# FabricioArendTorres/FlowConductor

Measured on AMD Instinct MI355X. Metric: log_prob samples/sec, 32xRQ-NSF coupling D=64 K=8, higher is better.
Workload: dtype f32

## Files before the change

flowconductor_amd/_hip.py:

```python
import ctypes
import os

import torch

_HERE = os.path.dirname(os.path.abspath(__file__))
LIB_PATH = os.path.join(_HERE, "csrc", "libflowcon_hip.so")

ABI_VERSION = 3

ERR_OUTSIDE_DOMAIN = 1
ERR_DISCRIMINANT = 2
ERR_NONFINITE = 4
ERR_NOT_LOWER_TRIANGULAR = 8
ERR_DIAGONAL_NONPOSITIVE = 16
ERR_NOT_SYMMETRIC = 32
ERR_NOT_POSITIVE_DEFINITE = 64
ERR_CHOLESKY_FAILED = 128


class HipLibraryMissing(RuntimeError):
    pass


class RQConfig(ctypes.Structure):

    _fields_ = [
        ("num_bins", ctypes.c_int32),
        ("tails", ctypes.c_int32),
        ("inverse", ctypes.c_int32),
        ("flags", ctypes.c_int32),
        ("left", ctypes.c_float),
        ("right", ctypes.c_float),
        ("bottom", ctypes.c_float),
        ("top", ctypes.c_float),
        ("min_bin_width", ctypes.c_double),
        ("min_bin_height", ctypes.c_double),
        ("min_derivative", ctypes.c_double),
        ("wh_divisor", ctypes.c_float),
        ("softplus_beta", ctypes.c_float),
        ("tail_constant", ctypes.c_float),
        ("reserved2", ctypes.c_float),
    ]


class SplineConfig(ctypes.Structure):

    _fields_ = [
        ("kind", ctypes.c_int32),
        ("num_bins", ctypes.c_int32),
        ("tails", ctypes.c_int32),
        ("inverse", ctypes.c_int32),
        ("left", ctypes.c_float),
        ("right", ctypes.c_float),
        ("bottom", ctypes.c_float),
        ("top", ctypes.c_float),
        ("min_bin_width", ctypes.c_double),
        ("min_bin_height", ctypes.c_double),
        ("width_divisor", ctypes.c_float),
        ("height_divisor", ctypes.c_float),
        ("cubic_eps", ctypes.c_float),
        ("cubic_quadratic_threshold", ctypes.c_float),
    ]


class PackJob(ctypes.Structure):

    _fields_ = [("w", ctypes.c_void_p), ("b", ctypes.c_void_p), ("frag", ctypes.c_void_p), ("unscale", ctypes.c_void_p),
                ("bias_out", ctypes.c_void_p), ("rows", ctypes.c_int32), ("cols", ctypes.c_int32),
                ("mode", ctypes.c_int32), ("p", ctypes.c_int32), ("pp", ctypes.c_int32), ("nks", ctypes.c_int32),
                ("nt", ctypes.c_int32), ("group", ctypes.c_int32)]


_P = ctypes.c_void_p
_I32 = ctypes.c_int32
_I64 = ctypes.c_int64
_F = ctypes.c_float

SIGNATURES = {
    "fc_abi_version": [],
    "fc_rq_spline": [_P, _P, _P, _P, _P, _P, _I64, _I32, _I32, _I32, _I32,
                     ctypes.POINTER(RQConfig), _P],
    "fc_rq_spline_backward": [_P, _P, _P, _P, _P, _P, _P, _I64, _I32, _I32, ctypes.POINTER(RQConfig), _P],
    "fc_standard_normal_log_prob": [_P, _P, _P, _I64, _I32, _F, _P],
    "fc_permute": [_P, _P, _P, _I64, _I32, _I64, _P],
    "fc_pointwise_affine": [_P, _P, _P, _P, _P, _P, _I64, _I64, _I32, _I32, _I32, _P],
    "fc_householder": [_P, _P, _P, _I64, _I32, _I32, _I32, _I32, _P],
    "fc_planar": [_P, _P, _P, _P, _P, _P, _I64, _I32, _I32, _P],
    "fc_linear_per_sample": [_P, _P, _P, _P, _I64, _I32, _I32, _F, _F, _P],
    "fc_linear": [_P, _P, _P, _P, _P, _I64, _I32, _I32, _P],
    "fc_sylvester": [_P, _P, _P, _P, _P, _P, _P, _P, _I64, _I32, _I32, _I32, _P],
    "fc_sum_of_sigmoids": [_P, _P, _P, _P, _P, _P, _I64, _I32, _I32, _I32, _I32, _I32, _F, _F, _F,
                           _I32, _I32, _P],
    "fc_sum_of_sigmoids_backward": [_P, _P, _P, _P, _P, _P, _I64, _I32, _I32, _F, _P],
    "fc_deep_sigmoid": [_P, _P, _P, _P, _P, _P, _I64, _I32, _I32, _I32, _I32, _I32, _F, _F, _F, _F, _I32, _I32, _P],
    "fc_deep_sigmoid_backward": [_P, _P, _P, _P, _P, _P, _I64, _I32, _I32, _F, _F, _F, _I32, _P],
    "fc_deep_sigmoid_backward_rows": [_I64, _I32, _I32],
    "fc_planar_backward": [_P, _P, _P, _P, _P, _P, _P, _P, _P, _P, _I64, _I32, _P],
    "fc_sylvester_mid_backward": [_P, _P, _P, _P, _P, _P, _I64, _I32, _P],
    "fc_householder_backward": [_P, _P, _P, _P, _P, _I64, _I32, _I32, _I32, _P],
    "fc_hdh_linear": [_P] * 7 + [_I64, _I32, _I32, _I32, _I32, _I32, _P],
    "fc_hdh_linear_backward": [_P] * 12 + [_I64, _I32, _I32, _I32, _I32, _I32, _P],
    "fc_elementwise": [_P, _P, _P, _P, _P, _P, _I64, _I64, _I32, _I32, _F, _F, _F, _F, _P],
    "fc_piecewise_spline_backward": [_P, _P, _P, _P, _P, _P, _P, _I64, _I32, _I32, ctypes.POINTER(SplineConfig), _P],
    "fc_piecewise_spline": [_P, _P, _P, _P, _P, _P, _I64, _I32, _I32, _I32, _I32,
                            ctypes.POINTER(SplineConfig), _P],
    "fc_rq_spline_fused_linear": [_P, _P, _P, _P, _P, _P, _P, _P, _I64, _I32, _I32, _I32,
                                  ctypes.POINTER(RQConfig), _P],
    "fc_rq_spline_fused_general": [_P, _P, _P, _P, _P, _P, _P, _P, _P, _I64, _I32, _I32, _I32,
                                   ctypes.POINTER(RQConfig), _P],
    "fc_rq_fused_linear_backward": [_I32, _P, _P, _P, _P, _P, _P, _P, _P, _P, _P, _P, _P, _P, _I64, _I32, _I32,
                                    ctypes.POINTER(RQConfig), _P],
    "fc_resnet_hidden": [_P, _P, _P, _P, _P, _P, _P, _I64, _I32, _I32, _I32, _I32, _I32, ctypes.c_float, _P],
    "fc_affine_coupling_resnet": [_P, _P, _P, _P, _P, _P, _P, _P, _I64, _I32, _I32, _I32, _I32, _I32, _I32, _I32, _I32, _P],
    "fc_made_inverse": [_P, _P, _P, _P, _P, _P, _P, _P, _P, _P, _P, _I64, _I32, _I32, _I32, _I32, ctypes.POINTER(RQConfig), _P],
    "fc_made_inverse_context": [_P] * 15 + [_I64, _I32, _I32, _I32, _I32, _I32, ctypes.POINTER(RQConfig), _P],
    "fc_mog_log_prob": [_P, _P, _P, _I64, _I32, _I32, _F, _I32, _P],
    "fc_mog_log_prob_backward": [_P, _P, _P, _P, _P, _I64, _I32, _I32, _F, _P],
    "fc_made_mog_sample": [_P] * 11 + [_I64, _I32, _I32, _I32, _F, _P],
    "fc_made_mog_sample_context": [_P] * 15 + [_I64, _I32, _I32, _I32, _I32, _F, _P],
    "fc_resnet_hidden_packed": [_P, _P, _P, _P, _P, _P, _I64, _I32, _I32, _I32, _I32, _I32, ctypes.c_float, _P],
    "fc_resnet_hidden_backward": [_P, _P, _P, _P, _P, _P, _P, _P, _P, _P, _P, _I64, _I32, _I32, _I32, _I32, _I32, _P],
    "fc_resnet_hidden_backward_accum": [_P, _P, _P, _P, _P, _P, _P, _P, _P, _P, _P, _I64, _I32, _I32, _I32, _I32, _I32, _P],
    "fc_resnet_hidden_wide": [_P, _P, _P, _P, _P, _P, _I64, _I32, _I32, _I32, _I32, _I32, ctypes.c_float, _P],
    "fc_resnet_hidden_context": [_P, _P, _P, _P, _P, _P, _P, _P, _P, _P, _I64, _I32, _I32, _I32, _I32, _I32, _I32,
                                 _I32, ctypes.c_float, _P],
    "fc_affine": [_P, _P, _P, _P, _P, _I64, _I32, _I32, _I32, _I32, _I32, _I32, _P],
    "fc_dense_mm": [_P, _P, _P, _P, _I64, _I32, _P],
    "fc_dense_mm_shifted": [_P, _P, _P, _P, _P, _I64, _I32, _P],
    "fc_sylvester_mm": [_P, _P, _P, _P, _P, _P, _P, _I64, _I32, _P],
    "fc_affine_backward": [_P, _P, _P, _P, _P, _P, _P, _I64, _I32, _I32, _I32, _P],
    "fc_pack_fragments": [_P, _I32, _P],
    "fc_pack_job_bytes": [],
    "fc_comm_unique_id": [_P],
    "fc_comm_init_rank": [ctypes.POINTER(ctypes.c_void_p), _I32, _P, _I32],
    "fc_comm_init_rank_on_device": [ctypes.POINTER(ctypes.c_void_p), _I32, _P, _I32, _I32],
    "fc_comm_destroy": [_P],
    "fc_comm_abort": [_P],
    "fc_allreduce_loglik": [_P, _P, _P],
    "fc_tril_pack": [_P, _P, _I64, _I32, _I32, _P],
    "fc_matrix_diag": [_P, _P, _P, _I64, _I32, _I32, _P],
    "fc_cholesky_outer": [_P, _P, _P, _P, _I64, _I32, _I32, _P],
    "fc_cholesky_outer_backward": [_P, _P, _P, _P, _I64, _I32, _P],
    "fc_cholesky": [_P, _P, _P, _P, _I64, _I32, _F, _I32, _P],
    "fc_squeeze": [_P, _P, _I64, _I32, _I32, _I32, _I32, _P],
    "fc_conv1x1": [_P, _P, _P, _P, _P, _I64, _I32, _I64, _P],
    "fc_iresnet_forward": [_P, _P, _P, _P, _P, _P, _I64, _I32, _I32, _I32, _I32, _I32, _I32, _P],
    "fc_iresnet_inverse": [_P, _P, _P, _P, _P, _P, _I64, _I32, _I32, _I32, _I32, _I32, _I32, _I32, _F, _F, _P],
    "fc_umnn": [_P] * 7 + [_I64, _I32, _I32, _I32, _I32, _I32, _I32, _P],
    "fc_radial": [_P] * 6 + [_I64, _I32, _I32, _P],
    "fc_radial_backward": [_P] * 10 + [_I64, _I32, _P],
    "fc_unit_vector": [_P] * 4 + [_I64, _I32, _I32, _P],
    "fc_unit_vector_backward": [_P] * 4 + [_I64, _I32, _I32, _P],
}

_lib = None


def use_library(path):
    global LIB_PATH
    if _lib is not None:
        raise RuntimeError("flowconductor_amd: %s is already loaded" % LIB_PATH)
    LIB_PATH = os.path.abspath(path)


def library_info():
    import hashlib

    with open(LIB_PATH, "rb") as f:
        blob = f.read()
    return {"path": os.path.relpath(LIB_PATH, os.path.dirname(_HERE)), "sha256": hashlib.sha256(blob).hexdigest(),
            "bytes": len(blob)}


def load():
    global _lib
    if _lib is not None:
        return _lib
    if not os.path.exists(LIB_PATH):
        raise HipLibraryMissing(
            "flowconductor_amd: %s not found. Build it with `python -c 'import __graft_entry__ as g; "
            "g.build()'` or `make -C flowconductor_amd/csrc`. There is no CPU fallback." % LIB_PATH
        )
    lib = ctypes.CDLL(LIB_PATH)
    for name, argtypes in SIGNATURES.items():
        fn = getattr(lib, name)
        fn.argtypes = argtypes
        fn.restype = ctypes.c_int
    got = lib.fc_abi_version()
    if got != ABI_VERSION:
        raise HipLibraryMissing("libflowcon_hip.so ABI %d != expected %d: rebuild" % (got, ABI_VERSION))
    _lib = lib
    return lib


def is_built():
    return os.path.exists(LIB_PATH)


def check(code, what):
    if code != 0:
        raise RuntimeError("flowconductor_amd: %s failed with hipError %d" % (what, code))


_raw_stream = getattr(torch._C, "_cuda_getCurrentRawStream", None)


def stream_ptr(device):
    if _raw_stream is not None:
        index = device.index
        return ctypes.c_void_p(_raw_stream(torch.cuda.current_device() if index is None else index))
    return ctypes.c_void_p(torch.cuda.current_stream(device).cuda_stream)


def dev_f32(t, name):
    if not isinstance(t, torch.Tensor):
        raise TypeError("%s must be a tensor" % name)
    if not t.is_cuda:
        raise RuntimeError(
            "flowconductor_amd: %s lives on %s; the bijector kernels run on a HIP device only "
            "(no CPU fallback)" % (name, t.device)
        )
    if t.dtype != torch.float32:
        raise TypeError("flowconductor_amd: %s must be float32, got %s" % (name, t.dtype))
    return t if t.is_contiguous() else t.contiguous()


def ptr(t):
    return ctypes.c_void_p(t.data_ptr()) if t is not None else None


def require_no_grad(*tensors):
    if torch.is_grad_enabled() and any(t is not None and t.requires_grad for t in tensors):
        raise RuntimeError(
            "flowconductor_amd: the HIP bijector kernels implement forward/inverse/logabsdet only; "
            "autograd through them is not available yet. Wrap the call in torch.no_grad()."
        )
```

flowconductor_amd/csrc/fc_resnet_hidden.hip:

```cpp
#include <hip/hip_runtime.h>
#include <stdint.h>
#include "fc_split.h"
#include "fc_lane.h"
#include "fc_math.h"
#include "fc_device.h"
#include "../../include/flowcon_hip.h"

#ifndef FC_HIDDEN_PREFETCH_X
#define FC_HIDDEN_PREFETCH_X 1
#endif

namespace fc {

constexpr int kHid = 64;
constexpr int kHidThreads = 512;

struct HiddenArgs {
  const float* x;
  float* h;
  const int32_t* id_cols;
  const float* w0;
  const float* b0;
  const float* wb;
  const float* bb;
  int64_t blocks16;
  int D;
  int k0;
  const float* ctx;
  const float* wc;
  const float* bc;
  int C;
  int act;
  float act_param;
  const f16x8* image;
  const float* image_un;
  const float* image_bias;
  float* y;
  const int32_t* tr_cols;
  float* lad;
  int d_t, affine_act, inverse, accumulate;
};

__host__ __device__ constexpr int hid_feat(int t, int g, int r) { return 32 * (t >> 1) + 8 * g + 4 * (t & 1) + r; }

template <int NB, int K0S, int kCtx, int kTail = 0>
struct HiddenLds {
  static constexpr int kMain = 1 + 2 * NB + kTail;
  static constexpr int kCtxLayers = kCtx == 1 ? NB : kCtx == 2 ? NB + 1 : 0;
  static constexpr int kLayers = kMain + kCtxLayers;
  static constexpr int kFrag0 = K0S * 4 * 2;
  static constexpr int kFragL = 2 * 4 * 2;
  static constexpr int kFragG = 1 * 4 * 2;
  static constexpr int kFragsMain = kFrag0 + (2 * NB + kTail) * kFragL;
  static constexpr int kFrags = kFragsMain + kCtxLayers * kFragG;
  static constexpr size_t kBytes = (size_t)kFrags * 64 * 16 + kLayers * 64 * 4 + 16 * 4 + 32 * K0S * 4 + 16 * 8 * 4;
  static_assert(kLayers <= 16, "wun holds 16 entries");
  static_assert(kBytes <= 160 * 1024, "weight fragments exceed the CU's LDS");
};

template <int NB, int K0S, int kCtx, int kAct, int BPW, int kTail = 0, int XVT = 8>
__global__ __launch_bounds__(512, (kCtx || BPW > 1 || kTail) ? 2 : 4) void resnet_hidden_kernel(HiddenArgs a) {
  static_assert(!kTail || kCtx == 0, "the coupling tail: no context");
  using L = HiddenLds<NB, K0S, kCtx, kTail>;
  constexpr bool kPrefetchX = FC_HIDDEN_PREFETCH_X && (K0S == 1 || kCtx != 0 || BPW > 1);
  extern __shared__ __attribute__((aligned(16))) unsigned char hsmem[];
  f16x8* wfrag = reinterpret_cast<f16x8*>(hsmem);
  float* bias = reinterpret_cast<float*>(hsmem + (size_t)L::kFrags * 64 * 16);
  float* wun = bias + L::kLayers * 64;
  int* ids = reinterpret_cast<int*>(wun + 16);
  float* red = reinterpret_cast<float*>(ids + 32 * K0S);

  const int tid = threadIdx.x, lane = tid & 63, wave = tid >> 6;
  const int s16 = lane & 15, g = lane >> 4;
  const int k0 = a.k0, D = a.D, C = kCtx ? a.C : 0;
#ifdef FC_HID_STAMP
  const uint64_t stamp_entry = __builtin_amdgcn_s_memtime();
#endif

  const int C0 = kCtx == 1 ? C : 0;
  for (int i = tid; i < 32 * K0S; i += kHidThreads) ids[i] = i < k0 ? a.id_cols[i] : (i < k0 + C0 ? -2 - (i - k0) : -1);
  if (kCtx == 0 && a.image) {
    for (int f = wave; f < L::kFrags; f += kHidThreads / 64)
      __builtin_amdgcn_global_load_lds((const __attribute__((address_space(1))) void*)(a.image + (size_t)f * 64 + lane),
                                       (__attribute__((address_space(3))) void*)(wfrag + f * 64), 16, 0, 0);
    for (int i = tid; i < L::kLayers * 64; i += kHidThreads) bias[i] = a.image_bias[i];
    if (tid < L::kLayers) wun[tid] = a.image_un[tid];
    asm volatile("s_waitcnt vmcnt(0)" ::: "memory");
    __syncthreads();
  } else if constexpr (!kTail) {
  auto layer_src = [&](int l, const float*& w, const float*& b, int& kin, int& nks, int& base) {
    const bool gate = l >= L::kMain;
    w = l == 0 ? a.w0 : gate ? a.wc + (size_t)(l - L::kMain) * kHid * C : a.wb + (size_t)(l - 1) * kHid * kHid;
    b = l == 0 ? a.b0 : gate ? a.bc + (size_t)(l - L::kMain) * kHid : a.bb + (size_t)(l - 1) * kHid;
    kin = l == 0 ? k0 + C0 : gate ? C : kHid;
    nks = l == 0 ? K0S : gate ? 1 : 2;
    base = l == 0 ? 0 : gate ? L::kFragsMain + (l - L::kMain) * L::kFragG : L::kFrag0 + (l - 1) * L::kFragL;
  };
  float wmax[L::kLayers];
#pragma unroll
  for (int l = 0; l < L::kLayers; ++l) {
    const float *w, *b;
    int kin, nks, base;
    layer_src(l, w, b, kin, nks, base);
    float m = 0.f;
    if (kin == kHid) {
      const float4* w4 = reinterpret_cast<const float4*>(w) + 2 * tid;
      const float4 p = w4[0], q = w4[1];
      m = fmaxf(fmaxf(fmaxf(fabsf(p.x), fabsf(p.y)), fmaxf(fabsf(p.z), fabsf(p.w))),
                fmaxf(fmaxf(fabsf(q.x), fabsf(q.y)), fmaxf(fabsf(q.z), fabsf(q.w))));
    } else {
      const int total = kHid * kin;
      for (int i = tid; i < total; i += 4 * kHidThreads) {
        const float v0 = w[i];
        const float v1 = i + kHidThreads < total ? w[i + kHidThreads] : 0.f;
        const float v2 = i + 2 * kHidThreads < total ? w[i + 2 * kHidThreads] : 0.f;
        const float v3 = i + 3 * kHidThreads < total ? w[i + 3 * kHidThreads] : 0.f;
        m = fmaxf(fmaxf(m, fmaxf(fabsf(v0), fabsf(v1))), fmaxf(fabsf(v2), fabsf(v3)));
      }
    }
    wmax[l] = m;
  }
#pragma unroll
  for (int l = 0; l < L::kLayers; ++l) {
    float m = wmax[l];
#pragma unroll
    for (int o = 32; o > 0; o >>= 1) m = fmaxf(m, __shfl_xor(m, o));
    if (lane == 0) red[l * (kHidThreads / 64) + wave] = m;
  }
  __syncthreads();
#pragma unroll
  for (int l = 0; l < L::kLayers; ++l) {
    const float *w, *b;
    int kin, nks, base;
    layer_src(l, w, b, kin, nks, base);
    float m = red[l * (kHidThreads / 64)];
#pragma unroll
    for (int i = 1; i < kHidThreads / 64; ++i) m = fmaxf(m, red[l * (kHidThreads / 64) + i]);
    float sc, un;
    pow2_scale(m, sc, un);
    if (tid == 0) wun[l] = un;
    for (int e = tid; e < nks * 4 * 64; e += kHidThreads) {
      const int ln = e & 63, t = (e >> 6) & 3, ks = e >> 8;
      const int rho = ln & 15, f = hid_feat(t, rho >> 2, rho & 3);
      f16x8 hi, lo;
      float v[8];
      if (kin == kHid) {
        const float4* w4 = reinterpret_cast<const float4*>(w + (size_t)f * kHid + 32 * ks + 8 * (ln >> 4));
        const float4 p = w4[0], q = w4[1];
        v[0] = p.x, v[1] = p.y, v[2] = p.z, v[3] = p.w, v[4] = q.x, v[5] = q.y, v[6] = q.z, v[7] = q.w;
      } else {
#pragma unroll
        for (int j = 0; j < 8; ++j) {
          const int k = 32 * ks + 8 * (ln >> 4) + j;
          v[j] = k < kin ? w[(size_t)f * kin + k] : 0.f;
        }
      }
#pragma unroll
      for (int j = 0; j < 8; ++j) {
        _Float16 ph, pl;
        split2(v[j] * sc, ph, pl);
        hi[j] = ph;
        lo[j] = pl;
      }
      wfrag[(base + (ks * 4 + t) * 2 + 0) * 64 + ln] = hi;
      wfrag[(base + (ks * 4 + t) * 2 + 1) * 64 + ln] = lo;
    }
    for (int i = tid; i < 64; i += kHidThreads) {
      const int gg = i >> 4, t = (i >> 2) & 3, r = i & 3;
      bias[l * 64 + i] = b[hid_feat(t, gg, r)];
    }
  }
  __syncthreads();
  }

  auto activate16 = [&](const f32x4 (&in)[4], f32x4 (&out)[4]) {
#define FC_ACT_LOOP(expr)                                            \
  _Pragma("unroll") for (int t = 0; t < 4; ++t)                      \
  _Pragma("unroll") for (int r = 0; r < 4; ++r) {                    \
    const float v = in[t][r];                                        \
    out[t][r] = (expr);                                              \
  }
    if constexpr (kAct == 0) {
      FC_ACT_LOOP(fmaxf(v, 0.f))
    } else {
      switch (a.act) {
        case FC_ACT_TANH: FC_ACT_LOOP(tanhf(v)) break;
        case FC_ACT_SILU: FC_ACT_LOOP(div_lean(v, 1.f + exp_lean(fminf(-v, 87.f)))) break;
        case FC_ACT_ELU: FC_ACT_LOOP(v > 0.f ? v : a.act_param * (exp_lean(v) - 1.f)) break;
        case FC_ACT_LEAKY_RELU: FC_ACT_LOOP(v > 0.f ? v : v * a.act_param) break;
        case FC_ACT_SIGMOID: FC_ACT_LOOP(div_lean(1.f, 1.f + exp_lean(fminf(-v, 87.f)))) break;
        default: FC_ACT_LOOP(fmaxf(v, 0.f)) break;
      }
    }
#undef FC_ACT_LOOP
  };
  auto make_operand = [&](const f32x4 (&v)[4], f16x8 (&bh)[2], f16x8 (&bl)[2]) {
    float m = 0.f;
#pragma unroll
    for (int t = 0; t < 4; ++t)
#pragma unroll
      for (int r = 0; r < 4; ++r) m = fmaxf(m, fabsf(v[t][r]));
    m = rows4_allmax(m, lane);
    float sc, un;
    pow2_scale(m, sc, un);
    u32x4 hh[2], ll[2];
#pragma unroll
    for (int t = 0; t < 4; ++t)
#pragma unroll
      for (int p = 0; p < 2; ++p) {
        uint32_t ph, pl;
        split2_pair(v[t][2 * p], v[t][2 * p + 1], sc, ph, pl);
        hh[t >> 1][2 * (t & 1) + p] = ph;
        ll[t >> 1][2 * (t & 1) + p] = pl;
      }
#pragma unroll
    for (int ks = 0; ks < 2; ++ks) {
      bh[ks] = __builtin_bit_cast(f16x8, hh[ks]);
      bl[ks] = __builtin_bit_cast(f16x8, ll[ks]);
    }
    return un;
  };
  auto layer = [&](int base, int nks, const f16x8 (&bh)[BPW][2], const f16x8 (&bl)[BPW][2], f32x4 (&acc)[BPW][4]) {
#pragma unroll
    for (int b = 0; b < BPW; ++b)
#pragma unroll
      for (int t = 0; t < 4; ++t) acc[b][t] = f32x4{0.f, 0.f, 0.f, 0.f};
    const f16x8* wf = wfrag + base * 64 + lane;
#pragma unroll
    for (int ks = 0; ks < 2; ++ks)
      if (ks < nks) {
        f16x8 wl[4];
#pragma unroll
        for (int t = 0; t < 4; ++t) wl[t] = wf[((ks * 4 + t) * 2 + 1) * 64];
#pragma unroll
        for (int t = 0; t < 4; ++t)
#pragma unroll
          for (int b = 0; b < BPW; ++b) acc[b][t] = __builtin_amdgcn_mfma_f32_16x16x32_f16(wl[t], bh[b][ks], acc[b][t], 0, 0, 0);
      }
#pragma unroll
    for (int ks = 0; ks < 2; ++ks)
      if (ks < nks) {
        f16x8 wh[4];
#pragma unroll
        for (int t = 0; t < 4; ++t) wh[t] = wf[((ks * 4 + t) * 2 + 0) * 64];
#pragma unroll
        for (int t = 0; t < 4; ++t)
#pragma unroll
          for (int b = 0; b < BPW; ++b) acc[b][t] = __builtin_amdgcn_mfma_f32_16x16x32_f16(wh[t], bl[b][ks], acc[b][t], 0, 0, 0);
#pragma unroll
        for (int t = 0; t < 4; ++t)
#pragma unroll
          for (int b = 0; b < BPW; ++b) acc[b][t] = __builtin_amdgcn_mfma_f32_16x16x32_f16(wh[t], bh[b][ks], acc[b][t], 0, 0, 0);
      }
  };
  auto finish = [&](int l, float un_act, const f32x4 (&acc)[4], f32x4 (&out)[4]) {
    const float c = un_act * wun[l];
    const f32x4* bsrc = reinterpret_cast<const f32x4*>(bias + l * 64 + g * 16);
#pragma unroll
    for (int t = 0; t < 4; ++t) {
      const f32x4 b = bsrc[t];
#pragma unroll
      for (int r = 0; r < 4; ++r) out[t][r] = __builtin_fmaf(acc[t][r], c, b[r]);
    }
  };

  int mycol[K0S][8];
#pragma unroll
  for (int ks = 0; ks < K0S; ++ks)
#pragma unroll
    for (int j = 0; j < 8; ++j) mycol[ks][j] = ids[32 * ks + 8 * g + j];

  const int64_t nwaves = (int64_t)gridDim.x * (kHidThreads / 64);
  int alt = -1;
  if (kCtx == 0 && D == 2 * k0 && k0 == 32 * K0S && ((uintptr_t)a.x & 15u) == 0 && (ids[0] == 0 || ids[0] == 1)) {
    alt = ids[0];
    for (int i = 1; i < k0; ++i)
      if (ids[i] != 2 * i + ids[0]) alt = -1;
  }
  auto gather = [&](int64_t blk, f32x4 (&xv)[4]) {
    const float* xrow = a.x + (blk * 16 + s16) * D;
    const float* crow_ = kCtx ? a.ctx + (blk * 16 + s16) * C : nullptr;
    if (alt >= 0) {
#pragma unroll
      for (int ks = 0; ks < 2; ++ks) {
        if (ks < K0S) {
          const float4* q = reinterpret_cast<const float4*>(xrow + 64 * ks + 16 * g);
          const float4 q0 = q[0], q1 = q[1], q2 = q[2], q3 = q[3];
          xv[2 * ks] = alt ? f32x4{q0.y, q0.w, q1.y, q1.w} : f32x4{q0.x, q0.z, q1.x, q1.z};
          xv[2 * ks + 1] = alt ? f32x4{q2.y, q2.w, q3.y, q3.w} : f32x4{q2.x, q2.z, q3.x, q3.z};
        } else {
          xv[2 * ks] = xv[2 * ks + 1] = f32x4{0.f, 0.f, 0.f, 0.f};
        }
      }
      return;
    }
#pragma unroll
    for (int t = 0; t < 4; ++t)
#pragma unroll
      for (int r = 0; r < 4; ++r) {
        const int ks = t >> 1, j = 4 * (t & 1) + r;
        float v = 0.f;
        if (ks < K0S) {
          const int c = mycol[ks < K0S ? ks : 0][j];
          if constexpr (kCtx == 1)
            v = c >= 0 ? xrow[c] : (c <= -2 ? crow_[-2 - c] : 0.f);
          else
            v = c >= 0 ? xrow[c] : 0.f;
        }
        xv[t][r] = v;
      }
  };
  if constexpr (kTail) {
    const int TS = D | 1, wrap = TS - D;
    float* tile = reinterpret_cast<float*>(hsmem + ((L::kBytes + 15) & ~size_t(15))) + (size_t)wave * BPW * 16 * TS;
    const int chunk4 = 4 * D;
    constexpr int XV = XVT;
    int toff[XV], tcol[XV];
#pragma unroll
    for (int k = 0; k < XV; ++k) {
      const int e = 4 * (lane + 64 * k), r = e / D;
      tcol[k] = e - r * D;
      toff[k] = r * TS + tcol[k];
    }
    auto fetch_rows = [&](int64_t blk, float4 (&raw)[XV]) __attribute__((always_inline)) {
      const float4* src = reinterpret_cast<const float4*>(a.x + blk * 16 * D);
#pragma unroll
      for (int k = 0; k < XV; ++k)
        if (lane + 64 * k < chunk4) raw[k] = src[lane + 64 * k];
    };
    const int64_t groups = (a.blocks16 + BPW - 1) / BPW;
    const int64_t nw = (int64_t)gridDim.x * (kHidThreads / 64);
    const int64_t first = (int64_t)blockIdx.x * (kHidThreads / 64) + wave;
    auto blk_of = [&](int64_t grp, int b) {
      const int64_t blk = grp * BPW + b;
      return blk < a.blocks16 ? blk : a.blocks16 - 1;
    };
    float4 raw[BPW][XV];
    if (first < groups) {
#pragma unroll
      for (int b = 0; b < BPW; ++b) fetch_rows(blk_of(first, b), raw[b]);
    }
    int tc[8];
#pragma unroll
    for (int e = 0; e < 8; ++e) {
      const int dim = 8 * g + e;
      tc[e] = a.tr_cols[dim < a.d_t ? dim : 0];
    }
    for (int64_t grp = first; grp < groups; grp += nw) {
      asm volatile("" ::: "memory");
#pragma unroll
      for (int b = 0; b < BPW; ++b)
#pragma unroll
        for (int k = 0; k < XV; ++k)
          if (lane + 64 * k < chunk4) {
            const float v[4] = {raw[b][k].x, raw[b][k].y, raw[b][k].z, raw[b][k].w};
#pragma unroll
            for (int j = 0; j < 4; ++j) tile[b * 16 * TS + toff[k] + j + (tcol[k] + j >= D ? wrap : 0)] = v[j];
          }
      __builtin_amdgcn_wave_barrier();
      if (grp + nw < groups) {
#pragma unroll
        for (int b = 0; b < BPW; ++b) fetch_rows(blk_of(grp + nw, b), raw[b]);
      }
      f32x4 xin[BPW][4];
      float xt[BPW][8];
#pragma unroll
      for (int b = 0; b < BPW; ++b) {
        const float* trow = tile + (b * 16 + s16) * TS;
#pragma unroll
        for (int t = 0; t < 4; ++t)
#pragma unroll
          for (int r = 0; r < 4; ++r) {
            const int ks = t >> 1, j = 4 * (t & 1) + r;
            float v = 0.f;
            if (ks < K0S) {
              const int c = mycol[ks < K0S ? ks : 0][j];
              v = c >= 0 ? trow[c] : 0.f;
            }
            xin[b][t][r] = v;
          }
#pragma unroll
        for (int e = 0; e < 8; ++e) xt[b][e] = trow[tc[e]];
      }
      f16x8 bh[BPW][2], bl[BPW][2];
      f32x4 acc[BPW][4], h[BPW][4], tmid[BPW][4];
      float un[BPW];
#pragma unroll
      for (int b = 0; b < BPW; ++b) un[b] = make_operand(xin[b], bh[b], bl[b]);
      layer(0, K0S, bh, bl, acc);
#pragma unroll
      for (int b = 0; b < BPW; ++b) finish(0, un[b], acc[b], h[b]);
#pragma unroll
      for (int nb = 0; nb < NB; ++nb) {
#pragma unroll
        for (int b = 0; b < BPW; ++b) {
          f32x4 act[4];
          activate16(h[b], act);
          un[b] = make_operand(act, bh[b], bl[b]);
        }
        layer(L::kFrag0 + (2 * nb) * L::kFragL, 2, bh, bl, acc);
#pragma unroll
        for (int b = 0; b < BPW; ++b) {
          finish(1 + 2 * nb, un[b], acc[b], tmid[b]);
          f32x4 act[4];
          activate16(tmid[b], act);
          un[b] = make_operand(act, bh[b], bl[b]);
        }
        layer(L::kFrag0 + (2 * nb + 1) * L::kFragL, 2, bh, bl, acc);
#pragma unroll
        for (int b = 0; b < BPW; ++b) {
          finish(2 + 2 * nb, un[b], acc[b], tmid[b]);
#pragma unroll
          for (int t = 0; t < 4; ++t)
#pragma unroll
            for (int r = 0; r < 4; ++r) h[b][t][r] += tmid[b][t][r];
        }
      }
#pragma unroll
      for (int b = 0; b < BPW; ++b) un[b] = make_operand(h[b], bh[b], bl[b]);
      layer(L::kFrag0 + 2 * NB * L::kFragL, 2, bh, bl, acc);
#pragma unroll
      for (int b = 0; b < BPW; ++b) {
        f32x4 prm[4];
        finish(1 + 2 * NB, un[b], acc[b], prm);
        float ladsum = 0.f;
        float* wrow = tile + (b * 16 + s16) * TS;
#pragma unroll
        for (int t = 0; t < 2; ++t)
#pragma unroll
          for (int r = 0; r < 4; ++r) {
            const int e = 4 * t + r;
            if (8 * g + e < a.d_t) {
              const float xv = xt[b][e], shift = prm[t][r], u = prm[2 + t][r];
              float sc = 1.f, ls = 0.f;
              if (a.affine_act == FC_AFFINE_SIGMOID_PLUS2) {
                const float v = u + 2.f;
                const float ex = exp_lean(-fabsf(v));
                const float rcp = div_lean(1.f, 1.f + ex);
                sc = (v >= 0.f ? rcp : ex * rcp) + 1e-3f;
                ls = log_lean(sc);
              } else if (a.affine_act == FC_AFFINE_SOFTPLUS_CLAMP3) {
                const float v = softplus_lean(u, 1.f) + 1e-3f;
                sc = v < 0.f ? 0.f : (v > 3.f ? 3.f : v);
                ls = log_lean(sc);
              } else if (a.affine_act == FC_AFFINE_MAF_SOFTPLUS) {
                sc = softplus_lean(u, 1.f) + 1e-3f;
                ls = log_lean(sc);
              }
              wrow[tc[e]] = a.inverse ? div_lean(xv - shift, sc) : xv * sc + shift;
              ladsum += a.inverse ? -ls : ls;
            }
          }
        const float l = rows4_allsum(ladsum, lane);
        const bool real = grp * BPW + b < a.blocks16;
        const int64_t row = blk_of(grp, b) * 16 + s16;
        if (g == 0 && real) a.lad[row] = a.accumulate ? a.lad[row] + l : l;
      }
      __builtin_amdgcn_wave_barrier();
#pragma unroll
      for (int b = 0; b < BPW; ++b) {
        if (grp * BPW + b >= a.blocks16) continue;
        float4* dst = reinterpret_cast<float4*>(a.y + blk_of(grp, b) * 16 * D);
#pragma unroll
        for (int k = 0; k < XV; ++k)
          if (lane + 64 * k < chunk4) {
            float v[4];
#pragma unroll
            for (int j = 0; j < 4; ++j) v[j] = tile[b * 16 * TS + toff[k] + j + (tcol[k] + j >= D ? wrap : 0)];
            dst[lane + 64 * k] = float4{v[0], v[1], v[2], v[3]};
          }
      }
      __builtin_amdgcn_wave_barrier();
    }
    return;
  }

  const int64_t groups = (a.blocks16 + BPW - 1) / BPW;
  const int64_t grp0 = (int64_t)blockIdx.x * (kHidThreads / 64) + wave;
  auto block_of = [&](int64_t grp, int b) {
    const int64_t blk = grp * BPW + b;
    return blk < a.blocks16 ? blk : a.blocks16 - 1;
  };
  f32x4 xpre[kPrefetchX ? BPW : 1][kPrefetchX ? 4 : 1];
  if constexpr (kPrefetchX) {
    if (grp0 < groups) {
#pragma unroll
      for (int b = 0; b < BPW; ++b) gather(block_of(grp0, b), xpre[b]);
    }
  }
#define FC_EACH_BLOCK _Pragma("unroll") for (int b = 0; b < BPW; ++b)
#ifdef FC_HID_STAMP
  const uint64_t stamp0 = __builtin_amdgcn_s_memtime(), stamp_r0 = __builtin_amdgcn_s_memrealtime();
#endif
  for (int64_t grp = grp0; grp < groups; grp += nwaves) {
    asm volatile("" ::: "memory");
    f32x4 xin[BPW][4];
    FC_EACH_BLOCK {
      if constexpr (kPrefetchX) {
#pragma unroll
        for (int t = 0; t < 4; ++t) xin[b][t] = xpre[b][t];
      } else {
        gather(block_of(grp, b), xin[b]);
      }
    }
    f16x8 bh[BPW][2], bl[BPW][2];
    f32x4 acc[BPW][4], h[BPW][4], tmid[BPW][4];
    float un[BPW];
    f16x8 ch[BPW][2] = {}, cl[BPW][2] = {};
    float unc[BPW];
    FC_EACH_BLOCK unc[b] = 1.f;
    if constexpr (kCtx) {
      FC_EACH_BLOCK {
        const float* crow = a.ctx + (block_of(grp, b) * 16 + s16) * C;
        float cv[8], m = 0.f;
#pragma unroll
        for (int j = 0; j < 8; ++j) {
          const int k = 8 * g + j;
          cv[j] = crow[k < C ? k : 0];
          cv[j] = k < C ? cv[j] : 0.f;
          m = fmaxf(m, fabsf(cv[j]));
        }
        m = rows4_allmax(m, lane);
        float sc;
        pow2_scale(m, sc, unc[b]);
#pragma unroll
        for (int j = 0; j < 8; ++j) {
          _Float16 ph, pl;
          split2(cv[j] * sc, ph, pl);
          ch[b][0][j] = ph;
          cl[b][0][j] = pl;
        }
      }
    }
    FC_EACH_BLOCK un[b] = make_operand(xin[b], bh[b], bl[b]);
    if constexpr (kPrefetchX) {
      const int64_t nxt = grp + nwaves < groups ? grp + nwaves : grp;
      FC_EACH_BLOCK gather(block_of(nxt, b), xpre[b]);
    }
    layer(0, K0S, bh, bl, acc);
    FC_EACH_BLOCK finish(0, un[b], acc[b], h[b]);
    if constexpr (kCtx == 2) {
      layer(L::kFragsMain, 1, ch, cl, acc);
      FC_EACH_BLOCK {
        f32x4 cpre[4], cact[4];
        finish(L::kMain, unc[b], acc[b], cpre);
        activate16(cpre, cact);
#pragma unroll
        for (int t = 0; t < 4; ++t)
#pragma unroll
          for (int r = 0; r < 4; ++r) h[b][t][r] += cact[t][r];
      }
    }
#pragma unroll
    for (int nb = 0; nb < NB; ++nb) {
      FC_EACH_BLOCK {
        f32x4 act[4];
        activate16(h[b], act);
        un[b] = make_operand(act, bh[b], bl[b]);
      }
      layer(L::kFrag0 + (2 * nb) * L::kFragL, 2, bh, bl, acc);
      FC_EACH_BLOCK finish(1 + 2 * nb, un[b], acc[b], tmid[b]);
      if constexpr (kCtx == 2) {
        layer(L::kFragsMain + (1 + nb) * L::kFragG, 1, ch, cl, acc);
        FC_EACH_BLOCK {
          f32x4 cpre[4];
          finish(L::kMain + 1 + nb, unc[b], acc[b], cpre);
#pragma unroll
          for (int t = 0; t < 4; ++t)
#pragma unroll
            for (int r = 0; r < 4; ++r) tmid[b][t][r] += cpre[t][r];
        }
      }
      FC_EACH_BLOCK {
        f32x4 act[4];
        activate16(tmid[b], act);
        un[b] = make_operand(act, bh[b], bl[b]);
      }
      layer(L::kFrag0 + (2 * nb + 1) * L::kFragL, 2, bh, bl, acc);
      FC_EACH_BLOCK finish(2 + 2 * nb, un[b], acc[b], tmid[b]);
      if constexpr (kCtx == 1) {
        layer(L::kFragsMain + nb * L::kFragG, 1, ch, cl, acc);
        FC_EACH_BLOCK {
          f32x4 gpre[4];
          finish(L::kMain + nb, unc[b], acc[b], gpre);
#pragma unroll
          for (int t = 0; t < 4; ++t)
#pragma unroll
            for (int r = 0; r < 4; ++r)
              tmid[b][t][r] *= __builtin_amdgcn_rcpf(1.f + exp_lean(fminf(-gpre[t][r], 87.f)));
        }
      }
      FC_EACH_BLOCK {
#pragma unroll
        for (int t = 0; t < 4; ++t)
#pragma unroll
          for (int r = 0; r < 4; ++r) h[b][t][r] += tmid[b][t][r];
      }
    }
    FC_EACH_BLOCK {
      const int64_t blk = grp * BPW + b;
      if (blk < a.blocks16) {
        float4* hrow = reinterpret_cast<float4*>(a.h + (blk * 16 + s16) * kHid);
        hrow[2 * g] = float4{h[b][0][0], h[b][0][1], h[b][0][2], h[b][0][3]};
        hrow[2 * g + 1] = float4{h[b][1][0], h[b][1][1], h[b][1][2], h[b][1][3]};
        hrow[8 + 2 * g] = float4{h[b][2][0], h[b][2][1], h[b][2][2], h[b][2][3]};
        hrow[8 + 2 * g + 1] = float4{h[b][3][0], h[b][3][1], h[b][3][2], h[b][3][3]};
      }
    }
  }
#ifdef FC_HID_STAMP
  if (lane == 0 && grp0 < groups) {
    float* dst = a.h + (grp0 * BPW * 16) * kHid;
    dst[0] = (float)(__builtin_amdgcn_s_memtime() - stamp0);
    dst[1] = (float)((groups - grp0 + nwaves - 1) / nwaves * BPW);
    dst[2] = (float)(stamp0 - stamp_entry);
    dst[3] = (float)(__builtin_amdgcn_s_memrealtime() - stamp_r0);
  }
#endif
#undef FC_EACH_BLOCK
}

template <int NB, int K0S, int kCtx, int kAct, int BPW, int kTail = 0, int XVT = 8>
hipError_t launch_hidden(const HiddenArgs& a, int64_t grid, hipStream_t s) {
  using L = HiddenLds<NB, K0S, kCtx, kTail>;
  static PerDeviceOnce attr;
  const hipError_t ea = ensure_max_dynamic_lds(
      attr, reinterpret_cast<const void*>(&resnet_hidden_kernel<NB, K0S, kCtx, kAct, BPW, kTail, XVT>), 160 * 1024);
  if (ea != hipSuccess) return ea;
  if (kTail && a.D > 16 * XVT) return hipErrorInvalidValue;
  const size_t lds = kTail ? ((L::kBytes + 15) & ~size_t(15)) + (size_t)(kHidThreads / 64) * BPW * 16 * (a.D | 1) * 4 : L::kBytes;
  if (lds > 160 * 1024) return hipErrorInvalidConfiguration;
  hipLaunchKernelGGL((resnet_hidden_kernel<NB, K0S, kCtx, kAct, BPW, kTail, XVT>), dim3((unsigned)grid), dim3(kHidThreads), lds,
                     s, a);
  return hipGetLastError();
}

template <int NB, int K0S>
inline hipError_t launch_coupling_tail(const HiddenArgs& a, hipStream_t s) {
  using L = HiddenLds<NB, K0S, 0, 1>;
  const int64_t cus = device_cu_count();
  const size_t lds2 = ((L::kBytes + 15) & ~size_t(15)) + (size_t)(kHidThreads / 64) * 2 * 16 * (a.D | 1) * 4;
  const bool pairs = a.blocks16 >= 2 * cus * 8 && lds2 <= 160 * 1024 && a.D <= 64;
  const int64_t units = pairs ? (a.blocks16 + 1) / 2 : a.blocks16;
  int64_t grid = cus;
  const int64_t need = (units + 7) / 8;
  if (grid > need) grid = need;
  if (!pairs) return launch_hidden<NB, K0S, 0, 0, 1, 1>(a, grid, s);
  if (a.D <= 32) return launch_hidden<NB, K0S, 0, 0, 2, 1, 2>(a, grid, s);
  return launch_hidden<NB, K0S, 0, 0, 2, 1, 4>(a, grid, s);
}

inline hipError_t dispatch_coupling_tail(const HiddenArgs& a, int num_blocks, hipStream_t s) {
  const bool wide = a.k0 > 32;
  switch (num_blocks * 2 + (wide ? 1 : 0)) {
    case 0: return launch_coupling_tail<0, 1>(a, s);
    case 1: return launch_coupling_tail<0, 2>(a, s);
    case 2: return launch_coupling_tail<1, 1>(a, s);
    case 3: return launch_coupling_tail<1, 2>(a, s);
    case 4: return launch_coupling_tail<2, 1>(a, s);
    case 5: return launch_coupling_tail<2, 2>(a, s);
    case 6: return launch_coupling_tail<3, 1>(a, s);
    case 7: return launch_coupling_tail<3, 2>(a, s);
    default: return hipErrorInvalidValue;
  }
}

template <int kCtx, int kAct>
hipError_t dispatch_hidden(const HiddenArgs& a, int num_blocks, hipStream_t s) {
  const int cus = device_cu_count();
  const bool wide = a.k0 + (kCtx == 1 ? a.C : 0) > 32;
#ifdef FC_HID_FORCE_BPW
  constexpr bool kPairs = kCtx == 0 && kAct == 0;
  const bool pairs = kPairs && FC_HID_FORCE_BPW == 2;
#else
  const bool pairs = false;
#endif
  const size_t frags = (size_t)(wide ? 16 : 8) + (size_t)num_blocks * (2 * 16 + (kCtx ? 8 : 0));
  int64_t grid = (int64_t)cus * (!pairs && !kCtx && frags * 1024 + 2048 <= 80 * 1024 ? 2 : 1);
  const int64_t need = ((pairs ? (a.blocks16 + 1) / 2 : a.blocks16) + 7) / 8;
  if (grid > need) grid = need;
#ifdef FC_HID_FORCE_BPW
#define FC_HIDDEN_CASE(NB_, K0S_)                                                            \
  do {                                                                                       \
    if constexpr (kPairs) {                                                                  \
      if (pairs) return launch_hidden<NB_, K0S_, kCtx, kAct, 2>(a, grid, s);                 \
    }                                                                                        \
    return launch_hidden<NB_, K0S_, kCtx, kAct, 1>(a, grid, s);                              \
  } while (0)
#else
#define FC_HIDDEN_CASE(NB_, K0S_) return launch_hidden<NB_, K0S_, kCtx, kAct, 1>(a, grid, s)
#endif
  switch (num_blocks * 2 + (wide ? 1 : 0)) {
    case 0: FC_HIDDEN_CASE(0, 1);
    case 1: FC_HIDDEN_CASE(0, 2);
    case 2: FC_HIDDEN_CASE(1, 1);
    case 3: FC_HIDDEN_CASE(1, 2);
    case 4: FC_HIDDEN_CASE(2, 1);
    case 5: FC_HIDDEN_CASE(2, 2);
    case 6: FC_HIDDEN_CASE(3, 1);
    case 7: FC_HIDDEN_CASE(3, 2);
    default: break;
  }
  if constexpr (!kCtx) {
    if (wide) FC_HIDDEN_CASE(4, 2);
    FC_HIDDEN_CASE(4, 1);
  }
#undef FC_HIDDEN_CASE
  return hipErrorInvalidValue;
}

}

extern "C" int fc_resnet_hidden(const float* x, float* h, const int32_t* id_cols, const float* w0,
                                const float* b0, const float* wb, const float* bb, int64_t n, int32_t d,
                                int32_t in_features, int32_t hidden, int32_t num_blocks, int32_t activation,
                                float activation_param, void* stream) {
  if (n < 0 || d <= 0 || hidden != fc::kHid || num_blocks < 0 || num_blocks > 4) return hipErrorInvalidValue;
  if (activation < FC_ACT_RELU || activation > FC_ACT_SIGMOID) return hipErrorInvalidValue;
  if (in_features <= 0 || in_features > 64 || in_features > d) return hipErrorInvalidValue;
  if (n % 16 != 0) return hipErrorInvalidValue;
  if (n == 0) return hipSuccess;
  if (!x || !h || !id_cols || !w0 || !b0 || (num_blocks > 0 && (!wb || !bb))) return hipErrorInvalidValue;
  if (((uintptr_t)h & 15u) != 0 || ((uintptr_t)wb & 15u) != 0) return hipErrorInvalidValue;
  fc::HiddenArgs a{x, h, id_cols, w0, b0, wb, bb, n / 16, d, in_features, nullptr, nullptr, nullptr, 0,
                   activation, activation_param, nullptr, nullptr, nullptr, nullptr, nullptr, nullptr, 0, 0, 0, 0};
  if (activation == FC_ACT_RELU) return fc::dispatch_hidden<0, 0>(a, num_blocks, static_cast<hipStream_t>(stream));
  return fc::dispatch_hidden<0, 1>(a, num_blocks, static_cast<hipStream_t>(stream));
}

extern "C" int fc_resnet_hidden_packed(const float* x, float* h, const int32_t* id_cols, const void* w_frag,
                                       const float* w_unscale, const float* bias_acc, int64_t n, int32_t d,
                                       int32_t in_features, int32_t hidden, int32_t num_blocks, int32_t activation,
                                       float activation_param, void* stream) {
  if (n < 0 || d <= 0 || hidden != fc::kHid || num_blocks < 0 || num_blocks > 4) return hipErrorInvalidValue;
  if (activation < FC_ACT_RELU || activation > FC_ACT_SIGMOID) return hipErrorInvalidValue;
  if (in_features <= 0 || in_features > 64 || in_features > d) return hipErrorInvalidValue;
  if (n % 16 != 0) return hipErrorInvalidValue;
  if (n == 0) return hipSuccess;
  if (!x || !h || !id_cols || !w_frag || !w_unscale || !bias_acc) return hipErrorInvalidValue;
  if (((uintptr_t)h & 15u) != 0 || ((uintptr_t)w_frag & 15u) != 0) return hipErrorInvalidValue;
  fc::HiddenArgs a{x, h, id_cols, nullptr, nullptr, nullptr, nullptr, n / 16, d, in_features, nullptr, nullptr, nullptr, 0,
                   activation, activation_param, static_cast<const fc::f16x8*>(w_frag), w_unscale, bias_acc,
                   nullptr, nullptr, nullptr, 0, 0, 0, 0};
  if (activation == FC_ACT_RELU) return fc::dispatch_hidden<0, 0>(a, num_blocks, static_cast<hipStream_t>(stream));
  return fc::dispatch_hidden<0, 1>(a, num_blocks, static_cast<hipStream_t>(stream));
}

extern "C" int fc_affine_coupling_resnet(const float* x, float* y, const int32_t* id_cols, const int32_t* tr_cols,
                                         const void* w_frag, const float* w_unscale, const float* bias_acc,
                                         float* logabsdet, int64_t n, int32_t d, int32_t in_features, int32_t d_t,
                                         int32_t hidden, int32_t num_blocks, int32_t scale_activation, int32_t inverse,
                                         int32_t accumulate, void* stream) {
  if (n < 0 || d <= 0 || hidden != fc::kHid || num_blocks < 0 || num_blocks > 3) return hipErrorInvalidValue;
  if (in_features <= 0 || in_features > 64 || d_t <= 0 || d_t > 32 || in_features > d || d_t > d || d > 128) return hipErrorInvalidValue;
  if (scale_activation != FC_AFFINE_SIGMOID_PLUS2 && scale_activation != FC_AFFINE_SOFTPLUS_CLAMP3 &&
      scale_activation != FC_AFFINE_ADDITIVE && scale_activation != FC_AFFINE_MAF_SOFTPLUS)
    return hipErrorInvalidValue;
  if (n % 16 != 0) return hipErrorInvalidValue;
  if (n == 0) return hipSuccess;
  if (!x || !y || x == y || !id_cols || !tr_cols || !w_frag || !w_unscale || !bias_acc || !logabsdet) return hipErrorInvalidValue;
  if (((uintptr_t)w_frag & 15u) != 0) return hipErrorInvalidValue;
  fc::HiddenArgs a{x, nullptr, id_cols, nullptr, nullptr, nullptr, nullptr, n / 16, d, in_features, nullptr, nullptr, nullptr, 0,
                   FC_ACT_RELU, 0.f, static_cast<const fc::f16x8*>(w_frag), w_unscale, bias_acc,
                   y, tr_cols, logabsdet, d_t, scale_activation, inverse ? 1 : 0, accumulate ? 1 : 0};
  return fc::dispatch_coupling_tail(a, num_blocks, static_cast<hipStream_t>(stream));
}

extern "C" int fc_resnet_hidden_context(const float* x, const float* context, float* h, const int32_t* id_cols,
                                        const float* w0, const float* b0, const float* wb, const float* bb,
                                        const float* wc, const float* bc, int64_t n, int32_t d,
                                        int32_t in_features, int32_t context_features, int32_t hidden,
                                        int32_t num_blocks, int32_t context_mode, int32_t activation,
                                        float activation_param, void* stream) {
  if (activation < FC_ACT_RELU || activation > FC_ACT_SIGMOID) return hipErrorInvalidValue;
  if (context_mode != FC_CONTEXT_GLU && context_mode != FC_CONTEXT_ADDITIVE) return hipErrorInvalidValue;
  if (n < 0 || d <= 0 || hidden != fc::kHid || num_blocks < 0 || num_blocks > 3) return hipErrorInvalidValue;
  if (in_features <= 0 || in_features > d || context_features <= 0 || context_features > 32 ||
      in_features + (context_mode == FC_CONTEXT_GLU ? context_features : 0) > 64)
    return hipErrorInvalidValue;
  if (n % 16 != 0) return hipErrorInvalidValue;
  if (n == 0) return hipSuccess;
  if (!x || !context || !h || !id_cols || !w0 || !b0 || (num_blocks > 0 && (!wb || !bb || !wc || !bc)))
    return hipErrorInvalidValue;
  if (context_mode == FC_CONTEXT_ADDITIVE && (!wc || !bc)) return hipErrorInvalidValue;
  if (((uintptr_t)h & 15u) != 0 || ((uintptr_t)wb & 15u) != 0) return hipErrorInvalidValue;
  fc::HiddenArgs a{x, h, id_cols, w0, b0, wb, bb, n / 16, d, in_features, context, wc, bc, context_features,
                   activation, activation_param, nullptr, nullptr, nullptr, nullptr, nullptr, nullptr, 0, 0, 0, 0};
  hipStream_t s = static_cast<hipStream_t>(stream);
  if (context_mode == FC_CONTEXT_GLU)
    return activation == FC_ACT_RELU ? fc::dispatch_hidden<1, 0>(a, num_blocks, s) : fc::dispatch_hidden<1, 1>(a, num_blocks, s);
  return activation == FC_ACT_RELU ? fc::dispatch_hidden<2, 0>(a, num_blocks, s) : fc::dispatch_hidden<2, 1>(a, num_blocks, s);
}
```

flowconductor_amd/csrc/fc_rq_fused.h:

```cpp
#pragma once
#include <hip/hip_runtime.h>
#include <stdint.h>
#include "fc_rq_op.h"

namespace fc {

constexpr int kRowsMin = 32;
constexpr int kH = 64;
constexpr int kDt = 32;
constexpr int kK = 8;
constexpr int kPP = 24;

struct FusedArgs {
  const float* x;
  float* y;
  const float* h;
  const float* wpad;
  const float* bias;
  const int32_t* cols;
  float* logabsdet;
  uint32_t* err;
  int64_t tiles;
  int D;
  int accumulate;
  int dt;
  int wrows;
};

size_t fused3_lds_bytes(int d, int rows);
hipError_t launch_fused3(const RQOp<kK>& op, const FusedArgs& a, int rows, unsigned grid, hipStream_t stream);

}
```

flowconductor_amd/csrc/fc_rq_fused.hip:

```cpp
#include <hip/hip_runtime.h>
#include <stdint.h>
#include "fc_tile.h"
#include "fc_rq_op.h"
#include "fc_rq_fused.h"
#include "../../include/flowcon_hip.h"

extern "C" int fc_rq_spline_fused_linear(const float* x, float* y, const float* h, const float* w_pad,
                                         const float* bias_pad, const int32_t* cols, float* logabsdet,
                                         uint32_t* err_flag, int64_t n, int32_t d, int32_t d_t, int32_t hidden,
                                         const fc_rq_config* cfg, void* stream) {
  if (!cfg || n < 0 || d < d_t) return hipErrorInvalidValue;
  if (hidden != fc::kH || d_t < 1 || d_t > fc::kDt || cfg->num_bins != fc::kK || cfg->tails != 1 ||
      d > 128)
    return hipErrorInvalidValue;
  if (n % fc::kRowsMin != 0) return hipErrorInvalidValue;
  if (n == 0) return hipSuccess;
  if (!x || !y || !h || !w_pad || !bias_pad || !cols || !logabsdet) return hipErrorInvalidValue;
  if ((((uintptr_t)h | (uintptr_t)x | (uintptr_t)y) & 15u) != 0) return hipErrorInvalidValue;

  fc::RQOp<fc::kK> op;
  fc::RQParams& q = op.q;
  q.K = cfg->num_bins; q.tails = 1; q.inverse = cfg->inverse;
  q.left = cfg->left; q.right = cfg->right; q.bottom = cfg->bottom; q.top = cfg->top;
  q.min_w = (float)cfg->min_bin_width; q.min_h = (float)cfg->min_bin_height; q.min_d = (float)cfg->min_derivative;
  q.cw = (float)(1.0 - cfg->min_bin_width * q.K);
  q.ch = (float)(1.0 - cfg->min_bin_height * q.K);
  fc::rq_finish_params(q);
  q.wh_div = cfg->wh_divisor > 0.f ? cfg->wh_divisor : 1.f;
  q.beta = cfg->softplus_beta;
  q.tail_const = cfg->tail_constant;
  op.inv_div = 1.f / q.wh_div;
  op.inv_beta = 1.f / q.beta;

  const int acc = (cfg->flags & FC_RQ_ACCUMULATE_LOGABSDET) ? 1 : 0;
  const int wrows = (cfg->flags & FC_RQ_RAW_WEIGHTS) ? fc::kPP - 1 : fc::kPP;
  hipStream_t s = static_cast<hipStream_t>(stream);
  const int64_t cus = fc::device_cu_count();
  const bool wide_ok = fc::fused3_lds_bytes(d, 64) <= 160 * 1024;
  const int64_t n64 = wide_ok ? n - n % 64 : 0;
  if (n64 > 0) {
    fc::FusedArgs a{x, y, h, w_pad, bias_pad, cols, logabsdet, err_flag, n64 / 64, d, acc, d_t, wrows};
    const hipError_t e = fc::launch_fused3(op, a, 64, (unsigned)(cus < a.tiles ? cus : a.tiles), s);
    if (e != hipSuccess) return e;
  }
  if (n64 < n) {
    fc::FusedArgs a{x + n64 * d, y + n64 * d, h + n64 * fc::kH, w_pad, bias_pad, cols, logabsdet + n64, err_flag,
                    (n - n64) / 32, d, acc, d_t, wrows};
    return fc::launch_fused3(op, a, 32, (unsigned)(cus < a.tiles ? cus : a.tiles), s);
  }
  return hipSuccess;
}
```

flowconductor_amd/csrc/fc_rq_fused3.hip:

```cpp
#include <hip/hip_runtime.h>
#include <stdint.h>
#include <type_traits>
#include "fc_tile.h"
#include "fc_math.h"
#include "fc_rq_op.h"
#include "fc_rq_fused.h"
#include "fc_split.h"
#include "fc_lane.h"
#include "../../include/flowcon_hip.h"

#ifndef FC_ABL
#define FC_ABL 0
#endif

namespace fc {

#ifndef FC_HOOK_MASK
#define FC_HOOK_MASK 0
#endif
#define FC_F2 f2
#ifndef FC_PRIO_PERIOD
#define FC_PRIO_PERIOD 36
#endif

constexpr int kCt3 = 6;
constexpr int kHB = kH + 16;
constexpr int kKnotFloats = (kK + 1) * 64 * 2;
constexpr int kDerFloats = (kK + 1) * 64;
constexpr int kTabBytes = 8 * (kKnotFloats + kDerFloats) * 4;

template <int R>
struct Fused3Lds {
  static constexpr int kHPiece = R * kHB;
  static constexpr int kHbufBytes = 2 * 2 * kHPiece * 2;
  static constexpr int kLpartBytes = 3 * 8 * R * 4;
  static constexpr int kHscaleBytes = 3 * R * 4;
  static constexpr size_t bytes(int d) {
    return (size_t)kHbufBytes + kLpartBytes + kHscaleBytes + kTabBytes + 3 * R * (d + 4) * 4 + kDt * 4;
  }
};

size_t fused3_lds_bytes(int d, int rows) { return rows == 64 ? Fused3Lds<64>::bytes(d) : Fused3Lds<32>::bytes(d); }

template <bool kInv, int R, int XV, bool kFull, bool kPadX>
__global__ __launch_bounds__(512) void rq_fused_linear_kernel3(RQOp<kK> op, FusedArgs a) {
  using L = Fused3Lds<R>;
  constexpr int kHPiece = L::kHPiece;
  constexpr int NB = R / 16;
  constexpr int HV = R / 32;
  extern __shared__ __attribute__((aligned(16))) unsigned char smem3[];
  _Float16* hbuf = reinterpret_cast<_Float16*>(smem3);
  float* lpart = reinterpret_cast<float*>(smem3 + L::kHbufBytes);
  float* hscale = lpart + 3 * 8 * R;
  float* tabs = hscale + 3 * R;
  float* xbuf = tabs + kTabBytes / 4;
  const int D = a.D, XS = kPadX ? D + 4 : D;
  int* cs = reinterpret_cast<int*>(xbuf + 3 * R * (D + 4));

  const int tid = threadIdx.x, wave = tid >> 6, lane = tid & 63;
  const int s16 = lane & 15, g = lane >> 4;
  const int64_t stride = gridDim.x;
  const int64_t tile0 = blockIdx.x;
  if (tile0 >= a.tiles) return;
  if (tid < kDt) cs[tid] = tid < a.dt ? a.cols[tid] : 0;
  const int WD = kFull ? 8 : (a.dt + 3) >> 2;
  const bool dim_ok = kFull || 4 * wave + g < a.dt;
  const bool active = kFull || wave < WD;
  const float inv_div = op.inv_div;
#if FC_ABL & 16
  const uint64_t stamp_r_entry = __builtin_amdgcn_s_memrealtime();
#endif

  constexpr auto slot_param = [](int s) { return s < 16 ? ((s & 1) ? 8 + (s >> 1) : (s >> 1)) : s; };
  f16x8 wh[kCt3][2], wl[kCt3][2];
  float w_unscale;
  {
    float wv[kCt3][2][8];
    float wmax = 0.f;
#pragma unroll
    for (int t = 0; t < kCt3; ++t) {
      const int wdim = 4 * (active ? wave : 0) + (s16 >> 2), wprm = slot_param(4 * t + (s16 & 3));
      const bool wreal = wprm < kPP - 1 && wdim < a.dt;
      const int row = wreal ? wdim * a.wrows + wprm : 0;
      const float wmask = wreal ? 1.f : 0.f;
#pragma unroll
      for (int ks = 0; ks < 2; ++ks) {
        const float4* src = reinterpret_cast<const float4*>(a.wpad + (int64_t)row * kH + 32 * ks + 8 * g);
        const float4 v0 = src[0], v1 = src[1];
        const float v[8] = {v0.x * wmask, v0.y * wmask, v0.z * wmask, v0.w * wmask,
                            v1.x * wmask, v1.y * wmask, v1.z * wmask, v1.w * wmask};
#pragma unroll
        for (int j = 0; j < 8; ++j) {
          wv[t][ks][j] = v[j];
          wmax = fmaxf(wmax, fabsf(v[j]));
        }
      }
    }
#pragma unroll
    for (int o = 32; o > 0; o >>= 1) wmax = fmaxf(wmax, __shfl_xor(wmax, o));
    float w_scale;
    pow2_scale(wmax, w_scale, w_unscale);
#pragma unroll
    for (int t = 0; t < kCt3; ++t)
#pragma unroll
      for (int ks = 0; ks < 2; ++ks)
#pragma unroll
        for (int j = 0; j < 8; ++j) {
          _Float16 ph, pl;
          split2(wv[t][ks][j] * w_scale, ph, pl);
          wh[t][ks][j] = ph;
          wl[t][ks][j] = pl;
        }
  }
  const float wh_mul = (float)((double)inv_div * 1.4426950408889634);
  f32x4 bw[kCt3];
#pragma unroll
  for (int t = 0; t < kCt3; ++t) {
    const int bdim = 4 * (active ? wave : 0) + g;
    const float* bsrc = a.bias + bdim * a.wrows;
    const float m = t < 4 ? wh_mul : op.q.beta;
    const bool bdim_ok = bdim < a.dt;
    auto bias_of = [&](int slot) {
      const int prm = slot_param(slot);
      const bool real = prm < kPP - 1 && bdim_ok;
      return (real ? bsrc[prm] : a.bias[0]) * (real ? m : 0.f);
    };
    bw[t] = f32x4{bias_of(4 * t), bias_of(4 * t + 1), bias_of(4 * t + 2), bias_of(4 * t + 3)};
  }
  const double span_x = (double)op.q.right - (double)op.q.left, span_y = (double)op.q.top - (double)op.q.bottom;
  const f2 sc1 = {(float)(span_x * (double)op.q.cw), (float)(span_y * (double)op.q.ch)};
  auto knot_const = [&](int i) {
    if (i < kK / 2)
      return f2{(float)((double)op.q.left + span_x * (double)op.q.min_w * (double)(i + 1)),
                (float)((double)op.q.bottom + span_y * (double)op.q.min_h * (double)(i + 1))};
    return f2{(float)((double)op.q.right - span_x * (double)op.q.min_w * (double)(kK - 1 - i)),
              (float)((double)op.q.top - span_y * (double)op.q.min_h * (double)(kK - 1 - i))};
  };
  const f2 kc0 = knot_const(0), kc1 = knot_const(1), kc2 = knot_const(2), kc3 = knot_const(3), kc4 = knot_const(4),
           kc5 = knot_const(5), kc6 = knot_const(6);
  static_assert(kK == 8, "kc0 .. kc6: the generated evaluation is for 8 bins");

  float* ktab = tabs + wave * (kKnotFloats + kDerFloats) + lane * 2;
  float* dtab = tabs + wave * (kKnotFloats + kDerFloats) + kKnotFloats + lane;
  *reinterpret_cast<f2*>(ktab) = f2{op.q.left, op.q.bottom};
  *reinterpret_cast<f2*>(ktab + kK * 128) = f2{op.q.right, op.q.top};
  dtab[0] = op.q.tail_const * op.q.beta;
  dtab[kK * 64] = op.q.tail_const * op.q.beta;

  uint32_t err = 0;
  int mycol = 0;
  const int xvec = R * D / 4;
  constexpr bool kCarry = kFull && XV <= 2;
  float4 hv0, hv1, xv0, xv1, xv2, xv3;
  hv0 = hv1 = xv0 = xv1 = xv2 = xv3 = float4{0.f, 0.f, 0.f, 0.f};
  int64_t fetched = tile0;
  auto fetch = [&](int64_t t) __attribute__((always_inline)) {
    fetched = t;
    if (FC_ABL & 8) t = tile0;
    const float4* hg = reinterpret_cast<const float4*>(a.h + t * R * kH);
    hv0 = hg[tid];
    if constexpr (HV > 1 && kFull) hv1 = hg[tid + 512];
    const float4* xg = reinterpret_cast<const float4*>(a.x + t * R * D);
    xv0 = xg[tid < xvec ? tid : 0];
    if constexpr (kCarry) {
      if constexpr (XV > 1) xv1 = xg[tid + 512 < xvec ? tid + 512 : 0];
      if constexpr (XV > 2) xv2 = xg[tid + 1024 < xvec ? tid + 1024 : 0];
      if constexpr (XV > 3) xv3 = xg[tid + 1536 < xvec ? tid + 1536 : 0];
    }
  };
  auto xslot = [&](int buf, int i) __attribute__((always_inline)) {
    if constexpr (!kPadX) return reinterpret_cast<float4*>(xbuf + buf * R * XS + 4 * i);
    const int e = i * 4, r = e / D, c = e - r * D;
    return reinterpret_cast<float4*>(xbuf + (buf * R + r) * XS + c);
  };
  auto park_h = [&](int buf, int xbuf3, int k, const float4& hvk) __attribute__((always_inline)) {
    const int c = (tid & 15) * 4, r = (tid >> 4) + 32 * k;
#if FC_ABL & 32
    {
      _Float16* dst = hbuf + (buf * 2 * R + r) * kHB + c;
      *reinterpret_cast<u32x2*>(dst) = u32x2{__float_as_uint(hvk.x) & 0x3bff3bffu, __float_as_uint(hvk.y) & 0x3bff3bffu};
      *reinterpret_cast<u32x2*>(dst + kHPiece) = u32x2{__float_as_uint(hvk.z) & 0x3bff3bffu, __float_as_uint(hvk.w) & 0x3bff3bffu};
      if ((tid & 15) == 0) hscale[xbuf3 * R + r] = 1.f;
      return;
    }
#endif
    const float v[4] = {hvk.x, hvk.y, hvk.z, hvk.w};
    const float m = row16_allmax(fmaxf(fmaxf(fabsf(v[0]), fabsf(v[1])), fmaxf(fabsf(v[2]), fabsf(v[3]))));
    float sc, un;
    pow2_scale(m, sc, un);
    u32x2 p0, p1;
#pragma unroll
    for (int j = 0; j < 2; ++j) {
      uint32_t ph, pl;
      split2_pair(v[2 * j], v[2 * j + 1], sc, ph, pl);
      p0[j] = ph; p1[j] = pl;
    }
    _Float16* dst = hbuf + (buf * 2 * R + r) * kHB + c;
    *reinterpret_cast<u32x2*>(dst) = p0;
    *reinterpret_cast<u32x2*>(dst + kHPiece) = p1;
    if ((tid & 15) == 0) hscale[xbuf3 * R + r] = un;
  };
  auto park = [&](int hb2, int x3) __attribute__((always_inline)) {
    park_h(hb2, x3, 0, hv0);
    if constexpr (HV > 1 && !kFull)
      hv1 = reinterpret_cast<const float4*>(a.h + ((FC_ABL & 8) ? tile0 : fetched) * R * kH)[tid + 512];
    if constexpr (HV > 1) park_h(hb2, x3, 1, hv1);
    if (tid < xvec) *xslot(x3, tid) = xv0;
    if constexpr (!kCarry && XV > 1) {
      const float4* xg = reinterpret_cast<const float4*>(a.x + ((FC_ABL & 8) ? tile0 : fetched) * R * D);
      xv1 = xg[tid + 512 < xvec ? tid + 512 : 0];
      if constexpr (XV > 2) xv2 = xg[tid + 1024 < xvec ? tid + 1024 : 0];
      if constexpr (XV > 3) xv3 = xg[tid + 1536 < xvec ? tid + 1536 : 0];
    }
    if constexpr (XV > 1) if (tid + 512 < xvec) *xslot(x3, tid + 512) = xv1;
    if constexpr (XV > 2) if (tid + 1024 < xvec) *xslot(x3, tid + 1024) = xv2;
    if constexpr (XV > 3) if (tid + 1536 < xvec) *xslot(x3, tid + 1536) = xv3;
  };
  auto hfrag = [&](int hb, int blk, int hp, int ks) {
    return *reinterpret_cast<const f16x8*>(hbuf + ((hb * 2 + hp) * R + 16 * blk + s16) * kHB + 32 * ks + 8 * g);
  };

  auto mfma_n = [&](auto N, f32x4 (&acc)[kCt3], const f16x8& bcur) {
    constexpr int n = decltype(N)::value, term = n / 12, ks = (n / 6) % 2, t = n % 6;
    const f16x8& aop = term == 0 ? wl[t][ks] : wh[t][ks];
    acc[t] = __builtin_amdgcn_mfma_f32_16x16x32_f16(aop, bcur, n < kCt3 ? f32x4{0.f, 0.f, 0.f, 0.f} : acc[t], 0, 0, 0);
  };
  constexpr auto term_h = [](int term) { return term == 1 ? 1 : 0; };

#define FC_ALL36(M)                                                                                          \
  M(0) M(1) M(2) M(3) M(4) M(5) M(6) M(7) M(8) M(9) M(10) M(11) M(12) M(13) M(14) M(15) M(16) M(17) M(18)     \
  M(19) M(20) M(21) M(22) M(23) M(24) M(25) M(26) M(27) M(28) M(29) M(30) M(31) M(32) M(33) M(34) M(35)

  auto produce_only = [&](f32x4 (&acc)[kCt3], int hb, int blk) {
    f16x8 bcur = hfrag(hb, blk, term_h(0), 0);
    auto one = [&](auto N) {
      constexpr int n = decltype(N)::value;
      if constexpr (n % 6 == 0 && n > 0) bcur = hfrag(hb, blk, term_h(n / 12), (n / 6) % 2);
      mfma_n(N, acc, bcur);
    };
#define FC_S(n) one(std::integral_constant<int, n>{});
    FC_ALL36(FC_S)
#undef FC_S
  };

  auto step = [&](const f32x4 (&pa)[kCt3], int xb, int cblk, f32x4 (&acc)[kCt3], int hb, int pblk, float& lad_out) {
    float* xr = xbuf + (xb * R + 16 * cblk + s16) * XS + mycol;
    const float x = *xr;
    const float c_d = hscale[xb * R + 16 * cblk + s16] * w_unscale;
    const float c_wh = c_d * wh_mul;
    const float c_ud = c_d * op.q.beta;
    f16x8 bcur, bnext = hfrag(hb, pblk, term_h(0), 0);
    auto hook = [&](auto N) {
      constexpr int n = decltype(N)::value;
      if constexpr (n % 6 == 0) {
        bcur = bnext;
        if constexpr (n + 6 < 36) bnext = hfrag(hb, pblk, term_h((n + 6) / 12), ((n + 6) / 6) % 2);
      }
      if constexpr (!(FC_ABL & 4)) mfma_n(N, acc, bcur);
      if constexpr (n % (FC_PRIO_PERIOD / 4) == FC_PRIO_PERIOD / 4 - 1)
        __builtin_amdgcn_s_setprio(3 - ((n + 1) % FC_PRIO_PERIOD) / (FC_PRIO_PERIOD / 4));
      __builtin_amdgcn_sched_barrier(FC_HOOK_MASK);
    };
    const RQParams& q = op.q;
    const float inv_beta = op.inv_beta;
    float y, lad;
    __builtin_amdgcn_s_setprio(3);
    __builtin_amdgcn_sched_barrier(0);
#define FC_HOOK(n) hook(std::integral_constant<int, n>{});
#define FC_WH_SLOT(i) ((i) < 8 ? 2 * (i) : 2 * ((i) - 8) + 1)
#define FC_WH(i) __builtin_fmaf(pa[FC_WH_SLOT(i) >> 2][FC_WH_SLOT(i) & 3], c_wh, bw[FC_WH_SLOT(i) >> 2][FC_WH_SLOT(i) & 3])
#define FC_UD(j) __builtin_fmaf(pa[((j) + 16) >> 2][((j) + 16) & 3], c_ud, bw[((j) + 16) >> 2][((j) + 16) & 3])
#define FC_KNOT_ST(slot, v) *reinterpret_cast<f2*>(ktab + (slot) * 128) = (v)
#define FC_KNOT_LD(i, off) *reinterpret_cast<const f2*>(ktab + ((i) + (off)) * 128)
#define FC_DER_ST(slot, v) dtab[(slot) * 64] = (v)
#define FC_DER_LD(i, off) dtab[((i) + (off)) * 64]
#define FC_COUNT_GE(count, a, b)                                                              \
  do {                                                                                        \
    const float fc_b_ = (b);                                                                  \
    asm("v_cmp_ge_f32 vcc, %1, %2\n\tv_addc_co_u32 %0, vcc, 0, %0, vcc" : "+v"(count) : "v"(a), "v"(fc_b_) : "vcc"); \
  } while (0)
#if FC_ABL & 1
    FC_ALL36(FC_HOOK)
    y = x + (FC_WH(0) + FC_WH(5) + FC_WH(10) + FC_WH(15) + FC_UD(0) + FC_UD(5)) * 0.f + q.left * 0.f;
    lad = 0.f;
#else
#include "fc_rq_fused3_eval.inc"
#endif
#undef FC_COUNT_GE
#undef FC_DER_LD
#undef FC_DER_ST
#undef FC_KNOT_LD
#undef FC_KNOT_ST
#undef FC_UD
#undef FC_WH
#undef FC_WH_SLOT
#undef FC_HOOK
    if (dim_ok) *xr = y;
    lad_out = dim_ok ? lad : 0.f;
  };
  auto after_steps = [&](int xb, const float (&lb)[NB]) __attribute__((always_inline)) {
    if constexpr (NB == 4) {
      const float l = lane_merge16(lb[0], lane_merge32(lb[2], lb[3]));
      lpart[(xb * 8 + wave) * R + 16 * rows4_sum4_index(g) + s16] = l;
    } else {
      const float m = lane_merge32(lb[0], lb[1]);
      const float l = m + lane_xor16(m, lane);
      if ((g & 1) == 0) lpart[(xb * 8 + wave) * R + 16 * (g >> 1) + s16] = l;
    }
  };

#if FC_ABL & 16
  const uint64_t stamp_c0 = __builtin_amdgcn_s_memtime(), stamp_r0 = __builtin_amdgcn_s_memrealtime();
#endif
#if FC_ABL & 16
  uint64_t barrier_wait = 0, phase_cyc[6] = {0, 0, 0, 0, 0, 0}, phase_t = __builtin_amdgcn_s_memtime();
#define FC_PHASE(k)                                              \
  do {                                                           \
    const uint64_t now = __builtin_amdgcn_s_memtime();           \
    phase_cyc[k] += now - phase_t;                               \
    phase_t = now;                                               \
  } while (0)
#define FC_TIMED_BARRIER()                                        \
  do {                                                            \
    const uint64_t b0 = __builtin_amdgcn_s_memtime();             \
    __syncthreads();                                              \
    barrier_wait += __builtin_amdgcn_s_memtime() - b0;            \
  } while (0)
#else
#define FC_TIMED_BARRIER() __syncthreads()
#define FC_PHASE(k)
#endif
  f32x4 acc0[kCt3], acc1[kCt3];
#pragma unroll
  for (int t = 0; t < kCt3; ++t) acc0[t] = acc1[t] = f32x4{0.f, 0.f, 0.f, 0.f};
  auto write_out = [&](int64_t t, int x3) __attribute__((always_inline)) {
    float4* yg = reinterpret_cast<float4*>(a.y + t * R * D);
#pragma unroll
    for (int k = 0; k < XV; ++k)
      if (tid + 512 * k < xvec) yg[tid + 512 * k] = *xslot(x3, tid + 512 * k);
    if (tid < R) {
      const float* lp = lpart + x3 * 8 * R + tid;
      float l = lp[0];
#pragma unroll
      for (int w = 1; w < 8; ++w)
        if (w < WD) l += lp[w * R];
      a.logabsdet[t * R + tid] = a.accumulate ? a.logabsdet[t * R + tid] + l : l;
    }
  };
  fetch(tile0);
  park(0, 0);
  __syncthreads();
  mycol = cs[(4 * wave + g) & (kDt - 1)];
  if (active) produce_only(acc0, 0, 0);
  int hb = 0, x3 = 0;
  int64_t prev_tile = -1;
  for (int64_t tile = tile0; tile < a.tiles; tile += stride) {
    const bool has_next = tile + stride < a.tiles;
    const int x3n = x3 == 2 ? 0 : x3 + 1, x3p = x3 == 0 ? 2 : x3 - 1;
    FC_PHASE(0);
    if (has_next) fetch(tile + stride);
    float lb[NB];
#pragma unroll
    for (int b = 0; b < NB; ++b) lb[b] = 0.f;
    if (active) {
      step(acc0, x3, 0, acc1, hb, 1, lb[0]);
      if constexpr (NB == 4) {
        step(acc1, x3, 1, acc0, hb, 2, lb[1]);
        lb[0] = lane_merge32(lb[0], lb[1]);
        step(acc0, x3, 2, acc1, hb, 3, lb[2]);
      }
    }
    FC_PHASE(1);
    if (has_next) park(hb ^ 1, x3n);
    FC_PHASE(2);
    FC_TIMED_BARRIER();
    FC_PHASE(3);
    if (prev_tile >= 0) write_out(prev_tile, x3p);
    FC_PHASE(5);
    if (active) {
      step(acc1, x3, NB - 1, acc0, hb ^ 1, 0, lb[NB - 1]);
      after_steps(x3, lb);
    }
    FC_PHASE(4);
    prev_tile = tile;
    hb ^= 1;
    x3 = x3n;
  }
  __syncthreads();
  if (prev_tile >= 0) write_out(prev_tile, x3 == 0 ? 2 : x3 - 1);
#if FC_ABL & 16
  if (tid == 0) {
    a.y[tile0 * R * D] = (float)(__builtin_amdgcn_s_memtime() - stamp_c0);
    a.y[tile0 * R * D + 1] = (float)(__builtin_amdgcn_s_memrealtime() - stamp_r0);
    a.y[tile0 * R * D + 2] = (float)(stamp_r0 - stamp_r_entry);
    a.y[tile0 * R * D + 3] = (float)(stamp_r_entry & 0xffffff);
  }
  if (lane == 0) {
    a.y[tile0 * R * D + 4 + wave] = (float)barrier_wait;
#pragma unroll
    for (int k = 0; k < 6; ++k) a.y[tile0 * R * D + 12 + wave * 6 + k] = (float)phase_cyc[k];
  }
#endif
  if (err && a.err) atomicOr(a.err, err);
}
#undef FC_ALL36
#undef FC_TIMED_BARRIER
#undef FC_PHASE

template <bool kInv, int R, int XV, bool kFull, bool kPadX>
static hipError_t launch_cfg(const RQOp<kK>& op, const FusedArgs& a, unsigned grid, hipStream_t stream) {
  const size_t lds = Fused3Lds<R>::bytes(a.D);
  if (lds > 160 * 1024) return hipErrorInvalidConfiguration;
  static PerDeviceOnce attr;
  const hipError_t ea = ensure_max_dynamic_lds(
      attr, reinterpret_cast<const void*>(&rq_fused_linear_kernel3<kInv, R, XV, kFull, kPadX>), 160 * 1024);
  if (ea != hipSuccess) return ea;
  hipLaunchKernelGGL((rq_fused_linear_kernel3<kInv, R, XV, kFull, kPadX>), dim3(grid), dim3(512), lds, stream, op, a);
  return hipGetLastError();
}

template <bool kInv, int R, int XV>
static hipError_t launch_one(const RQOp<kK>& op, const FusedArgs& a, unsigned grid, hipStream_t stream) {
  if (a.D & 3) return launch_cfg<kInv, R, XV, false, false>(op, a, grid, stream);
  return a.dt == kDt ? launch_cfg<kInv, R, XV, true, true>(op, a, grid, stream)
                     : launch_cfg<kInv, R, XV, false, true>(op, a, grid, stream);
}

hipError_t launch_fused3(const RQOp<kK>& op, const FusedArgs& a, int rows, unsigned grid, hipStream_t stream) {
  const bool inv = op.q.inverse != 0;
  if (rows == 64) {
    if (a.D <= 32) return inv ? launch_one<true, 64, 1>(op, a, grid, stream) : launch_one<false, 64, 1>(op, a, grid, stream);
    if (a.D <= 64) return inv ? launch_one<true, 64, 2>(op, a, grid, stream) : launch_one<false, 64, 2>(op, a, grid, stream);
    return inv ? launch_one<true, 64, 4>(op, a, grid, stream) : launch_one<false, 64, 4>(op, a, grid, stream);
  }
  if (a.D <= 64) return inv ? launch_one<true, 32, 1>(op, a, grid, stream) : launch_one<false, 32, 1>(op, a, grid, stream);
  return inv ? launch_one<true, 32, 2>(op, a, grid, stream) : launch_one<false, 32, 2>(op, a, grid, stream);
}

}
```

flowconductor_amd/nn/nets/resnet.py:

```python
import torch
from torch import nn
from torch.nn import functional as F

from flowconductor_amd import ops


class ResidualBlock(nn.Module):

    def __init__(self, features, context_features, activation=torch.nn.ReLU(),
                 dropout_probability=0.0, use_batch_norm=False, zero_initialization=True):
        super().__init__()
        self.activation = activation
        self.use_batch_norm = use_batch_norm
        if use_batch_norm:
            self.batch_norm_layers = nn.ModuleList(nn.BatchNorm1d(features, eps=1e-3) for _ in range(2))
        if context_features is not None:
            self.context_layer = nn.Linear(context_features, features)
        self.linear_layers = nn.ModuleList(nn.Linear(features, features) for _ in range(2))
        self.dropout = nn.Dropout(p=dropout_probability)
        if zero_initialization:
            last = self.linear_layers[-1]
            nn.init.uniform_(last.weight, -1e-3, 1e-3)
            nn.init.uniform_(last.bias, -1e-3, 1e-3)

    def forward(self, inputs, context=None):
        h = inputs
        for i in range(2):
            if self.use_batch_norm:
                h = self.batch_norm_layers[i](h)
            h = self.activation(h)
            if i == 1:
                h = self.dropout(h)
            h = self.linear_layers[i](h)
        if context is not None:
            h = F.glu(torch.cat((h, self.context_layer(context)), dim=1), dim=1)
        return inputs + h


class ResidualNet(nn.Module):

    def __init__(self, in_features, out_features, hidden_features, context_features=None,
                 num_blocks=2, activation=torch.nn.ReLU(), dropout_probability=0.0,
                 use_batch_norm=False):
        super().__init__()
        self.hidden_features = hidden_features
        self.context_features = context_features
        first_in = in_features if context_features is None else in_features + context_features
        self.initial_layer = nn.Linear(first_in, hidden_features)
        self.blocks = nn.ModuleList(
            ResidualBlock(features=hidden_features, context_features=context_features,
                          activation=activation, dropout_probability=dropout_probability,
                          use_batch_norm=use_batch_norm)
            for _ in range(num_blocks)
        )
        self.final_layer = nn.Linear(hidden_features, out_features)

    def hidden(self, inputs, context=None):
        if context is not None:
            inputs = torch.cat((inputs, context), dim=1)
        h = self.initial_layer(inputs)
        for block in self.blocks:
            h = block(h, context=context)
        return h

    def forward(self, inputs, context=None):
        if self._hip_forward_ok(inputs, context):
            n = inputs.shape[0]
            body = n - n % 16
            ids = ops.memo(self, "all_cols", (inputs.shape[1], inputs.device),
                           lambda: torch.arange(inputs.shape[1], dtype=torch.int32, device=inputs.device))
            hidden = self.hidden_hip(inputs[:body], ids, None if context is None else context[:body])
            if body < n:
                hidden = torch.cat((hidden, self.hidden_padded(inputs[body:],
                                                               None if context is None else context[body:])))
            return self.final_from_padded(hidden)
        return self.final_layer(self.hidden(inputs, context))

    def _hip_forward_ok(self, inputs, context):
        from flowconductor_amd import options

        from flowconductor_amd import ops

        if not (inputs.dim() == 2 and inputs.is_cuda and inputs.dtype == torch.float32 and inputs.shape[0] >= 16
                and options.get("fused_hidden") and not ops.has_hooks(self)):
            return False
        if torch.is_grad_enabled() and (inputs.requires_grad or any(p.requires_grad for p in self.parameters())):
            return False
        return inputs.shape[1] + (0 if context is None else self.context_features or 0) == self.initial_layer.in_features \
            and self.hip_hidden_supported(inputs.shape[1], context)

    def train(self, mode=True):
        from flowconductor_amd import ops

        ops.invalidate_hip_caches()
        return super().train(mode)

    def hip_hidden_supported(self, features_total, context=None):
        from flowconductor_amd import ops

        def known(f):
            return ops.activation_code(f) is not None

        if self.hidden_features > 64 or len(self.blocks) > 4:
            return False
        in_f = self.initial_layer.in_features
        if (self.context_features is None) != (context is None):
            return False
        if context is not None:
            c = self.context_features
            if len(self.blocks) > 3:
                return False
            if (context.dim() != 2 or context.shape[1] != c or c > 32 or context.dtype != torch.float32
                    or not context.is_cuda or context.requires_grad and torch.is_grad_enabled()):
                return False
            if in_f - c <= 0 or in_f - c > features_total:
                return False
        if in_f > 64 or (context is None and in_f > features_total):
            return False
        for block in self.blocks:
            if block.use_batch_norm or not known(block.activation):
                return False
            if ops.activation_code(block.activation) != ops.activation_code(self.blocks[0].activation):
                return False
            if block.dropout.p > 0 and self.training:
                return False
        return True

    def hip_hidden_wide_supported(self, features_total, context=None):
        from flowconductor_amd import ops

        if not 64 < self.hidden_features <= 256 or context is not None or self.context_features is not None:
            return False
        in_f = self.initial_layer.in_features
        if in_f > 64 or in_f > features_total or len(self.blocks) > 16:
            return False
        for block in self.blocks:
            code = ops.activation_code(block.activation)
            if block.use_batch_norm or code is None or code != ops.activation_code(self.blocks[0].activation):
                return False
            if block.dropout.p > 0 and self.training:
                return False
        return True

    def hidden_hip_wide(self, rows, id_cols):
        from flowconductor_amd import ops

        width = ops.general_hidden_width(self.hidden_features)
        packed = ops.memo(self, "hip_packed_wide", ops.cache_key(*self._param_list(), extra=("wide", width)),
                          lambda: ops.pack_resnet_hidden_wide(self, width))
        act = ops.activation_code(self.blocks[0].activation) if len(self.blocks) else (ops.ACT_RELU, 0.0)
        return ops.resnet_hidden_wide(rows, id_cols, packed, self.initial_layer.in_features, len(self.blocks), width, act)

    def hip_hidden_backward_supported(self):
        from flowconductor_amd import ops

        if self.hidden_features > 64 or len(self.blocks) > 2 or self.context_features is not None:
            return False
        if self.initial_layer.in_features > 64:
            return False
        for block in self.blocks:
            code = ops.activation_code(block.activation)
            if block.use_batch_norm or code is None or code[0] != ops.ACT_RELU or (block.dropout.p > 0 and self.training):
                return False
        return True

    def _storage_key(self):
        return tuple(p.data_ptr() for p in self._param_list())

    def _param_list(self):
        return ops.param_list(self)

    def _apply(self, fn, *args, **kwargs):
        out = super()._apply(fn, *args, **kwargs)
        ops.drop_param_list(self)
        return out

    def hidden_backward_packed(self):
        from flowconductor_amd import ops

        pack, packed = self.hidden_backward_plan()
        pack.refresh()
        return packed

    def hidden_backward_plan(self):
        from flowconductor_amd import ops

        return ops.device_plan(self, "hip_packed_bwd", self._storage_key(),
                               lambda: ops.device_pack_resnet_hidden_backward(self))

    def hidden_padded(self, inputs, context=None):
        h = self.hidden(inputs, context)
        return h if h.shape[1] == 64 else F.pad(h, (0, 64 - h.shape[1]))

    def final_from_padded(self, hidden64):
        from flowconductor_amd import ops

        lin = self.final_layer
        if lin.in_features == 64:
            return lin(hidden64)
        weight = ops.memo(self, "final_padded", ops.cache_key(lin.weight),
                          lambda: F.pad(lin.weight.detach(), (0, 64 - lin.in_features)))
        return F.linear(hidden64, weight, lin.bias)

    def hidden_hip(self, rows, id_cols, context=None):
        from flowconductor_amd import ops

        in_features = self.initial_layer.in_features - (self.context_features or 0)
        act = ops.activation_code(self.blocks[0].activation) if len(self.blocks) else (ops.ACT_RELU, 0.0)
        if context is None:
            if self.training and self.hip_hidden_backward_supported():
                w_frag, _, w_un, bias_acc, _ = self.hidden_backward_packed()
                return ops.resnet_hidden_packed(rows, id_cols, (w_frag, w_un, bias_acc), in_features, len(self.blocks), act)
            pack, image = ops.device_plan(self, "hip_image", self._storage_key(),
                                          lambda: ops.device_pack_resnet_hidden_forward(self))
            pack.refresh()
            return ops.resnet_hidden_packed(rows, id_cols, image, in_features, len(self.blocks), act)
        packed = ops.memo(self, "hip_packed", ops.cache_key(*self._param_list()), lambda: ops.pack_resnet_hidden(self))
        return ops.resnet_hidden(rows, id_cols, packed, in_features, len(self.blocks), context, act)


class ConvResidualBlock(nn.Module):

    def __init__(self, channels, context_channels=None, activation=F.relu, dropout_probability=0.0,
                 use_batch_norm=False, zero_initialization=True):
        super().__init__()
        self.activation = activation
        if context_channels is not None:
            self.context_layer = nn.Conv2d(in_channels=context_channels, out_channels=channels, kernel_size=1,
                                           padding=0)
        self.use_batch_norm = use_batch_norm
        if use_batch_norm:
            self.batch_norm_layers = nn.ModuleList(nn.BatchNorm2d(channels, eps=1e-3) for _ in range(2))
        self.conv_layers = nn.ModuleList(nn.Conv2d(channels, channels, kernel_size=3, padding=1) for _ in range(2))
        self.dropout = nn.Dropout(p=dropout_probability)
        if zero_initialization:
            nn.init.uniform_(self.conv_layers[-1].weight, -1e-3, 1e-3)
            nn.init.uniform_(self.conv_layers[-1].bias, -1e-3, 1e-3)

    def forward(self, inputs, context=None):
        h = inputs
        for i in range(2):
            if self.use_batch_norm:
                h = self.batch_norm_layers[i](h)
            h = self.activation(h)
            if i == 1:
                h = self.dropout(h)
            h = self.conv_layers[i](h)
        if context is not None:
            h = F.glu(torch.cat((h, self.context_layer(context)), dim=1), dim=1)
        return inputs + h


class ConvResidualNet(nn.Module):

    def __init__(self, in_channels, out_channels, hidden_channels, context_channels=None, num_blocks=2,
                 activation=F.relu, dropout_probability=0.0, use_batch_norm=False):
        super().__init__()
        self.context_channels = context_channels
        self.hidden_channels = hidden_channels
        first_in = in_channels if context_channels is None else in_channels + context_channels
        self.initial_layer = nn.Conv2d(in_channels=first_in, out_channels=hidden_channels, kernel_size=1, padding=0)
        self.blocks = nn.ModuleList(
            ConvResidualBlock(channels=hidden_channels, context_channels=context_channels, activation=activation,
                              dropout_probability=dropout_probability, use_batch_norm=use_batch_norm)
            for _ in range(num_blocks))
        self.final_layer = nn.Conv2d(hidden_channels, out_channels, kernel_size=1, padding=0)

    def forward(self, inputs, context=None):
        if context is None:
            temps = self.initial_layer(inputs)
        else:
            temps = self.initial_layer(torch.cat((inputs, context), dim=1))
        for block in self.blocks:
            temps = block(temps, context)
        return self.final_layer(temps)
```

flowconductor_amd/ops/__init__.py:

```python
from ._core import (
    InputOutsideDomain, InverseNotAvailable, KernelTimer, LAD_ACCUMULATE, LAD_ACCUMULATE_NEG, LAD_STORE, LAD_STORE_NEG,
    MSG_CHOLESKY_FAILED, MSG_DIAGONAL_NONPOSITIVE, MSG_NOT_LOWER_TRIANGULAR, MSG_NOT_POSITIVE_DEFINITE, MSG_NOT_SQUARE,
    MSG_NOT_SYMMETRIC, _aligned16, _as_cols, _call, _check_now, _err_word, _finish, _flag_for, _flags,
    _logabsdet_target, _pad_to, _prep_2d, _raise_for, _state, buffer_list, cache_key, cached, capture_mode,
    check_errors, deferred_errors, device_plan, drop_param_list, has_hooks, invalidate_hip_caches, memo, module_list,
    param_list, rq_param_count, static_memo, structure_key)
from .rq import (
    DEFAULT_MIN_BIN_HEIGHT, DEFAULT_MIN_BIN_WIDTH, DEFAULT_MIN_DERIVATIVE, _RQSplineFunction, _inverse_through_forward,
    _rq_config, rq_spline, rq_spline_autograd, rq_spline_backward)
from .packing import (
    DevicePack, FRAG_ELEMS, FRAG_KSTEP, FUSED_BINS, FUSED_DT, FUSED_HIDDEN, FUSED_ROWS, PACK_FINAL, PACK_FINAL_T,
    PACK_HIDDEN, PACK_HIDDEN_T, PACK_HIDDEN_T0, _a_fragments, _add_hidden_jobs, _bias_accumulator_order, _exact_pow2,
    _hb_perm, _hidden_image, _hidden_image_fragments, _hidden_layer_fragments, _hidden_linears, _made_pass_prefix,
    _pow2_scale, device_pack_affine_coupling, device_pack_final_layer, device_pack_made_affine,
    device_pack_resnet_hidden_backward, device_pack_resnet_hidden_forward, householder_matrix, pack_final_layer,
    pack_final_layer_general, pack_final_layer_transposed, pack_made_inverse, pack_made_inverse_context,
    pack_resnet_hidden, pack_resnet_hidden_backward, pack_resnet_hidden_wide, pack_sylvester)
from .fused_rq import (
    GENERAL_BINS, GENERAL_HIDDEN, fused_backward_supported, fused_general_supported, fused_linear_supported,
    general_hidden_width, rq_fused_linear_backward, rq_spline_fused_general, rq_spline_fused_linear)
from .affine import (
    AFFINE_ADDITIVE, AFFINE_MAF_SOFTPLUS, AFFINE_SCALE_GIVEN, AFFINE_SCALE_SOFTPLUS, AFFINE_SHIFT_TANH2,
    AFFINE_SIGMOID_PLUS2, AFFINE_SOFTPLUS_CLAMP3, _AffineFunction, _StdNormalLogProbFunction, _affine_coupling_nograd,
    _standard_normal_log_prob_nograd, affine_coupling, standard_normal_log_prob)
from .conditioner import (
    ACT_ELU, ACT_LEAKY_RELU, ACT_RELU, ACT_SIGMOID, ACT_SILU, ACT_TANH, CONTEXT_ADDITIVE, CONTEXT_GLU, HIDDEN_BWD_ROWS,
    HIDDEN_ROWS, MADE_AFFINE, MADE_RQ, WIDE_ROWS, activation_code, affine_coupling_resnet, affine_tail_activation,
    affine_tail_fits, made_inverse, made_inverse_context_fits, resnet_hidden, resnet_hidden_backward,
    resnet_hidden_packed, resnet_hidden_wide)
from .mog import (
    MOG_MAX_COMPONENTS, _MoGLogProbFunction, _mog_log_prob_nograd, _mog_operands, made_mog_sample, mog_log_prob,
    mog_log_prob_backward)
from .pointwise import (
    EW_CAUCHY_CDF, EW_EXP, EW_EXTENDED_SOFTPLUS, EW_GLU, EW_LEAKY_RELU, EW_LOGTANH, EW_SIGMOID, EW_SOFTPLUS, EW_TANH,
    _PermuteFunction, _PointwiseAffineFunction, _item_vector, _permute_nograd, batchnorm_eval, elementwise, permute,
    pointwise_affine, pointwise_affine_autograd)
from .rowwave import (
    HDH_MAX_REFLECTIONS, LINEAR_DENSE, LINEAR_DENSE_SHIFTED, LINEAR_LU_FORWARD, LINEAR_LU_INVERSE, MAX_ROW_FEATURES,
    PER_SAMPLE_DENSE, PER_SAMPLE_DENSE_T, PER_SAMPLE_LU_FORWARD, PER_SAMPLE_LU_INVERSE, SYLVESTER_MM_ROWS,
    _DenseLinearFunction, _HDHLinearFunction, _HouseholderFunction, _LULinearFunction, _PlanarFunction, _SylvesterFunction,
    _UpperLinearFunction, _hdh_operands, _householder_backward, _param, _rows, dense_linear_autograd, dense_mm, hdh_linear,
    hdh_linear_autograd, householder, householder_autograd, linear, linear_per_sample, lu_linear_autograd, planar,
    planar_autograd, sylvester, sylvester_autograd, sylvester_mm, sylvester_mm_supported, upper_linear,
    upper_linear_autograd)
from .rownorm import (
    _RadialFunction, _UnitVectorFunction, _radial_inverse_through_forward, radial, radial_autograd, unit_vector,
    unit_vector_autograd)
from .sigmoids import (
    _DeepSigmoidFunction, _SoSFunction, deep_sigmoid, deep_sigmoid_autograd, deep_sigmoid_bound, deep_sigmoid_fits,
    sum_of_sigmoids, sum_of_sigmoids_autograd)
from .splines import (
    SPLINE_CUBIC, SPLINE_LINEAR, SPLINE_QUADRATIC, _PiecewiseSplineFunction, _spline_config, piecewise_spline,
    piecewise_spline_autograd, piecewise_spline_backward_supported, spline_multiplier)
from .spd import (
    SPD_MAX_DIM, _CholeskyOuterFunction, _DiagExtractFunction, _DiagReplaceFunction, _TrilPackFunction,
    _cholesky_outer_nograd, _diag_extract_nograd, _diag_replace_nograd, _matrices, _tril_pack_nograd, cholesky,
    cholesky_outer, fill_triangular, matrix_diagonal, matrix_replace_diagonal, tril_gather)
from .image import (
    CONV1X1_MAX_CHANNELS, _Conv1x1Function, _SqueezeFunction, _conv1x1_nograd, _conv1x1_operand, _squeeze_nograd,
    conv1x1, squeeze)
from .iresnet import (
    IRES_ACT_CLIPSWISH, IRES_ACT_CSIN, IRES_ACT_ELU, IRES_ACT_LEAKY_LSWISH, IRES_ACT_LIPSWISH, IRES_ACT_RELU,
    IRES_ACT_SIN, IRES_ACT_SWISH, IRES_ACT_TANH, IRES_CONCAT_ACTS, IRES_MAX_DEPTH, IRES_MAX_DIM, IRES_MAX_WIDTH,
    _ires_operands, _pad4, iresnet_forward, iresnet_image_floats, iresnet_inverse, iresnet_supported)
from .umnn import (
    UMNN_MAX_COND, UMNN_MAX_HIDDEN_LAYERS, UMNN_MAX_STEPS, UMNN_MAX_WIDTH, UMNN_POINTS, pack_umnn, umnn, umnn_fits,
    umnn_image, umnn_image_floats)
```

flowconductor_amd/ops/conditioner.py:

```python
import torch

from flowconductor_amd import _hip
from ._core import _aligned16, _as_cols, _call, _err_word, _finish, _logabsdet_target, _prep_2d
from .rq import DEFAULT_MIN_BIN_HEIGHT, DEFAULT_MIN_BIN_WIDTH, DEFAULT_MIN_DERIVATIVE, _rq_config
from .affine import AFFINE_ADDITIVE, AFFINE_MAF_SOFTPLUS, AFFINE_SIGMOID_PLUS2, AFFINE_SOFTPLUS_CLAMP3


HIDDEN_ROWS = 16

ACT_RELU, ACT_TANH, ACT_SILU, ACT_ELU, ACT_LEAKY_RELU, ACT_SIGMOID = range(6)


def activation_code(fn):
    import torch.nn as nn
    from torch.nn import functional as F

    if isinstance(fn, nn.ReLU) or fn in (F.relu, torch.relu):
        return ACT_RELU, 0.0
    if isinstance(fn, nn.Tanh) or fn in (torch.tanh, F.tanh):
        return ACT_TANH, 0.0
    if isinstance(fn, nn.SiLU) or fn is F.silu:
        return ACT_SILU, 0.0
    if isinstance(fn, nn.ELU):
        return ACT_ELU, float(fn.alpha)
    if fn is F.elu:
        return ACT_ELU, 1.0
    if isinstance(fn, nn.LeakyReLU):
        return ACT_LEAKY_RELU, float(fn.negative_slope)
    if fn is F.leaky_relu:
        return ACT_LEAKY_RELU, 0.01
    if isinstance(fn, nn.Sigmoid) or fn in (torch.sigmoid, F.sigmoid):
        return ACT_SIGMOID, 0.0
    return None


CONTEXT_GLU, CONTEXT_ADDITIVE = 1, 2

WIDE_ROWS = 64

HIDDEN_BWD_ROWS = 128

MADE_AFFINE, MADE_RQ = 0, 1


def made_inverse_context_fits(features, num_blocks, per_dim):
    k0s = 1 if features <= 32 else 2
    pt = -(-per_dim // 16)
    image = (k0s * 8 + 2 * num_blocks * 16) * 1024 + (1 + 2 * num_blocks) * 256 + 64 + 8 * 16 * (16 * pt + 4) * 4
    context = (1 + num_blocks) * (8 * 1024 + 256) + 64
    return num_blocks <= 3 and features <= 64 and per_dim <= 48 and image + context <= 160 * 1024


def made_inverse(inputs, packed, num_blocks, per_dim, kind, rq=None, logabsdet_accum=None, context=None,
                 context_pack=None):
    lib = _hip.load()
    z = _prep_2d(inputs)
    _hip.require_no_grad(inputs)
    n, d = z.shape
    if n % HIDDEN_ROWS != 0 or d > 64:
        raise ValueError("fc_made_inverse: rows must be a multiple of %d, D <= 64" % HIDDEN_ROWS)
    if (context is None) != (context_pack is None):
        raise ValueError("made_inverse: context and context_pack go together")
    if context is not None:
        _hip.require_no_grad(context)
        if (not torch.is_tensor(context) or context.dtype != torch.float32 or context.dim() != 2 or context.shape[0] != n
                or not 1 <= context.shape[1] <= 32 or not context.is_contiguous() or context.device != z.device):
            raise ValueError("made_inverse: context must be a contiguous float32 [N, C <= 32] tensor on the inputs' device")
        if not made_inverse_context_fits(d, num_blocks, per_dim):
            raise ValueError("fc_made_inverse_context has no instantiation for D = %d, %d blocks, %d parameters per dim"
                             % (d, num_blocks, per_dim))
        cf, cu, cb = context_pack
        if cf.numel() != (1 + num_blocks) * 4096 or cu.numel() != 1 + num_blocks or cb.numel() != (1 + num_blocks) * 64:
            raise ValueError("made_inverse: context_pack does not match num_blocks = %d" % num_blocks)
    cfg = None
    if kind == MADE_RQ:
        rq = dict(rq)
        cfg = _rq_config(rq.pop("num_bins"), rq.pop("tails"), rq.pop("tail_bound", 1.0),
                         (rq.pop("left", 0.0), rq.pop("right", 1.0), rq.pop("bottom", 0.0), rq.pop("top", 1.0)),
                         rq.pop("min_bin_width", DEFAULT_MIN_BIN_WIDTH), rq.pop("min_bin_height", DEFAULT_MIN_BIN_HEIGHT),
                         rq.pop("min_derivative", DEFAULT_MIN_DERIVATIVE), rq.pop("enable_identity_init", False),
                         rq.pop("wh_divisor", 1.0), True)
        if rq:
            raise TypeError("made_inverse: unknown spline arguments %s" % sorted(rq))
    y = torch.empty_like(z)
    lad, flags = _logabsdet_target(logabsdet_accum, n, z.device)
    if flags:
        if cfg is None:
            cfg = _hip.RQConfig()
        cfg.flags = flags
    err = _err_word(z.device, True)
    hf, hu, hb, ff, fu, fb, need = packed
    if need.dtype != torch.int32 or need.numel() != d:
        raise ValueError("made_inverse: units_needed must hold one int32 per dim")
    if context is not None:
        _call("fc_made_inverse_context", lib.fc_made_inverse_context, z.device, _hip.ptr(z), _hip.ptr(context), _hip.ptr(y),
              _hip.ptr(lad), _hip.ptr(hf), _hip.ptr(hu), _hip.ptr(hb), _hip.ptr(cf), _hip.ptr(cu), _hip.ptr(cb), _hip.ptr(ff),
              _hip.ptr(fu), _hip.ptr(fb), _hip.ptr(need), _hip.ptr(err), n, d, context.shape[1], num_blocks, per_dim, kind, cfg,
              _hip.stream_ptr(z.device))
        _finish(True)
        return y, lad
    _call("fc_made_inverse", lib.fc_made_inverse, z.device, _hip.ptr(z), _hip.ptr(y), _hip.ptr(lad), _hip.ptr(hf),
          _hip.ptr(hu), _hip.ptr(hb), _hip.ptr(ff), _hip.ptr(fu), _hip.ptr(fb), _hip.ptr(need), _hip.ptr(err), n, d, num_blocks, per_dim,
          kind, cfg, _hip.stream_ptr(z.device))
    _finish(True)
    return y, lad


def affine_tail_fits(in_features, num_blocks, d):
    k0s = 1 if in_features <= 32 else 2
    layers = 2 + 2 * num_blocks
    image = (k0s * 8 + (2 * num_blocks + 1) * 16) * 1024 + layers * 64 * 4 + 64 + 32 * k0s * 4 + 512
    return d <= 128 and num_blocks <= 3 and image + 16 + 8 * 16 * (d | 1) * 4 <= 160 * 1024


def affine_tail_activation(code):
    return code in (AFFINE_SIGMOID_PLUS2, AFFINE_SOFTPLUS_CLAMP3, AFFINE_ADDITIVE, AFFINE_MAF_SOFTPLUS)


def affine_coupling_resnet(inputs, id_cols, tr_cols, packed, in_features, num_blocks, activation, inverse=False,
                           logabsdet_accum=None):
    lib = _hip.load()
    x = _prep_2d(inputs, align16=True)
    _hip.require_no_grad(inputs)
    n, d = x.shape
    if n % HIDDEN_ROWS != 0 or not affine_tail_activation(activation):
        raise ValueError("fc_affine_coupling_resnet: unsupported rows / activation")
    w_frag, w_un, bias_acc = packed
    ids, cols = _as_cols(id_cols, x.device), _as_cols(tr_cols, x.device)
    y = torch.empty_like(x)
    lad, accumulate = _logabsdet_target(logabsdet_accum, n, x.device)
    _call("fc_affine_coupling_resnet", lib.fc_affine_coupling_resnet, x.device, _hip.ptr(x), _hip.ptr(y), _hip.ptr(ids),
          _hip.ptr(cols), _hip.ptr(w_frag), _hip.ptr(w_un), _hip.ptr(bias_acc), _hip.ptr(lad), n, d, in_features,
          cols.numel(), 64, num_blocks, int(activation), 1 if inverse else 0, accumulate, _hip.stream_ptr(x.device))
    return y, lad


def resnet_hidden_packed(inputs, id_cols, packed, in_features, num_blocks, activation=(ACT_RELU, 0.0)):
    lib = _hip.load()
    x = _prep_2d(inputs)
    _hip.require_no_grad(inputs)
    n, d = x.shape
    if n % HIDDEN_ROWS != 0:
        raise ValueError("fc_resnet_hidden needs a multiple of %d rows" % HIDDEN_ROWS)
    w_frag, w_un, bias_acc = packed
    k0s = 1 if in_features <= 32 else 2
    if w_frag.numel() != (k0s + 4 * num_blocks) * 4096 or w_un.numel() != 1 + 2 * num_blocks:
        raise ValueError("weight image does not match in_features = %d, num_blocks = %d" % (in_features, num_blocks))
    ids = _as_cols(id_cols, x.device)
    h = torch.empty(n, 64, dtype=torch.float32, device=x.device)
    _call("fc_resnet_hidden", lib.fc_resnet_hidden_packed, x.device, _hip.ptr(x), _hip.ptr(h), _hip.ptr(ids),
          _hip.ptr(w_frag), _hip.ptr(w_un), _hip.ptr(bias_acc), n, d, in_features, 64, num_blocks, int(activation[0]),
          float(activation[1]), _hip.stream_ptr(x.device))
    return h


def resnet_hidden_backward(inputs, grad_hidden, id_cols, packed, in_features, num_blocks, grad_inputs_accum=None):
    lib = _hip.load()
    x = _prep_2d(inputs.detach())
    gh = _aligned16(_hip.dev_f32(grad_hidden, "grad_hidden"))
    n, d = x.shape
    if n % HIDDEN_BWD_ROWS != 0 or gh.shape != (n, 64) or not 0 <= num_blocks <= 2:
        raise ValueError("fc_resnet_hidden_backward: unsupported shapes")
    w_frag, wt_frag, w_un, bias_acc, k0s = packed
    ids = _as_cols(id_cols, x.device)
    layers = 1 + 2 * num_blocks
    if grad_inputs_accum is not None and (grad_inputs_accum.shape != x.shape or not grad_inputs_accum.is_contiguous()
                                          or grad_inputs_accum.dtype != torch.float32):
        raise ValueError("grad_inputs_accum must be a contiguous float32 [N, D] tensor")
    gxid = None if grad_inputs_accum is not None else torch.empty(n, 32 * k0s, dtype=torch.float32, device=x.device)
    nb2 = max(1, 2 * num_blocks)
    acc = torch.zeros(64 * 32 * k0s + nb2 * 4096 + layers * 64, dtype=torch.float32, device=x.device)
    gw0 = acc[:64 * 32 * k0s].view(64, 32 * k0s)
    gwb = acc[64 * 32 * k0s:64 * 32 * k0s + nb2 * 4096].view(nb2, 64, 64)
    gb = acc[64 * 32 * k0s + nb2 * 4096:].view(layers, 64)
    fn = lib.fc_resnet_hidden_backward if gxid is not None else lib.fc_resnet_hidden_backward_accum
    _call("fc_resnet_hidden_backward", fn, x.device, _hip.ptr(x), _hip.ptr(gh), _hip.ptr(ids),
          _hip.ptr(w_frag), _hip.ptr(wt_frag), _hip.ptr(w_un), _hip.ptr(bias_acc),
          _hip.ptr(gxid if gxid is not None else grad_inputs_accum), _hip.ptr(gw0),
          _hip.ptr(gwb), _hip.ptr(gb), n, d, in_features, 64, num_blocks, ACT_RELU, _hip.stream_ptr(x.device))
    return (None if gxid is None else gxid[:, :in_features]), gw0[:, :in_features], gwb, gb


def resnet_hidden_wide(inputs, id_cols, packed, in_features, num_blocks, width, activation=(ACT_RELU, 0.0)):
    lib = _hip.load()
    x = _prep_2d(inputs)
    _hip.require_no_grad(inputs)
    n, d = x.shape
    if n % WIDE_ROWS != 0 or width not in (128, 256):
        raise ValueError("fc_resnet_hidden_wide needs a multiple of %d rows and a width of 128 or 256" % WIDE_ROWS)
    w_frag, w_un, bias = packed
    ids = _as_cols(id_cols, x.device)
    h = torch.empty(n, width, dtype=torch.float32, device=x.device)
    _call("fc_resnet_hidden_wide", lib.fc_resnet_hidden_wide, x.device, _hip.ptr(x), _hip.ptr(h), _hip.ptr(ids),
          _hip.ptr(w_frag), _hip.ptr(w_un), _hip.ptr(bias), n, d, in_features, width, num_blocks, int(activation[0]),
          float(activation[1]), _hip.stream_ptr(x.device))
    return h


def resnet_hidden(inputs, id_cols, packed, in_features, num_blocks, context=None, activation=(ACT_RELU, 0.0),
                  context_mode=CONTEXT_GLU):
    lib = _hip.load()
    x = _prep_2d(inputs)
    _hip.require_no_grad(inputs)
    n, d = x.shape
    if n % HIDDEN_ROWS != 0:
        raise ValueError("fc_resnet_hidden needs a multiple of %d rows" % HIDDEN_ROWS)
    w0, b0, wb, bb = packed[:4]
    ids = _as_cols(id_cols, x.device)
    h = torch.empty(n, 64, dtype=torch.float32, device=x.device)
    if context is None:
        _call("fc_resnet_hidden", lib.fc_resnet_hidden, x.device, _hip.ptr(x), _hip.ptr(h), _hip.ptr(ids),
              _hip.ptr(w0), _hip.ptr(b0), _hip.ptr(wb), _hip.ptr(bb), n, d, in_features, 64, num_blocks,
              int(activation[0]), float(activation[1]), _hip.stream_ptr(x.device))
        return h
    wc, bc = packed[4:6]
    c = _prep_2d(context)
    _hip.require_no_grad(context)
    if c.shape[0] != n or w0.shape[1] != in_features + (c.shape[1] if context_mode == CONTEXT_GLU else 0):
        raise ValueError("context rows / width do not match the inputs / the initial layer")
    _call("fc_resnet_hidden_context", lib.fc_resnet_hidden_context, x.device, _hip.ptr(x), _hip.ptr(c), _hip.ptr(h),
          _hip.ptr(ids), _hip.ptr(w0), _hip.ptr(b0), _hip.ptr(wb), _hip.ptr(bb), _hip.ptr(wc), _hip.ptr(bc), n, d,
          in_features, c.shape[1], 64, num_blocks, int(context_mode), int(activation[0]), float(activation[1]),
          _hip.stream_ptr(x.device))
    return h
```

flowconductor_amd/ops/fused_rq.py:

```python
import torch

from flowconductor_amd import _hip
from ._core import _aligned16, _as_cols, _call, _err_word, _finish, _logabsdet_target, _prep_2d, rq_param_count
from .rq import DEFAULT_MIN_BIN_HEIGHT, DEFAULT_MIN_BIN_WIDTH, DEFAULT_MIN_DERIVATIVE, _rq_config
from .packing import FUSED_BINS, FUSED_DT, FUSED_HIDDEN, FUSED_ROWS


def fused_linear_supported(n, d, d_t, hidden, num_bins, tails):
    return (1 <= hidden <= FUSED_HIDDEN and 1 <= d_t <= FUSED_DT and num_bins == FUSED_BINS and tails == "linear"
            and d <= 128 and n >= FUSED_ROWS)


def rq_spline_fused_linear(inputs, hidden, w_pad, bias_pad, cols, *, num_bins, tail_bound,
                           min_bin_width=DEFAULT_MIN_BIN_WIDTH, min_bin_height=DEFAULT_MIN_BIN_HEIGHT,
                           min_derivative=DEFAULT_MIN_DERIVATIVE, wh_divisor=1.0, inverse=False,
                           logabsdet_accum=None, enable_identity_init=False):
    lib = _hip.load()
    x = _prep_2d(inputs, align16=True)
    h = _aligned16(_hip.dev_f32(hidden, "hidden"))
    _hip.require_no_grad(inputs, hidden)
    n, d = x.shape
    cols = _as_cols(cols, x.device)
    d_t = cols.numel()
    raw = w_pad.shape[0] == d_t * 23
    if (n % FUSED_ROWS != 0 or h.shape != (n, FUSED_HIDDEN) or not 1 <= d_t <= FUSED_DT
            or (not raw and w_pad.shape[0] != -(-d_t // 4) * 4 * 24) or w_pad.shape[1] != FUSED_HIDDEN
            or bias_pad.numel() != w_pad.shape[0]):
        raise ValueError("fused RQ layer: unsupported shapes %s / %s" % (tuple(x.shape), tuple(h.shape)))
    w_pad = _aligned16(_hip.dev_f32(w_pad.detach(), "weight"))
    bias_pad = _hip.dev_f32(bias_pad.detach(), "bias")
    cfg = _rq_config(num_bins, "linear", tail_bound, None, min_bin_width, min_bin_height, min_derivative,
                     enable_identity_init, wh_divisor, inverse)
    y = torch.empty_like(x)
    lad, cfg.flags = _logabsdet_target(logabsdet_accum, n, x.device)
    if raw:
        cfg.flags |= 4
    err = _err_word(x.device, True)
    _call("fc_rq_spline_fused_linear", lib.fc_rq_spline_fused_linear, x.device, _hip.ptr(x), _hip.ptr(y),
          _hip.ptr(h), _hip.ptr(w_pad), _hip.ptr(bias_pad), _hip.ptr(cols), _hip.ptr(lad), _hip.ptr(err), n, d,
          d_t, FUSED_HIDDEN, cfg, _hip.stream_ptr(x.device))
    _finish(True)
    return y, lad


GENERAL_BINS = range(4, 17)
GENERAL_HIDDEN = (64, 128, 256)


def general_hidden_width(hidden):
    for w in GENERAL_HIDDEN:
        if hidden <= w:
            return w
    return None


def fused_general_supported(n, d, d_t, hidden, num_bins, tails):
    return (general_hidden_width(hidden) is not None and 1 <= d_t <= FUSED_DT and num_bins in GENERAL_BINS
            and tails in (None, "linear") and d <= 128 and n >= FUSED_ROWS)


def rq_fused_linear_backward(inputs, hidden, grad_outputs, grad_logabsdet, packed, packed_t, cols, *, num_bins, tails,
                             tail_bound=1.0, left=0.0, right=1.0, bottom=0.0, top=1.0,
                             min_bin_width=DEFAULT_MIN_BIN_WIDTH, min_bin_height=DEFAULT_MIN_BIN_HEIGHT,
                             min_derivative=DEFAULT_MIN_DERIVATIVE, wh_divisor=1.0, enable_identity_init=False):
    lib = _hip.load()
    x = _prep_2d(inputs.detach(), align16=True)
    h = _aligned16(_hip.dev_f32(hidden.detach(), "hidden"))
    gy = _aligned16(_hip.dev_f32(grad_outputs, "grad_outputs"))
    gl = None if grad_logabsdet is None else _hip.dev_f32(grad_logabsdet, "grad_logabsdet")
    n, d = x.shape
    cols = _as_cols(cols, x.device)
    d_t = cols.numel()
    w_frag, w_un, bias_pad = packed
    if n % FUSED_ROWS != 0 or h.shape != (n, 64) or not 1 <= d_t <= FUSED_DT:
        raise ValueError("fused RQ layer backward: unsupported shapes %s / %s" % (tuple(x.shape), tuple(h.shape)))
    cfg = _rq_config(num_bins, tails, tail_bound, (left, right, bottom, top), min_bin_width, min_bin_height,
                     min_derivative, enable_identity_init, wh_divisor, False)
    p = rq_param_count(num_bins, tails)
    pp = bias_pad.shape[-1]
    groups = bias_pad.shape[0]
    gx = torch.empty_like(x)
    gh = torch.empty(n, 64, dtype=torch.float32, device=x.device)
    acc = torch.zeros(groups * 4 * pp * 65, dtype=torch.float32, device=x.device)
    gb = acc[:groups * 4 * pp].view(groups, 4, pp)
    gw = acc[groups * 4 * pp:].view(groups, 4, pp, 64)
    args = (_hip.ptr(x), _hip.ptr(h), _hip.ptr(gy), _hip.ptr(gl), _hip.ptr(w_frag), _hip.ptr(w_un),
            _hip.ptr(bias_pad), _hip.ptr(packed_t), _hip.ptr(cols), _hip.ptr(gx), _hip.ptr(gh), _hip.ptr(gb),
            _hip.ptr(gw), n, d, d_t, cfg, _hip.stream_ptr(x.device))
    _call("fc_rq_fused_linear_backward", lib.fc_rq_fused_linear_backward, x.device, 3, *args)
    grad_w = gw.reshape(groups * 4, pp, 64)[:d_t, :p].reshape(d_t * p, 64)
    grad_b = gb.reshape(groups * 4, pp)[:d_t, :p].reshape(d_t * p)
    return gx, gh, grad_w, grad_b


def fused_backward_supported(n, d, d_t, hidden, num_bins, tails):
    if tails not in (None, "linear") or num_bins not in GENERAL_BINS or hidden > 64:
        return False
    p = rq_param_count(num_bins, tails)
    return p <= 32 and 1 <= d_t <= FUSED_DT and d <= 128 and n >= FUSED_ROWS


def rq_spline_fused_general(inputs, hidden, w_frag, w_unscale, bias_pad, cols, *, num_bins, tails, tail_bound=1.0,
                            left=0.0, right=1.0, bottom=0.0, top=1.0, min_bin_width=DEFAULT_MIN_BIN_WIDTH,
                            min_bin_height=DEFAULT_MIN_BIN_HEIGHT, min_derivative=DEFAULT_MIN_DERIVATIVE,
                            wh_divisor=1.0, inverse=False, logabsdet_accum=None, enable_identity_init=False,
                            streamed_weights=False):
    lib = _hip.load()
    x = _prep_2d(inputs, align16=True)
    h = _aligned16(_hip.dev_f32(hidden, "hidden"))
    _hip.require_no_grad(inputs, hidden)
    n, d = x.shape
    cols = _as_cols(cols, x.device)
    d_t = cols.numel()
    hw = h.shape[1]
    if (n % FUSED_ROWS != 0 or h.shape[0] != n or hw not in GENERAL_HIDDEN or not 1 <= d_t <= FUSED_DT
            or w_frag.shape[0] != -(-d_t // 4) or w_frag.shape[1] != hw // 32):
        raise ValueError("general fused RQ layer: unsupported shapes %s / %s" % (tuple(x.shape), tuple(h.shape)))
    cfg = _rq_config(num_bins, tails, tail_bound, (left, right, bottom, top), min_bin_width, min_bin_height,
                     min_derivative, enable_identity_init, wh_divisor, inverse)
    y = torch.empty_like(x)
    lad, cfg.flags = _logabsdet_target(logabsdet_accum, n, x.device)
    if streamed_weights:
        cfg.flags |= 8
    err = _err_word(x.device, True)
    _call("fc_rq_spline_fused_general", lib.fc_rq_spline_fused_general, x.device, _hip.ptr(x), _hip.ptr(y),
          _hip.ptr(h), _hip.ptr(w_frag), _hip.ptr(w_unscale), _hip.ptr(bias_pad), _hip.ptr(cols), _hip.ptr(lad),
          _hip.ptr(err), n, d, d_t, hw, cfg, _hip.stream_ptr(x.device))
    _finish(True)
    return y, lad
```

flowconductor_amd/options.py:

```python
import contextlib

__all__ = ["get", "override", "snapshot"]

_DEFAULTS = {
    "fused_final_layer": True,
    "fused_hidden": True,
    "sylvester_mm": True,
    "ar_incremental": "auto",
    "ar_device_loop": True,
    "rq_force_tile": False,
    "fused_training": True,
    "paranoid_caches": False,
}

_values = dict(_DEFAULTS)


def get(name):
    return _values[name]


def snapshot():
    return dict(_values)


@contextlib.contextmanager
def override(**kw):
    unknown = set(kw) - set(_DEFAULTS)
    if unknown:
        raise KeyError("unknown option(s): %s" % ", ".join(sorted(unknown)))
    saved = {k: _values[k] for k in kw}
    _values.update(kw)
    try:
        yield
    finally:
        _values.update(saved)
```

flowconductor_amd/transforms/coupling.py:

```python
import warnings

import numpy as np
import torch

from flowconductor_amd import ops, options
from flowconductor_amd.transforms import fused_rq
from flowconductor_amd.transforms.base import Transform
from flowconductor_amd.transforms.UMNN import MonotonicNormalizer


def _is_plain_resnet(net):
    from flowconductor_amd.nn.nets.resnet import ResidualNet

    return (isinstance(net, ResidualNet) and type(net).forward is ResidualNet.forward
            and type(net).hidden is ResidualNet.hidden)


def _rows_from_nchw(t):
    b, c, h, w = t.shape
    return t.permute(0, 2, 3, 1).reshape(b * h * w, c), (b, c, h, w)


def _nchw_from_rows(rows, shape):
    b, c, h, w = shape
    return rows.reshape(b, h, w, c).permute(0, 3, 1, 2).contiguous()


class CouplingTransform(Transform):

    def __init__(self, mask, transform_net_create_fn, unconditional_transform=None):
        mask = torch.as_tensor(mask)
        if mask.dim() != 1:
            raise ValueError("Mask must be a 1-dim tensor.")
        if mask.numel() <= 0:
            raise ValueError("Mask can't be empty.")

        super().__init__()
        self.features = len(mask)
        features_vector = torch.arange(self.features)
        self.register_buffer("identity_features", features_vector.masked_select(mask <= 0))
        self.register_buffer("transform_features", features_vector.masked_select(mask > 0))
        assert self.num_identity_features + self.num_transform_features == self.features

        self.transform_net = transform_net_create_fn(
            self.num_identity_features,
            self.num_transform_features * self._transform_dim_multiplier(),
        )
        if unconditional_transform is None:
            self.unconditional_transform = None
        else:
            self.unconditional_transform = unconditional_transform(features=self.num_identity_features)

    @property
    def num_identity_features(self):
        return len(self.identity_features)

    @property
    def num_transform_features(self):
        return len(self.transform_features)

    def _cols(self, device):
        return ops.memo(self, "cols", (self.num_transform_features, device),
                        lambda: self.transform_features.to(device=device, dtype=torch.int32).contiguous())

    def _id_cols(self, device):
        return ops.memo(self, "id_cols", (self.num_identity_features, device),
                        lambda: self.identity_features.to(device=device, dtype=torch.int32).contiguous())

    def _check(self, inputs):
        if inputs.dim() not in [2, 4]:
            raise ValueError("Inputs must be a 2D or a 4D tensor.")
        if inputs.shape[1] != self.features:
            raise ValueError("Expected features = {}, got {}.".format(self.features, inputs.shape[1]))

    def _run(self, inputs, context, inverse):
        self._check(inputs)
        identity_split = logabsdet_identity = None
        if self.unconditional_transform is not None:
            identity_split = inputs[:, self.identity_features, ...]
            if inverse:
                identity_split, logabsdet_identity = self.unconditional_transform.inverse(identity_split, context)

        transform_params = self._conditioner(inputs, identity_split, context)

        if inputs.dim() == 4:
            rows, shape = _rows_from_nchw(inputs)
            prows = self._param_rows_nchw(transform_params, shape)
            out_rows, lad_rows = self._coupling_kernel(rows, prows, inverse)
            outputs = _nchw_from_rows(out_rows, shape)
            logabsdet = lad_rows.reshape(shape[0], -1).sum(dim=1)
        else:
            outputs, logabsdet = self._coupling_kernel(inputs, transform_params, inverse)

        if self.unconditional_transform is not None:
            if not inverse:
                identity_split, logabsdet_identity = self.unconditional_transform(identity_split, context)
            outputs[:, self.identity_features, ...] = identity_split
            logabsdet = logabsdet + logabsdet_identity
        return outputs, logabsdet

    def _conditioner(self, inputs, identity_split, context):
        net = self.transform_net
        n = inputs.shape[0]
        if (_is_plain_resnet(net) and not ops.has_hooks(net) and self.unconditional_transform is None
                and inputs.dim() == 2 and inputs.is_cuda and inputs.dtype == torch.float32 and n >= ops.HIDDEN_ROWS
                and options.get("fused_hidden")
                and net.hip_hidden_supported(inputs.shape[1], context)
                and not (torch.is_grad_enabled()
                         and (inputs.requires_grad or any(p.requires_grad for p in net.parameters())))):
            body = n - n % ops.HIDDEN_ROWS
            hidden = net.hidden_hip(inputs[:body], self._id_cols(inputs.device),
                                    None if context is None else context[:body])
            if body < n:
                hidden = torch.cat((hidden, net.hidden_padded(inputs[body:, self.identity_features],
                                                              None if context is None else context[body:])))
            return net.final_from_padded(hidden)
        if identity_split is None:
            identity_split = inputs[:, self.identity_features, ...]
        return net(identity_split, context)

    def forward(self, inputs, context=None):
        return self._run(inputs, context, inverse=False)

    def inverse(self, inputs, context=None):
        return self._run(inputs, context, inverse=True)

    def _transform_dim_multiplier(self):
        raise NotImplementedError()

    def _coupling_kernel(self, inputs, transform_params, inverse):
        raise NotImplementedError()

    def _param_rows_nchw(self, transform_params, shape):
        raise NotImplementedError()


class UMNNCouplingTransform(CouplingTransform):

    def __init__(self, mask, transform_net_create_fn, integrand_net_layers=[50, 50, 50], cond_size=20, nb_steps=20,
                 solver="CCParallel", apply_unconditional_transform=False):
        if apply_unconditional_transform:
            def unconditional_transform(features):
                return MonotonicNormalizer(integrand_net_layers, 0, nb_steps, solver)
        else:
            unconditional_transform = None
        self.cond_size = cond_size
        super().__init__(mask, transform_net_create_fn, unconditional_transform=unconditional_transform)
        self.transformer = MonotonicNormalizer(integrand_net_layers, cond_size, nb_steps, solver)

    def _transform_dim_multiplier(self):
        return self.cond_size

    def _coupling_kernel(self, inputs, transform_params, inverse):
        split = inputs[:, self.transform_features]
        out, logabsdet = self.transformer.apply_with_logabsdet(
            split, transform_params.reshape(split.shape[0], split.shape[1], -1), inverse=inverse)
        outputs = inputs.clone()
        outputs[:, self.transform_features] = out
        return outputs, logabsdet

    def _run(self, inputs, context, inverse):
        if inputs.dim() != 4 or self.unconditional_transform is not None:
            return super()._run(inputs, context, inverse)
        self._check(inputs)
        transform_params = self._conditioner(inputs, None, context)
        rows, shape = _rows_from_nchw(inputs[:, self.transform_features])
        h = transform_params.permute(0, 2, 3, 1).reshape(rows.shape[0], 1, transform_params.shape[1])
        out_rows, lad_rows = self.transformer.apply_with_logabsdet(rows, h, inverse=inverse)
        outputs = inputs.clone()
        outputs[:, self.transform_features] = _nchw_from_rows(out_rows, shape)
        return outputs, lad_rows.reshape(shape[0], -1).sum(dim=1)


class AffineCouplingTransform(CouplingTransform):

    DEFAULT_SCALE_ACTIVATION = lambda x: torch.sigmoid(x + 2) + 1e-3
    GENERAL_SCALE_ACTIVATION = lambda x: (torch.nn.functional.softplus(x) + 1e-3).clamp(0, 3)

    def __init__(self, mask, transform_net_create_fn, unconditional_transform=None,
                 scale_activation=DEFAULT_SCALE_ACTIVATION):
        self.scale_activation = scale_activation
        super().__init__(mask, transform_net_create_fn, unconditional_transform)

    def _transform_dim_multiplier(self):
        return 2

    def _activation_code(self):
        if self.scale_activation is AffineCouplingTransform.DEFAULT_SCALE_ACTIVATION:
            return ops.AFFINE_SIGMOID_PLUS2
        if self.scale_activation is AffineCouplingTransform.GENERAL_SCALE_ACTIVATION:
            return ops.AFFINE_SOFTPLUS_CLAMP3
        return ops.AFFINE_SCALE_GIVEN

    def _coupling_kernel(self, inputs, transform_params, inverse, total=None):
        code = self._activation_code()
        if code == ops.AFFINE_SCALE_GIVEN:
            d_t = self.num_transform_features
            scale = self.scale_activation(transform_params[:, d_t:])
            transform_params = torch.cat((transform_params[:, :d_t], scale), dim=1)
        return ops.affine_coupling(inputs, transform_params, self._cols(inputs.device),
                                   activation=code, inverse=inverse, logabsdet_accum=total)

    def _one_kernel_ok(self, inputs, context):
        net = self.transform_net
        if not (context is None and inputs.dim() == 2 and inputs.is_cuda and inputs.dtype == torch.float32
                and inputs.shape[0] >= ops.HIDDEN_ROWS and options.get("fused_hidden") and options.get("fused_final_layer")):
            return False

        def structure_ok():
            return (self.unconditional_transform is None and self.num_transform_features <= 32
                    and ops.affine_tail_activation(self._activation_code()) and _is_plain_resnet(net)
                    and ops.affine_tail_fits(net.initial_layer.in_features, len(net.blocks), inputs.shape[1])
                    and net.hip_hidden_supported(inputs.shape[1], None)
                    and all(ops.activation_code(b.activation)[0] == ops.ACT_RELU for b in net.blocks))

        return (ops.static_memo(self, "static_ok", (inputs.shape[1], id(self.unconditional_transform)) + ops.structure_key(net),
                                structure_ok)
                and not ops.has_hooks(net)
                and not (torch.is_grad_enabled()
                         and (inputs.requires_grad or any(p.requires_grad for p in net.parameters()))))

    def _one_kernel(self, inputs, inverse, total):
        net = self.transform_net
        pack, image = ops.device_plan(self, "tail_image", net._storage_key(), lambda: ops.device_pack_affine_coupling(
            net, self.num_transform_features, self._activation_code() == ops.AFFINE_ADDITIVE))
        pack.refresh()
        n = inputs.shape[0]
        body = n - n % ops.HIDDEN_ROWS
        dev = inputs.device
        args = (self._id_cols(dev), self._cols(dev), image, net.initial_layer.in_features, len(net.blocks),
                self._activation_code())
        if body == n:
            return ops.affine_coupling_resnet(inputs, *args, inverse=inverse, logabsdet_accum=total)
        out_a, lad_a = ops.affine_coupling_resnet(inputs[:body], *args, inverse=inverse,
                                                  logabsdet_accum=None if total is None else total[:body])
        rest = inputs[body:].contiguous()
        params = net(rest[:, self.identity_features], None)
        out_b, lad_b = self._coupling_kernel(rest, params, inverse)
        outputs = torch.cat((out_a, out_b))
        if total is None:
            return outputs, torch.cat((lad_a, lad_b))
        total[body:] += lad_b
        return outputs, total

    def _run(self, inputs, context, inverse):
        if self._one_kernel_ok(inputs, context):
            self._check(inputs)
            return self._one_kernel(inputs, inverse, None)
        return super()._run(inputs, context, inverse)

    def _apply_accumulate(self, inputs, context, inverse, total):
        if inputs.dim() != 2 or self.unconditional_transform is not None or not inputs.is_cuda:
            outputs, logabsdet = self._run(inputs, context, inverse)
            total += logabsdet
            return outputs
        self._check(inputs)
        if self._one_kernel_ok(inputs, context):
            outputs, _ = self._one_kernel(inputs, inverse, total)
            return outputs
        transform_params = self._conditioner(inputs, None, context)
        outputs, _ = self._coupling_kernel(inputs, transform_params, inverse, total=total)
        return outputs

    def _param_rows_nchw(self, transform_params, shape):
        return _rows_from_nchw(transform_params)[0]


class AdditiveCouplingTransform(AffineCouplingTransform):

    def _transform_dim_multiplier(self):
        return 1

    def _activation_code(self):
        return ops.AFFINE_ADDITIVE

    def _coupling_kernel(self, inputs, transform_params, inverse, total=None):
        return ops.affine_coupling(inputs, transform_params, self._cols(inputs.device),
                                   activation=ops.AFFINE_ADDITIVE, inverse=inverse)


class PiecewiseCouplingTransform(CouplingTransform):

    def _param_rows_nchw(self, transform_params, shape):
        b, _, h, w = shape
        c = self.num_transform_features
        p = transform_params.reshape(b, c, -1, h, w).permute(0, 3, 4, 1, 2)
        return p.reshape(b * h * w, -1)

    def _wh_divisor(self):
        raise NotImplementedError()


def _softmax_divisor(net, warn):
    if hasattr(net, "hidden_features"):
        return float(np.sqrt(net.hidden_features))
    if hasattr(net, "hidden_channels"):
        return float(np.sqrt(net.hidden_channels))
    if warn:
        warnings.warn("Inputs to the softmax are not scaled down: initialization might be bad.")
    return 1.0


class PiecewiseRationalQuadraticCouplingTransform(PiecewiseCouplingTransform):

    def __init__(self, mask, transform_net_create_fn, num_bins=10, tails=None, tail_bound=1.0,
                 apply_unconditional_transform=False, img_shape=None,
                 min_bin_width=ops.DEFAULT_MIN_BIN_WIDTH, min_bin_height=ops.DEFAULT_MIN_BIN_HEIGHT,
                 min_derivative=ops.DEFAULT_MIN_DERIVATIVE):
        self.num_bins = num_bins
        self.min_bin_width = min_bin_width
        self.min_bin_height = min_bin_height
        self.min_derivative = min_derivative
        self.tails = tails
        self.tail_bound = tail_bound

        if apply_unconditional_transform:
            from flowconductor_amd.transforms.nonlinearities import PiecewiseRationalQuadraticCDF

            def unconditional_transform(features):
                return PiecewiseRationalQuadraticCDF(
                    shape=[features] + (img_shape if img_shape else []), num_bins=num_bins,
                    tails=tails, tail_bound=tail_bound, min_bin_width=min_bin_width,
                    min_bin_height=min_bin_height, min_derivative=min_derivative)
        else:
            unconditional_transform = None
        super().__init__(mask, transform_net_create_fn, unconditional_transform=unconditional_transform)

    def _transform_dim_multiplier(self):
        return ops.rq_param_count(self.num_bins, self.tails)

    def _coupling_kernel(self, inputs, transform_params, inverse):
        return ops.rq_spline_autograd(
            inputs, transform_params, self._cols(inputs.device), num_bins=self.num_bins,
            tails=self.tails, tail_bound=self.tail_bound, min_bin_width=self.min_bin_width,
            min_bin_height=self.min_bin_height, min_derivative=self.min_derivative,
            wh_divisor=_softmax_divisor(self.transform_net, warn=True), inverse=inverse)


    def _fused_mode(self, inputs):
        net = self.transform_net
        if torch.is_grad_enabled() and (inputs.requires_grad or any(p.requires_grad for p in net.parameters())):
            return None
        if not (options.get("fused_final_layer") and _is_plain_resnet(net) and not ops.has_hooks(net)
                and inputs.dim() == 2 and inputs.is_cuda and inputs.dtype == torch.float32):
            return None
        n, d = inputs.shape
        return fused_rq.fused_mode(n, d, min(self.num_transform_features, ops.FUSED_DT), net.hidden_features, self.num_bins,
                                   self.tails, net.hidden_features)

    def _fused_ok(self, inputs):
        return self._fused_mode(inputs) is not None

    def _chunk_spec(self, device):
        per_dim = self._transform_dim_multiplier()
        cols = self._cols(device)
        spec = []
        for lo in range(0, self.num_transform_features, ops.FUSED_DT):
            hi = min(lo + ops.FUSED_DT, self.num_transform_features)
            spec.append((slice(lo * per_dim, hi * per_dim), cols[lo:hi].contiguous()))
        return spec

    def _pack_spec(self):
        lin = self.transform_net.final_layer
        return lin.weight, ops.general_hidden_width(lin.in_features), self._chunk_spec(lin.weight.device)

    def _train_chunks(self, device):
        net = self.transform_net
        lin = net.final_layer
        hidden_pack = None
        if getattr(net, "hip_hidden_backward_supported", None) is not None and net.hip_hidden_backward_supported():
            hidden_pack = net.hidden_backward_plan()[0]

        def build():
            pack, chunks = ops.device_pack_final_layer(lin.weight.detach(), lin.bias.detach(), self.num_bins, self.tails,
                                                       self._chunk_spec(device))
            if hidden_pack is not None:
                pack.merge(hidden_pack)
            return pack, chunks, lin.weight, hidden_pack

        where = (id(lin.weight), lin.weight.data_ptr(), lin.bias.data_ptr(), device, id(hidden_pack))
        plan = ops.device_plan(self, "train_pack", where, build)
        plan[0].refresh()
        return plan[1]

    def _apply_accumulate(self, inputs, context, inverse, total):
        if (self._fused_mode(inputs) is None or self.unconditional_transform is not None
                or self._fused_training_ok(inputs, context, inverse)):
            outputs, logabsdet = self._run(inputs, context, inverse)
            total += logabsdet
            return outputs
        outputs, _ = self._run(inputs, context, inverse, total=total)
        return outputs

    def _fused_kw(self, net):
        return dict(num_bins=self.num_bins, tail_bound=self.tail_bound, min_bin_width=self.min_bin_width,
                    min_bin_height=self.min_bin_height, min_derivative=self.min_derivative,
                    wh_divisor=_softmax_divisor(net, warn=False))

    def _fused_forward_kw(self, net, mode, inverse):
        kw = self._fused_kw(net)
        kw["inverse"] = inverse
        if mode == "general":
            kw["tails"] = self.tails
        return kw

    def _hidden_for_fused(self, inputs, identity_split, context, width):
        net = self.transform_net
        n = inputs.shape[0]

        def on_torch(rows_identity, ctx):
            h = net.hidden(rows_identity, ctx)
            return h if h.shape[1] == width else torch.nn.functional.pad(h, (0, width - h.shape[1]))

        body16 = n - n % ops.HIDDEN_ROWS
        if (identity_split is None and width == 64 and body16 > 0 and options.get("fused_hidden")
                and net.hip_hidden_supported(inputs.shape[1], context)):
            hidden = net.hidden_hip(inputs[:body16], self._id_cols(inputs.device),
                                    None if context is None else context[:body16])
            if body16 < n:
                hidden = torch.cat((hidden, on_torch(inputs[body16:, self.identity_features],
                                                     None if context is None else context[body16:])))
            return hidden
        body64 = n - n % ops.WIDE_ROWS
        if (identity_split is None and width > 64 and body64 > 0 and options.get("fused_hidden")
                and net.hip_hidden_wide_supported(inputs.shape[1], context)):
            hidden = net.hidden_hip_wide(inputs[:body64], self._id_cols(inputs.device))
            if body64 < n:
                hidden = torch.cat((hidden, on_torch(inputs[body64:, self.identity_features], None)))
            return hidden
        if identity_split is None:
            identity_split = inputs[:, self.identity_features]
        return on_torch(identity_split, context)

    def _fused_training_ok(self, inputs, context, inverse):
        net = self.transform_net
        return (not inverse and context is None and self.unconditional_transform is None
                and options.get("fused_training") and options.get("fused_final_layer") and options.get("fused_hidden")
                and torch.is_grad_enabled() and _is_plain_resnet(net) and not ops.has_hooks(net)
                and inputs.dim() == 2 and inputs.is_cuda and inputs.dtype == torch.float32
                and (inputs.requires_grad or any(p.requires_grad for p in net.parameters()))
                and net.hip_hidden_supported(inputs.shape[1], None)
                and ops.fused_backward_supported(inputs.shape[0], inputs.shape[1],
                                                 min(self.num_transform_features, ops.FUSED_DT), net.hidden_features,
                                                 self.num_bins, self.tails))

    def _run(self, inputs, context, inverse, total=None):
        if self._fused_training_ok(inputs, context, inverse):
            self._check(inputs)
            outputs, logabsdet = _FusedRQCouplingFunction.apply(self, inputs, *self.transform_net.parameters())
            if total is not None:
                total += logabsdet
                logabsdet = total
            return outputs, logabsdet
        mode = self._fused_mode(inputs)
        if mode is None:
            return super()._run(inputs, context, inverse)
        self._check(inputs)
        net = self.transform_net
        identity_split = logabsdet_identity = None
        if self.unconditional_transform is not None:
            identity_split = inputs[:, self.identity_features]
            if inverse:
                identity_split, logabsdet_identity = self.unconditional_transform.inverse(identity_split, context)
        width = 64 if mode == "k8" else ops.general_hidden_width(net.hidden_features)
        hidden = self._hidden_for_fused(inputs, identity_split, context, width)
        chunks = fused_rq.packed_chunks(self, net.final_layer, mode, self.num_bins, self.tails, self._pack_spec)
        kw = self._fused_forward_kw(net, mode, inverse)

        def leftover(rows, h):
            lin = net.final_layer
            params = torch.nn.functional.linear(h[:, :lin.in_features], lin.weight, lin.bias)
            return self._coupling_kernel(rows, params, inverse)

        outputs, logabsdet = fused_rq.apply(inputs, hidden, chunks, mode, kw, total, leftover)
        if self.unconditional_transform is not None:
            if not inverse:
                identity_split, logabsdet_identity = self.unconditional_transform(identity_split, context)
            outputs[:, self.identity_features] = identity_split
            logabsdet = logabsdet + logabsdet_identity
        return outputs, logabsdet


class _FusedRQCouplingFunction(torch.autograd.Function):

    @staticmethod
    def forward(ctx, layer, inputs, *net_params):
        net = layer.transform_net
        n = inputs.shape[0]
        with torch.no_grad():
            x = inputs.detach()
            pad = (-n) % ops.HIDDEN_BWD_ROWS
            if pad:
                x = torch.cat((x, x.new_zeros(pad, x.shape[1])))
            hidden = layer._hidden_for_fused(x, None, None, 64)
            k8 = net.hidden_features == ops.FUSED_HIDDEN and ops.fused_linear_supported(
                x.shape[0], x.shape[1], min(layer.num_transform_features, ops.FUSED_DT), net.hidden_features,
                layer.num_bins, layer.tails)
            lin = net.final_layer
            if k8:
                chunks = [(lin.weight[rows_slice], lin.bias[rows_slice], cols)
                          for _, _, _, _, cols, rows_slice in layer._train_chunks(x.device)]
            else:
                chunks = [(w_frag, w_un, bias_pad, cols) for w_frag, w_un, bias_pad, _, cols, _ in layer._train_chunks(x.device)]
            mode = "k8" if k8 else "general"
            rows, lad = fused_rq.run_chunks(x, hidden, chunks, mode, layer._fused_forward_kw(net, mode, False))
        ctx.layer, ctx.n = layer, n
        ctx.save_for_backward(x, hidden, *net_params)
        ctx.param_ids = [id(p) for p in net_params]
        return rows[:n], lad[:n]

    @staticmethod
    @torch.autograd.function.once_differentiable
    def backward(ctx, grad_outputs, grad_logabsdet):
        layer, n = ctx.layer, ctx.n
        net = layer.transform_net
        x, hidden = ctx.saved_tensors[:2]
        rows_total = x.shape[0]
        gy = torch.zeros_like(x) if grad_outputs is None else grad_outputs
        gl = grad_logabsdet
        if rows_total != n:
            gy = torch.cat((gy, gy.new_zeros(rows_total - n, gy.shape[1])))
            gl = None if gl is None else torch.cat((gl, gl.new_zeros(rows_total - n)))
        kw = layer._fused_kw(net)
        lin = net.final_layer
        chunks = layer._train_chunks(x.device)
        grad_w = grad_b = gh = None
        g = gy.contiguous()
        for w_frag, w_un, bias_pad, wt_frag, cols, rows_slice in chunks:
            g, gh_c, gw_c, gb_c = ops.rq_fused_linear_backward(x, hidden, g, gl, (w_frag, w_un, bias_pad), wt_frag, cols,
                                                               tails=layer.tails, **kw)
            gh = gh_c if gh is None else gh + gh_c
            if len(chunks) == 1:
                grad_w, grad_b = gw_c[:, :lin.in_features], gb_c
            else:
                if grad_w is None:
                    grad_w, grad_b = torch.zeros_like(lin.weight), torch.zeros_like(lin.bias)
                grad_w[rows_slice] = gw_c[:, :lin.in_features]
                grad_b[rows_slice] = gb_c
        by_id = {id(lin.weight): grad_w, id(lin.bias): grad_b}
        if net.hip_hidden_backward_supported():
            _, gw0, gwb, gb = ops.resnet_hidden_backward(x, gh, layer._id_cols(x.device), net.hidden_backward_packed(),
                                                         net.initial_layer.in_features, len(net.blocks), grad_inputs_accum=g)
            hf = net.hidden_features
            by_id[id(net.initial_layer.weight)] = gw0[:hf]
            by_id[id(net.initial_layer.bias)] = gb[0, :hf]
            for bi, block in enumerate(net.blocks):
                for li, l2 in enumerate(block.linear_layers):
                    by_id[id(l2.weight)] = gwb[2 * bi + li, :hf, :hf]
                    by_id[id(l2.bias)] = gb[1 + 2 * bi + li, :hf]
            return (None, g[:n]) + tuple(by_id.get(pid) for pid in ctx.param_ids)
        hidden_params = [p for p in net.parameters() if p is not lin.weight and p is not lin.bias]
        with torch.enable_grad():
            xid = x[:, layer.identity_features].detach().requires_grad_(True)
            h2 = net.hidden(xid)
            wanted = [xid] + [p for p in hidden_params if p.requires_grad]
            got = torch.autograd.grad(h2, wanted, gh[:, :h2.shape[1]], allow_unused=True)
        g[:, layer.identity_features] += got[0]
        for p, gp_ in zip(wanted[1:], got[1:]):
            by_id[id(p)] = gp_
        grads = tuple(by_id.get(pid) for pid in ctx.param_ids)
        return (None, g[:n]) + grads


def _divisor_if_hidden_features(net):
    return float(np.sqrt(net.hidden_features)) if hasattr(net, "hidden_features") else 1.0


class PiecewiseLinearCouplingTransform(PiecewiseCouplingTransform):

    def __init__(self, mask, transform_net_create_fn, num_bins=10, tails=None, tail_bound=1.0,
                 apply_unconditional_transform=False, img_shape=None):
        self.num_bins = num_bins
        self.tails = tails
        self.tail_bound = tail_bound
        if apply_unconditional_transform:
            from flowconductor_amd.transforms.nonlinearities import PiecewiseLinearCDF

            def unconditional_transform(features):
                return PiecewiseLinearCDF(shape=[features] + (img_shape if img_shape else []), num_bins=num_bins,
                                          tails=tails, tail_bound=tail_bound)
        else:
            unconditional_transform = None
        super().__init__(mask, transform_net_create_fn, unconditional_transform=unconditional_transform)

    def _transform_dim_multiplier(self):
        return self.num_bins

    def _coupling_kernel(self, inputs, transform_params, inverse):
        return ops.piecewise_spline_autograd(inputs, transform_params, self._cols(inputs.device), kind=ops.SPLINE_LINEAR,
                                    num_bins=self.num_bins, tails=self.tails, tail_bound=self.tail_bound,
                                    inverse=inverse)


class PiecewiseQuadraticCouplingTransform(PiecewiseCouplingTransform):

    def __init__(self, mask, transform_net_create_fn, num_bins=10, tails=None, tail_bound=1.0,
                 apply_unconditional_transform=False, img_shape=None, min_bin_width=ops.DEFAULT_MIN_BIN_WIDTH,
                 min_bin_height=ops.DEFAULT_MIN_BIN_HEIGHT):
        self.num_bins = num_bins
        self.tails = tails
        self.tail_bound = tail_bound
        self.min_bin_width = min_bin_width
        self.min_bin_height = min_bin_height
        if apply_unconditional_transform:
            from flowconductor_amd.transforms.nonlinearities import PiecewiseQuadraticCDF

            def unconditional_transform(features):
                return PiecewiseQuadraticCDF(shape=[features] + (img_shape if img_shape else []),
                                             num_bins=num_bins, tails=tails, tail_bound=tail_bound,
                                             min_bin_width=min_bin_width, min_bin_height=min_bin_height)
        else:
            unconditional_transform = None
        super().__init__(mask, transform_net_create_fn, unconditional_transform=unconditional_transform)

    def _transform_dim_multiplier(self):
        return ops.spline_multiplier(ops.SPLINE_QUADRATIC, self.num_bins, self.tails)

    def _coupling_kernel(self, inputs, transform_params, inverse):
        div = _divisor_if_hidden_features(self.transform_net)
        return ops.piecewise_spline_autograd(inputs, transform_params, self._cols(inputs.device),
                                    kind=ops.SPLINE_QUADRATIC, num_bins=self.num_bins, tails=self.tails,
                                    tail_bound=self.tail_bound, min_bin_width=self.min_bin_width,
                                    min_bin_height=self.min_bin_height, width_divisor=div, height_divisor=div,
                                    inverse=inverse)


class PiecewiseCubicCouplingTransform(PiecewiseCouplingTransform):

    def __init__(self, mask, transform_net_create_fn, num_bins=10, tails=None, tail_bound=1.0,
                 apply_unconditional_transform=False, img_shape=None, min_bin_width=ops.DEFAULT_MIN_BIN_WIDTH,
                 min_bin_height=ops.DEFAULT_MIN_BIN_HEIGHT):
        self.num_bins = num_bins
        self.min_bin_width = min_bin_width
        self.min_bin_height = min_bin_height
        self.tails = tails
        self.tail_bound = tail_bound
        if apply_unconditional_transform:
            from flowconductor_amd.transforms.nonlinearities import PiecewiseCubicCDF

            def unconditional_transform(features):
                return PiecewiseCubicCDF(shape=[features] + (img_shape if img_shape else []), num_bins=num_bins,
                                         tails=tails, tail_bound=tail_bound, min_bin_width=min_bin_width,
                                         min_bin_height=min_bin_height)
        else:
            unconditional_transform = None
        super().__init__(mask, transform_net_create_fn, unconditional_transform=unconditional_transform)

    def _transform_dim_multiplier(self):
        return self.num_bins * 2 + 2

    def _coupling_kernel(self, inputs, transform_params, inverse):
        div = _divisor_if_hidden_features(self.transform_net)
        return ops.piecewise_spline_autograd(inputs, transform_params, self._cols(inputs.device), kind=ops.SPLINE_CUBIC,
                                    num_bins=self.num_bins, tails=self.tails, tail_bound=self.tail_bound,
                                    min_bin_width=self.min_bin_width, min_bin_height=self.min_bin_height,
                                    width_divisor=div, height_divisor=div, inverse=inverse)
```

flowconductor_amd/transforms/fused_rq.py:

```python
import torch

from flowconductor_amd import ops


def fused_mode(n, d, d_t, hidden, num_bins, tails, general_hidden):
    if ops.fused_linear_supported(n, d, d_t, hidden, num_bins, tails):
        return "k8"
    if general_hidden is not None and ops.fused_general_supported(n, d, d_t, general_hidden, num_bins, tails):
        return "general"
    return None


def packed_chunks(owner, lin, mode, num_bins, tails, spec):
    by_mode = ops.memo(owner, "packed", ops.cache_key(lin.weight, lin.bias), dict)
    packed = by_mode.get(mode)
    if packed is None:
        weight, hidden_pad, groups = spec()
        packed = []
        for rows, cols in groups:
            if mode == "k8":
                images = ops.pack_final_layer(weight[rows], lin.bias[rows], num_bins)
            else:
                images = ops.pack_final_layer_general(weight[rows], lin.bias[rows], num_bins, tails, hidden_pad)
            packed.append(tuple(images) + (cols,))
        by_mode[mode] = packed
    return packed


def run_chunks(inputs, hidden, chunks, mode, kw, logabsdet_accum=None):
    fn = ops.rq_spline_fused_linear if mode == "k8" else ops.rq_spline_fused_general
    rows, lad = inputs, logabsdet_accum
    for chunk in chunks:
        rows, lad = fn(rows, hidden, *chunk, logabsdet_accum=lad, **kw)
    return rows, lad


def apply(inputs, hidden, chunks, mode, kw, total, leftover_fn):
    n = inputs.shape[0]
    body = n - n % ops.FUSED_ROWS
    if body == n:
        if len(chunks) == 1:
            fn = ops.rq_spline_fused_linear if mode == "k8" else ops.rq_spline_fused_general
            return fn(inputs, hidden, *chunks[0], logabsdet_accum=total, **kw)
        return run_chunks(inputs, hidden, chunks, mode, kw, total)
    out_a, lad_a = run_chunks(inputs[:body], hidden[:body], chunks, mode, kw, None if total is None else total[:body])
    out_b, lad_b = leftover_fn(inputs[body:].contiguous(), hidden[body:])
    outputs = torch.cat((out_a, out_b))
    if total is None:
        return outputs, torch.cat((lad_a, lad_b))
    total[body:] += lad_b
    return outputs, total
```

include/flowcon_hip.h:

```cpp
#ifndef FLOWCON_HIP_H_
#define FLOWCON_HIP_H_

#include <stdint.h>

#ifdef __cplusplus
extern "C" {
#endif

#define FC_ERR_OUTSIDE_DOMAIN 1u
#define FC_ERR_DISCRIMINANT 2u
#define FC_ERR_NONFINITE 4u
#define FC_ERR_NOT_LOWER_TRIANGULAR 8u
#define FC_ERR_DIAGONAL_NONPOSITIVE 16u
#define FC_ERR_NOT_SYMMETRIC 32u
#define FC_ERR_NOT_POSITIVE_DEFINITE 64u
#define FC_ERR_CHOLESKY_FAILED 128u

#define FC_ABI_VERSION 3

int fc_abi_version(void);

#define FC_RQ_ACCUMULATE_LOGABSDET 1
#define FC_RQ_FORCE_TILE 2
#define FC_RQ_RAW_WEIGHTS 4
#define FC_RQ_STREAMED_WEIGHTS 8

typedef struct fc_rq_config {
  int32_t num_bins;
  int32_t tails;
  int32_t inverse;
  int32_t flags;
  float left, right, bottom, top;
  double min_bin_width, min_bin_height, min_derivative;
  float wh_divisor;
  float softplus_beta;
  float tail_constant;
  float reserved2;
} fc_rq_config;

int fc_rq_spline(const float* x, float* y, const float* params, const int32_t* cols,
                 float* logabsdet, uint32_t* err_flag, int64_t n, int32_t d, int32_t d_t,
                 int32_t shared_params, int32_t lad_mode, const fc_rq_config* cfg, void* stream);

int fc_rq_spline_fused_linear(const float* x, float* y, const float* h, const float* w_pad,
                              const float* bias_pad, const int32_t* cols, float* logabsdet,
                              uint32_t* err_flag, int64_t n, int32_t d, int32_t d_t, int32_t hidden,
                              const fc_rq_config* cfg, void* stream);

int fc_rq_spline_fused_general(const float* x, float* y, const float* h, const void* w_frag,
                               const float* w_unscale, const float* bias_pad, const int32_t* cols,
                               float* logabsdet, uint32_t* err_flag, int64_t n, int32_t d, int32_t d_t,
                               int32_t hidden, const fc_rq_config* cfg, void* stream);

#define FC_RQ_BACKWARD_ONE_LAUNCH 3
int fc_rq_fused_linear_backward(int32_t role, const float* x, const float* h, const float* grad_y,
                                const float* grad_logabsdet, const void* w_frag, const float* w_unscale,
                                const float* bias_pad, const void* wt_frag, const int32_t* cols, float* grad_x,
                                float* grad_h, float* grad_bias_pad, float* grad_w_pad, int64_t n, int32_t d,
                                int32_t d_t, const fc_rq_config* cfg, void* stream);

#define FC_MADE_AFFINE 0
#define FC_MADE_RQ 1
int fc_made_inverse(const float* z, float* y, float* logabsdet, const void* hidden_frag, const float* hidden_unscale,
                    const float* hidden_bias, const void* final_frag, const float* final_unscale, const float* final_bias,
                    const int32_t* units_needed, uint32_t* err_flag, int64_t n, int32_t d, int32_t num_blocks, int32_t params_per_dim, int32_t kind,
                    const fc_rq_config* cfg, void* stream);

int fc_made_inverse_context(const float* z, const float* context, float* y, float* logabsdet, const void* hidden_frag,
                            const float* hidden_unscale, const float* hidden_bias, const void* context_frag,
                            const float* context_unscale, const float* context_bias, const void* final_frag,
                            const float* final_unscale, const float* final_bias, const int32_t* units_needed,
                            uint32_t* err_flag, int64_t n, int32_t d, int32_t context_features, int32_t num_blocks,
                            int32_t params_per_dim, int32_t kind, const fc_rq_config* cfg, void* stream);

int fc_mog_log_prob(const float* x, const float* params, float* logp, int64_t n, int32_t d, int32_t c, float epsilon,
                    int32_t flags, void* stream);

int fc_mog_log_prob_backward(const float* grad_logp, const float* x, const float* params, float* grad_x, float* grad_params,
                             int64_t n, int32_t d, int32_t c, float epsilon, void* stream);

#define FC_MADE_MOG 2
int fc_made_mog_sample(const float* normal, const float* uniform, float* x, float* logp, const void* hidden_frag,
                       const float* hidden_unscale, const float* hidden_bias, const void* final_frag, const float* final_unscale,
                       const float* final_bias, const int32_t* units_needed, int64_t n, int32_t d, int32_t num_blocks, int32_t c,
                       float epsilon, void* stream);

int fc_made_mog_sample_context(const float* normal, const float* uniform, const float* context, float* x, float* logp,
                               const void* hidden_frag, const float* hidden_unscale, const float* hidden_bias,
                               const void* context_frag, const float* context_unscale, const float* context_bias,
                               const void* final_frag, const float* final_unscale, const float* final_bias,
                               const int32_t* units_needed, int64_t n, int32_t d, int32_t context_features, int32_t num_blocks,
                               int32_t c, float epsilon, void* stream);

int fc_affine_backward(const float* x, const float* params, const int32_t* cols, const float* grad_y,
                       const float* grad_logabsdet, float* grad_x, float* grad_params, int64_t n,
                       int32_t d, int32_t d_t, int32_t activation, void* stream);

int fc_rq_spline_backward(const float* x, const float* params, const int32_t* cols, const float* grad_y,
                          const float* grad_logabsdet, float* grad_x, float* grad_params, int64_t n,
                          int32_t d, int32_t d_t, const fc_rq_config* cfg, void* stream);

#define FC_ACT_RELU 0
#define FC_ACT_TANH 1
#define FC_ACT_SILU 2
#define FC_ACT_ELU 3
#define FC_ACT_LEAKY_RELU 4
#define FC_ACT_SIGMOID 5
int fc_resnet_hidden(const float* x, float* h, const int32_t* id_cols, const float* w0,
                     const float* b0, const float* wb, const float* bb, int64_t n, int32_t d,
                     int32_t in_features, int32_t hidden, int32_t num_blocks, int32_t activation,
                     float activation_param, void* stream);

int fc_resnet_hidden_packed(const float* x, float* h, const int32_t* id_cols, const void* w_frag,
                            const float* w_unscale, const float* bias_acc, int64_t n, int32_t d,
                            int32_t in_features, int32_t hidden, int32_t num_blocks, int32_t activation,
                            float activation_param, void* stream);

int fc_affine_coupling_resnet(const float* x, float* y, const int32_t* id_cols, const int32_t* tr_cols,
                              const void* w_frag, const float* w_unscale, const float* bias_acc, float* logabsdet,
                              int64_t n, int32_t d, int32_t in_features, int32_t d_t, int32_t hidden, int32_t num_blocks,
                              int32_t scale_activation, int32_t inverse, int32_t accumulate, void* stream);

int fc_resnet_hidden_backward(const float* x, const float* grad_h, const int32_t* id_cols, const void* w_frag,
                              const void* wt_frag, const float* w_unscale, const float* bias_acc, float* grad_x_id,
                              float* grad_w0, float* grad_wb, float* grad_b, int64_t n, int32_t d, int32_t in_features,
                              int32_t hidden, int32_t num_blocks, int32_t activation, void* stream);

int fc_resnet_hidden_backward_accum(const float* x, const float* grad_h, const int32_t* id_cols, const void* w_frag,
                                    const void* wt_frag, const float* w_unscale, const float* bias_acc, float* grad_x_full,
                                    float* grad_w0, float* grad_wb, float* grad_b, int64_t n, int32_t d, int32_t in_features,
                                    int32_t hidden, int32_t num_blocks, int32_t activation, void* stream);

int fc_resnet_hidden_wide(const float* x, float* h, const int32_t* id_cols, const void* w_frag,
                          const float* w_unscale, const float* bias, int64_t n, int32_t d, int32_t in_features,
                          int32_t hidden, int32_t num_blocks, int32_t activation, float activation_param,
                          void* stream);

#define FC_CONTEXT_GLU 1
#define FC_CONTEXT_ADDITIVE 2
int fc_resnet_hidden_context(const float* x, const float* context, float* h, const int32_t* id_cols,
                             const float* w0, const float* b0, const float* wb, const float* bb,
                             const float* wc, const float* bc, int64_t n, int32_t d, int32_t in_features,
                             int32_t context_features, int32_t hidden, int32_t num_blocks, int32_t context_mode,
                             int32_t activation, float activation_param, void* stream);

#define FC_SPLINE_LINEAR 0
#define FC_SPLINE_QUADRATIC 1
#define FC_SPLINE_CUBIC 2

typedef struct fc_spline_config {
  int32_t kind;
  int32_t num_bins;
  int32_t tails;
  int32_t inverse;
  float left, right, bottom, top;
  double min_bin_width, min_bin_height;
  float width_divisor, height_divisor;
  float cubic_eps;
  float cubic_quadratic_threshold;
} fc_spline_config;

int fc_piecewise_spline(const float* x, float* y, const float* params, const int32_t* cols,
                        float* logabsdet, uint32_t* err_flag, int64_t n, int32_t d, int32_t d_t,
                        int32_t shared_params, int32_t lad_mode, const fc_spline_config* cfg,
                        void* stream);

int fc_piecewise_spline_backward(const float* x, const float* params, const int32_t* cols, const float* grad_y,
                                 const float* grad_logabsdet, float* grad_x, float* grad_params, int64_t n,
                                 int32_t d, int32_t d_t, const fc_spline_config* cfg, void* stream);

#define FC_AFFINE_SIGMOID_PLUS2 0
#define FC_AFFINE_SOFTPLUS_CLAMP3 1
#define FC_AFFINE_SCALE_GIVEN 2
#define FC_AFFINE_ADDITIVE 3
#define FC_AFFINE_MAF_SOFTPLUS 4

#define FC_AFFINE_SHIFT_TANH2 5

#define FC_AFFINE_SCALE_SOFTPLUS 6

int fc_affine(const float* x, float* y, const float* params, const int32_t* cols,
              float* logabsdet, int64_t n, int32_t d, int32_t d_t, int32_t activation,
              int32_t inverse, int32_t shared_params, int32_t lad_mode, void* stream);

int fc_standard_normal_log_prob(const float* z, const float* add, float* out, int64_t n,
                                int32_t d, float log_z, void* stream);

int fc_permute(const float* x, float* y, const int32_t* perm, int64_t outer, int32_t d,
               int64_t inner, void* stream);

#define FC_SPD_MAX_DIM 128
int fc_tril_pack(const float* x, float* y, int64_t batch, int32_t m, int32_t mode, void* stream);
int fc_matrix_diag(const float* x, float* diag, float* y, int64_t batch, int32_t m, int32_t mode, void* stream);
int fc_cholesky_outer(const float* L, float* y, float* logabsdet, uint32_t* err_flag, int64_t batch, int32_t m,
                      int32_t checkargs, void* stream);
int fc_cholesky_outer_backward(const float* L, const float* grad_outputs, const float* grad_logabsdet,
                               float* grad_inputs, int64_t batch, int32_t m, void* stream);
int fc_cholesky(const float* A, float* L, float* logabsdet, uint32_t* err_flag, int64_t batch, int32_t m, float eps,
                int32_t checkargs, void* stream);

#define FC_CONV1X1_MAX_CHANNELS 128
int fc_squeeze(const float* x, float* y, int64_t planes, int32_t h, int32_t w, int32_t factor, int32_t mode,
               void* stream);
int fc_conv1x1(const float* x, const float* weight, const float* pre, const float* post, float* y, int64_t batch,
               int32_t c, int64_t hw, void* stream);

#define FC_IRES_MAX_DIM 16
#define FC_IRES_MAX_DEPTH 4
#define FC_IRES_MAX_WIDTH 128
#define FC_IRES_ACT_RELU 0
#define FC_IRES_ACT_TANH 1
#define FC_IRES_ACT_ELU 2
#define FC_IRES_ACT_SWISH 3
#define FC_IRES_ACT_LIPSWISH 4
#define FC_IRES_ACT_CLIPSWISH 5
#define FC_IRES_ACT_SIN 6
#define FC_IRES_ACT_CSIN 7
#define FC_IRES_ACT_LEAKY_LSWISH 8
int fc_iresnet_forward(const float* x, const float* extra, const float* scale, const float* image, float* y,
                       float* logabsdet, int64_t n, int32_t d, int32_t e, int32_t depth, int32_t growth,
                       int32_t activation, int32_t image_floats, void* stream);
int fc_iresnet_inverse(const float* y, const float* extra, const float* scale, const float* image, float* x,
                       uint32_t* max_iters, int64_t n, int32_t d, int32_t e, int32_t depth, int32_t growth,
                       int32_t activation, int32_t image_floats, int32_t max_iterations, float atol, float rtol,
                       void* stream);

int fc_pointwise_affine(const float* x, float* y, const float* scale, const float* shift,
                        const float* aux_mean, const float* aux_weight, int64_t n, int64_t m,
                        int32_t scale_len, int32_t shift_len, int32_t mode, void* stream);

#define FC_EW_EXP 0
#define FC_EW_TANH 1
#define FC_EW_LOGTANH 2
#define FC_EW_LEAKY_RELU 3
#define FC_EW_SIGMOID 4
#define FC_EW_SOFTPLUS 5
#define FC_EW_CAUCHY_CDF 6
#define FC_EW_EXTENDED_SOFTPLUS 7
#define FC_EW_GLU 8

int fc_elementwise(const float* x, float* y, float* logabsdet_row, float* logabsdet_elem,
                   const float* aux, uint32_t* err_flag, int64_t n, int64_t m, int32_t kind,
                   int32_t inverse, float p0, float p1, float p2, float p3, void* stream);

int fc_sum_of_sigmoids(const float* x, float* y, const float* params, const int32_t* cols,
                       float* logabsdet, uint32_t* err_flag, int64_t n, int32_t d, int32_t d_t,
                       int32_t n_sigmoids, int32_t inverse, int32_t bisection_iterations,
                       float bisection_lim, float offset, float log_scale_postact,
                       int32_t shared_params, int32_t lad_mode, void* stream);

int fc_sum_of_sigmoids_backward(const float* x, const float* params, const float* grad_y,
                                const float* grad_logabsdet, float* grad_x, float* grad_params, int64_t n, int32_t d,
                                int32_t n_sigmoids, float log_scale_postact, void* stream);

int fc_deep_sigmoid(const float* x, float* y, const float* params, const int32_t* cols, float* logabsdet,
                    uint32_t* err_flag, int64_t n, int32_t d, int32_t d_t, int32_t n_sigmoids, int32_t inverse,
                    int32_t inverse_iterations, float inverse_lim, float mollify, float eps, float prescale,
                    int32_t shared_params, int32_t lad_mode, void* stream);

int fc_deep_sigmoid_backward(const float* x, const float* raw, const float* grad_y, const float* grad_logabsdet,
                             float* grad_x, float* grad_raw, int64_t n, int32_t d, int32_t n_sigmoids, float mollify,
                             float eps, float prescale, int32_t shared_params, void* stream);

int fc_deep_sigmoid_backward_rows(int64_t n, int32_t d, int32_t n_sigmoids);

#define FC_UMNN_MAX_COND 31
#define FC_UMNN_MAX_HIDDEN_LAYERS 3
#define FC_UMNN_MAX_STEPS 63
#define FC_UMNN_POINTS 68
int fc_umnn(const float* x, const float* h, const void* w_frag, const float* aux, float* y, float* jac,
            float* logabsdet, int64_t n, int32_t d, int32_t cond_size, int32_t hidden_layers, int32_t nb_steps,
            int32_t inverse, int32_t lad_mode, void* stream);

int fc_householder(const float* x, float* y, const float* q, int64_t n, int32_t d,
                   int32_t num_transforms, int32_t per_sample, int32_t reverse, void* stream);

int fc_planar(const float* x, float* y, float* logabsdet, const float* w, const float* u_hat,
              const float* b, int64_t n, int32_t d, int32_t per_sample, void* stream);

int fc_planar_backward(const float* x, const float* grad_y, const float* grad_logabsdet, const float* w,
                       const float* u_hat, const float* b, float* grad_x, float* grad_w, float* grad_u_hat,
                       float* grad_b, int64_t n, int32_t d, void* stream);

int fc_householder_backward(const float* y, const float* grad_y, const float* q, float* grad_x, float* grad_q,
                            int64_t n, int32_t d, int32_t num_transforms, int32_t reverse, void* stream);

int fc_hdh_linear(const float* x, float* y, const float* q_a, const float* q_b, const float* scale, const float* pre,
                  const float* post, int64_t n, int32_t d, int32_t ka, int32_t kb, int32_t reverse_a, int32_t reverse_b,
                  void* stream);

int fc_hdh_linear_backward(const float* y, const float* grad_y, const float* q_a, const float* q_b, const float* scale,
                           const float* post, float* grad_x, float* grad_q_a, float* grad_q_b, float* grad_scale,
                           float* grad_pre, float* grad_post, int64_t n, int32_t d, int32_t ka, int32_t kb,
                           int32_t reverse_a, int32_t reverse_b, void* stream);

int fc_radial(const float* x, float* y, float* logabsdet, const float* z0, const float* a, const float* b, int64_t n,
              int32_t d, int32_t inverse, void* stream);

int fc_radial_backward(const float* x, const float* grad_y, const float* grad_logabsdet, const float* z0, const float* a,
                       const float* b, float* grad_x, float* grad_z0, float* grad_a, float* grad_b, int64_t n, int32_t d,
                       void* stream);

int fc_unit_vector(const float* x, float* y, float* logabsdet, uint32_t* err_flag, int64_t n, int32_t d, int32_t inverse,
                   void* stream);

int fc_unit_vector_backward(const float* x_or_y, const float* grad_out, const float* grad_logabsdet, float* grad_in,
                            int64_t n, int32_t d, int32_t inverse, void* stream);

int fc_sylvester_mid_backward(const float* pre, float* grad_act_inout, const float* grad_logabsdet,
                              const float* r_diag_prod, float* grad_bias, float* grad_r_diag_prod, int64_t n, int32_t d,
                              void* stream);

int fc_linear(const float* x, float* y, const float* a_t, const float* b_t, const float* bias,
              int64_t n, int32_t d, int32_t mode, void* stream);

int fc_linear_per_sample(const float* x, float* y, float* logabsdet, const float* m, int64_t n,
                         int32_t d, int32_t mode, float offdiag_scale, float eps, void* stream);

int fc_sylvester(const float* x, float* y, float* logabsdet, const float* q, const float* r1_t,
                 const float* r2_t, const float* bias, const float* r_diag_prod, int64_t n, int32_t d,
                 int32_t num_householder, int32_t per_sample, void* stream);

int fc_sylvester_mm(const float* x, float* y, float* logabsdet, const float* w1, const float* w2,
                    const float* bias, const float* r_diag_prod, int64_t n, int32_t d, void* stream);

int fc_dense_mm(const float* x, float* y, const float* w, const float* bias, int64_t n, int32_t d, void* stream);

int fc_dense_mm_shifted(const float* x, float* y, const float* w, const float* pre, const float* post, int64_t n,
                        int32_t d, void* stream);

#define FC_PACK_FINAL 0
#define FC_PACK_FINAL_T 1
#define FC_PACK_HIDDEN 2
#define FC_PACK_HIDDEN_T 3
#define FC_PACK_HIDDEN_T0 4
typedef struct fc_pack_job {
  const float* w;
  const float* b;
  void* frag;
  float* unscale;
  float* bias_out;
  int32_t rows, cols;
  int32_t mode;
  int32_t p, pp;
  int32_t nks, nt;
  int32_t group;
} fc_pack_job;
int fc_pack_fragments(const void* jobs, int32_t num_jobs, void* stream);
int fc_pack_job_bytes(void);

#define FC_COMM_UNIQUE_ID_BYTES 128
int fc_comm_unique_id(void* id_out128);
int fc_comm_init_rank(void** comm_out, int32_t nranks, const void* id128, int32_t rank);
int fc_comm_init_rank_on_device(void** comm_out, int32_t nranks, const void* id128, int32_t rank, int32_t device);
int fc_comm_destroy(void* comm);
int fc_comm_abort(void* comm);
int fc_allreduce_loglik(double* sum_count, void* comm, void* stream);

#ifdef __cplusplus
}
#endif
#endif
```

Baseline: 56.10 million.

## Hand hidden activations to fused RQ kernel as pre-split fp16 pieces

The ResNet hidden kernel can now write its output as hi/lo fp16 split fragments plus a per-row unscale factor, in place of fp32 rows. The fused RQ spline kernel reads these pieces directly into its LDS hidden buffer, so it no longer has to re-split fp32 hidden values into fp16 operands itself. The coupling layer enables this by default for the k8 mode without context. It adds new kernel instantiations, extra handling for tail rows, and more Python dispatch conditions. The hand-over traffic stays about the same size (two fp16 pieces per value plus one unscale per row).

Result: faster. 56.89 million, median of 6 (+1.4%).

```diff
diff --git a/flowconductor_amd/_hip.py b/flowconductor_amd/_hip.py
--- a/flowconductor_amd/_hip.py
+++ b/flowconductor_amd/_hip.py
@@ -106,6 +106,8 @@
                             ctypes.POINTER(SplineConfig), _P],
     "fc_rq_spline_fused_linear": [_P, _P, _P, _P, _P, _P, _P, _P, _I64, _I32, _I32, _I32,
                                   ctypes.POINTER(RQConfig), _P],
+    "fc_rq_spline_fused_linear_split": [_P, _P, _P, _P, _P, _P, _P, _P, _P, _I64, _I32, _I32, _I32,
+                                        ctypes.POINTER(RQConfig), _P],
     "fc_rq_spline_fused_general": [_P, _P, _P, _P, _P, _P, _P, _P, _P, _I64, _I32, _I32, _I32,
                                    ctypes.POINTER(RQConfig), _P],
     "fc_rq_fused_linear_backward": [_I32, _P, _P, _P, _P, _P, _P, _P, _P, _P, _P, _P, _P, _P, _I64, _I32, _I32,
@@ -119,6 +121,7 @@
     "fc_made_mog_sample": [_P] * 11 + [_I64, _I32, _I32, _I32, _F, _P],
     "fc_made_mog_sample_context": [_P] * 15 + [_I64, _I32, _I32, _I32, _I32, _F, _P],
     "fc_resnet_hidden_packed": [_P, _P, _P, _P, _P, _P, _I64, _I32, _I32, _I32, _I32, _I32, ctypes.c_float, _P],
+    "fc_resnet_hidden_packed_split": [_P, _P, _P, _P, _P, _P, _P, _P, _I64, _I32, _I32, _I32, _I32, _I32, ctypes.c_float, _P],
     "fc_resnet_hidden_backward": [_P, _P, _P, _P, _P, _P, _P, _P, _P, _P, _P, _I64, _I32, _I32, _I32, _I32, _I32, _P],
     "fc_resnet_hidden_backward_accum": [_P, _P, _P, _P, _P, _P, _P, _P, _P, _P, _P, _I64, _I32, _I32, _I32, _I32, _I32, _P],
     "fc_resnet_hidden_wide": [_P, _P, _P, _P, _P, _P, _I64, _I32, _I32, _I32, _I32, _I32, ctypes.c_float, _P],
diff --git a/flowconductor_amd/csrc/fc_resnet_hidden.hip b/flowconductor_amd/csrc/fc_resnet_hidden.hip
--- a/flowconductor_amd/csrc/fc_resnet_hidden.hip
+++ b/flowconductor_amd/csrc/fc_resnet_hidden.hip
@@ -39,6 +39,8 @@
   const int32_t* tr_cols;
   float* lad;
   int d_t, affine_act, inverse, accumulate;
+  uint4* hsplit;
+  float* hun;
 };
 
 __host__ __device__ constexpr int hid_feat(int t, int g, int r) { return 32 * (t >> 1) + 8 * g + 4 * (t & 1) + r; }
@@ -58,9 +60,10 @@
   static_assert(kBytes <= 160 * 1024, "weight fragments exceed the CU's LDS");
 };
 
-template <int NB, int K0S, int kCtx, int kAct, int BPW, int kTail = 0, int XVT = 8>
+template <int NB, int K0S, int kCtx, int kAct, int BPW, int kTail = 0, int XVT = 8, bool kSplit = false>
 __global__ __launch_bounds__(512, (kCtx || BPW > 1 || kTail) ? 2 : 4) void resnet_hidden_kernel(HiddenArgs a) {
   static_assert(!kTail || kCtx == 0, "the coupling tail: no context");
+  static_assert(!kSplit || (kCtx == 0 && !kTail), "the split hand-over: plain stack only");
   using L = HiddenLds<NB, K0S, kCtx, kTail>;
   constexpr bool kPrefetchX = FC_HIDDEN_PREFETCH_X && (K0S == 1 || kCtx != 0 || BPW > 1);
   extern __shared__ __attribute__((aligned(16))) unsigned char hsmem[];
@@ -599,18 +602,29 @@
     }
     FC_EACH_BLOCK {
       const int64_t blk = grp * BPW + b;
-      if (blk < a.blocks16) {
+      if (blk < a.blocks16 && (!kSplit || a.h)) {
         float4* hrow = reinterpret_cast<float4*>(a.h + (blk * 16 + s16) * kHid);
         hrow[2 * g] = float4{h[b][0][0], h[b][0][1], h[b][0][2], h[b][0][3]};
         hrow[2 * g + 1] = float4{h[b][1][0], h[b][1][1], h[b][1][2], h[b][1][3]};
         hrow[8 + 2 * g] = float4{h[b][2][0], h[b][2][1], h[b][2][2], h[b][2][3]};
         hrow[8 + 2 * g + 1] = float4{h[b][3][0], h[b][3][1], h[b][3][2], h[b][3][3]};
       }
+      if constexpr (kSplit) {
+        const float hu = make_operand(h[b], bh[b], bl[b]);
+        if (blk < a.blocks16) {
+          uint4* srow = a.hsplit + (blk * 16 + s16) * 16;
+          srow[g] = __builtin_bit_cast(uint4, bh[b][0]);
+          srow[4 + g] = __builtin_bit_cast(uint4, bh[b][1]);
+          srow[8 + g] = __builtin_bit_cast(uint4, bl[b][0]);
+          srow[12 + g] = __builtin_bit_cast(uint4, bl[b][1]);
+          if (g == 0) a.hun[blk * 16 + s16] = hu;
+        }
+      }
     }
   }
 #ifdef FC_HID_STAMP
   if (lane == 0 && grp0 < groups) {
-    float* dst = a.h + (grp0 * BPW * 16) * kHid;
+    float* dst = (kSplit && !a.h ? reinterpret_cast<float*>(a.hsplit) : a.h) + (grp0 * BPW * 16) * kHid;
     dst[0] = (float)(__builtin_amdgcn_s_memtime() - stamp0);
     dst[1] = (float)((groups - grp0 + nwaves - 1) / nwaves * BPW);
     dst[2] = (float)(stamp0 - stamp_entry);
@@ -620,17 +634,17 @@
 #undef FC_EACH_BLOCK
 }
 
-template <int NB, int K0S, int kCtx, int kAct, int BPW, int kTail = 0, int XVT = 8>
+template <int NB, int K0S, int kCtx, int kAct, int BPW, int kTail = 0, int XVT = 8, bool kSplit = false>
 hipError_t launch_hidden(const HiddenArgs& a, int64_t grid, hipStream_t s) {
   using L = HiddenLds<NB, K0S, kCtx, kTail>;
   static PerDeviceOnce attr;
   const hipError_t ea = ensure_max_dynamic_lds(
-      attr, reinterpret_cast<const void*>(&resnet_hidden_kernel<NB, K0S, kCtx, kAct, BPW, kTail, XVT>), 160 * 1024);
+      attr, reinterpret_cast<const void*>(&resnet_hidden_kernel<NB, K0S, kCtx, kAct, BPW, kTail, XVT, kSplit>), 160 * 1024);
   if (ea != hipSuccess) return ea;
   if (kTail && a.D > 16 * XVT) return hipErrorInvalidValue;
   const size_t lds = kTail ? ((L::kBytes + 15) & ~size_t(15)) + (size_t)(kHidThreads / 64) * BPW * 16 * (a.D | 1) * 4 : L::kBytes;
   if (lds > 160 * 1024) return hipErrorInvalidConfiguration;
-  hipLaunchKernelGGL((resnet_hidden_kernel<NB, K0S, kCtx, kAct, BPW, kTail, XVT>), dim3((unsigned)grid), dim3(kHidThreads), lds,
+  hipLaunchKernelGGL((resnet_hidden_kernel<NB, K0S, kCtx, kAct, BPW, kTail, XVT, kSplit>), dim3((unsigned)grid), dim3(kHidThreads), lds,
                      s, a);
   return hipGetLastError();
 }
@@ -665,7 +679,7 @@
   }
 }
 
-template <int kCtx, int kAct>
+template <int kCtx, int kAct, bool kSplit = false>
 hipError_t dispatch_hidden(const HiddenArgs& a, int num_blocks, hipStream_t s) {
   const int cus = device_cu_count();
   const bool wide = a.k0 + (kCtx == 1 ? a.C : 0) > 32;
@@ -683,12 +697,12 @@
 #define FC_HIDDEN_CASE(NB_, K0S_)                                                            \
   do {                                                                                       \
     if constexpr (kPairs) {                                                                  \
-      if (pairs) return launch_hidden<NB_, K0S_, kCtx, kAct, 2>(a, grid, s);                 \
+      if (pairs) return launch_hidden<NB_, K0S_, kCtx, kAct, 2, 0, 8, kSplit>(a, grid, s);   \
     }                                                                                        \
-    return launch_hidden<NB_, K0S_, kCtx, kAct, 1>(a, grid, s);                              \
+    return launch_hidden<NB_, K0S_, kCtx, kAct, 1, 0, 8, kSplit>(a, grid, s);                \
   } while (0)
 #else
-#define FC_HIDDEN_CASE(NB_, K0S_) return launch_hidden<NB_, K0S_, kCtx, kAct, 1>(a, grid, s)
+#define FC_HIDDEN_CASE(NB_, K0S_) return launch_hidden<NB_, K0S_, kCtx, kAct, 1, 0, 8, kSplit>(a, grid, s)
 #endif
   switch (num_blocks * 2 + (wide ? 1 : 0)) {
     case 0: FC_HIDDEN_CASE(0, 1);
@@ -702,8 +716,10 @@
     default: break;
   }
   if constexpr (!kCtx) {
-    if (wide) FC_HIDDEN_CASE(4, 2);
-    FC_HIDDEN_CASE(4, 1);
+    if constexpr (!kSplit) {
+      if (wide) FC_HIDDEN_CASE(4, 2);
+    }
+    if (!wide) FC_HIDDEN_CASE(4, 1);
   }
 #undef FC_HIDDEN_CASE
   return hipErrorInvalidValue;
@@ -728,22 +744,44 @@
   return fc::dispatch_hidden<0, 1>(a, num_blocks, static_cast<hipStream_t>(stream));
 }
 
-extern "C" int fc_resnet_hidden_packed(const float* x, float* h, const int32_t* id_cols, const void* w_frag,
-                                       const float* w_unscale, const float* bias_acc, int64_t n, int32_t d,
-                                       int32_t in_features, int32_t hidden, int32_t num_blocks, int32_t activation,
-                                       float activation_param, void* stream) {
+static int hidden_packed(const float* x, float* h, void* h_split, float* h_unscale, const int32_t* id_cols, const void* w_frag,
+                         const float* w_unscale, const float* bias_acc, int64_t n, int32_t d, int32_t in_features,
+                         int32_t hidden, int32_t num_blocks, int32_t activation, float activation_param, void* stream) {
   if (n < 0 || d <= 0 || hidden != fc::kHid || num_blocks < 0 || num_blocks > 4) return hipErrorInvalidValue;
   if (activation < FC_ACT_RELU || activation > FC_ACT_SIGMOID) return hipErrorInvalidValue;
   if (in_features <= 0 || in_features > 64 || in_features > d) return hipErrorInvalidValue;
   if (n % 16 != 0) return hipErrorInvalidValue;
   if (n == 0) return hipSuccess;
-  if (!x || !h || !id_cols || !w_frag || !w_unscale || !bias_acc) return hipErrorInvalidValue;
-  if (((uintptr_t)h & 15u) != 0 || ((uintptr_t)w_frag & 15u) != 0) return hipErrorInvalidValue;
+  if (!x || (!h && !h_split) || !id_cols || !w_frag || !w_unscale || !bias_acc) return hipErrorInvalidValue;
+  if (h_split && !h_unscale) return hipErrorInvalidValue;
+  if ((((uintptr_t)h | (uintptr_t)h_split | (uintptr_t)w_frag) & 15u) != 0) return hipErrorInvalidValue;
   fc::HiddenArgs a{x, h, id_cols, nullptr, nullptr, nullptr, nullptr, n / 16, d, in_features, nullptr, nullptr, nullptr, 0,
                    activation, activation_param, static_cast<const fc::f16x8*>(w_frag), w_unscale, bias_acc,
-                   nullptr, nullptr, nullptr, 0, 0, 0, 0};
-  if (activation == FC_ACT_RELU) return fc::dispatch_hidden<0, 0>(a, num_blocks, static_cast<hipStream_t>(stream));
-  return fc::dispatch_hidden<0, 1>(a, num_blocks, static_cast<hipStream_t>(stream));
+                   nullptr, nullptr, nullptr, 0, 0, 0, 0, static_cast<uint4*>(h_split), h_unscale};
+  hipStream_t s = static_cast<hipStream_t>(stream);
+  if (h_split) {
+    if (activation != FC_ACT_RELU || (num_blocks == 4 && in_features > 32)) return hipErrorInvalidValue;
+    return fc::dispatch_hidden<0, 0, true>(a, num_blocks, s);
+  }
+  return activation == FC_ACT_RELU ? fc::dispatch_hidden<0, 0>(a, num_blocks, s) : fc::dispatch_hidden<0, 1>(a, num_blocks, s);
+}
+
+extern "C" int fc_resnet_hidden_packed(const float* x, float* h, const int32_t* id_cols, const void* w_frag,
+                                       const float* w_unscale, const float* bias_acc, int64_t n, int32_t d,
+                                       int32_t in_features, int32_t hidden, int32_t num_blocks, int32_t activation,
+                                       float activation_param, void* stream) {
+  if (!h) return hipErrorInvalidValue;
+  return hidden_packed(x, h, nullptr, nullptr, id_cols, w_frag, w_unscale, bias_acc, n, d, in_features, hidden, num_blocks,
+                       activation, activation_param, stream);
+}
+
+extern "C" int fc_resnet_hidden_packed_split(const float* x, float* h, void* h_split, float* h_unscale, const int32_t* id_cols,
+                                             const void* w_frag, const float* w_unscale, const float* bias_acc, int64_t n,
+                                             int32_t d, int32_t in_features, int32_t hidden, int32_t num_blocks,
+                                             int32_t activation, float activation_param, void* stream) {
+  if (!h_split) return hipErrorInvalidValue;
+  return hidden_packed(x, h, h_split, h_unscale, id_cols, w_frag, w_unscale, bias_acc, n, d, in_features, hidden, num_blocks,
+                       activation, activation_param, stream);
 }
 
 extern "C" int fc_affine_coupling_resnet(const float* x, float* y, const int32_t* id_cols, const int32_t* tr_cols,
diff --git a/flowconductor_amd/csrc/fc_rq_fused.h b/flowconductor_amd/csrc/fc_rq_fused.h
--- a/flowconductor_amd/csrc/fc_rq_fused.h
+++ b/flowconductor_amd/csrc/fc_rq_fused.h
@@ -25,6 +25,7 @@
   int accumulate;
   int dt;
   int wrows;
+  const float* h_unscale;
 };
 
 size_t fused3_lds_bytes(int d, int rows);
diff --git a/flowconductor_amd/csrc/fc_rq_fused.hip b/flowconductor_amd/csrc/fc_rq_fused.hip
--- a/flowconductor_amd/csrc/fc_rq_fused.hip
+++ b/flowconductor_amd/csrc/fc_rq_fused.hip
@@ -5,10 +5,9 @@
 #include "fc_rq_fused.h"
 #include "../../include/flowcon_hip.h"
 
-extern "C" int fc_rq_spline_fused_linear(const float* x, float* y, const float* h, const float* w_pad,
-                                         const float* bias_pad, const int32_t* cols, float* logabsdet,
-                                         uint32_t* err_flag, int64_t n, int32_t d, int32_t d_t, int32_t hidden,
-                                         const fc_rq_config* cfg, void* stream) {
+static int fused_linear(const float* x, float* y, const float* h, const float* h_unscale, const float* w_pad,
+                        const float* bias_pad, const int32_t* cols, float* logabsdet, uint32_t* err_flag, int64_t n, int32_t d,
+                        int32_t d_t, int32_t hidden, const fc_rq_config* cfg, void* stream) {
   if (!cfg || n < 0 || d < d_t) return hipErrorInvalidValue;
   if (hidden != fc::kH || d_t < 1 || d_t > fc::kDt || cfg->num_bins != fc::kK || cfg->tails != 1 ||
       d > 128)
@@ -39,14 +38,30 @@
   const bool wide_ok = fc::fused3_lds_bytes(d, 64) <= 160 * 1024;
   const int64_t n64 = wide_ok ? n - n % 64 : 0;
   if (n64 > 0) {
-    fc::FusedArgs a{x, y, h, w_pad, bias_pad, cols, logabsdet, err_flag, n64 / 64, d, acc, d_t, wrows};
+    fc::FusedArgs a{x, y, h, w_pad, bias_pad, cols, logabsdet, err_flag, n64 / 64, d, acc, d_t, wrows, h_unscale};
     const hipError_t e = fc::launch_fused3(op, a, 64, (unsigned)(cus < a.tiles ? cus : a.tiles), s);
     if (e != hipSuccess) return e;
   }
   if (n64 < n) {
     fc::FusedArgs a{x + n64 * d, y + n64 * d, h + n64 * fc::kH, w_pad, bias_pad, cols, logabsdet + n64, err_flag,
-                    (n - n64) / 32, d, acc, d_t, wrows};
+                    (n - n64) / 32, d, acc, d_t, wrows, h_unscale ? h_unscale + n64 : nullptr};
     return fc::launch_fused3(op, a, 32, (unsigned)(cus < a.tiles ? cus : a.tiles), s);
   }
   return hipSuccess;
 }
+
+extern "C" int fc_rq_spline_fused_linear(const float* x, float* y, const float* h, const float* w_pad,
+                                         const float* bias_pad, const int32_t* cols, float* logabsdet,
+                                         uint32_t* err_flag, int64_t n, int32_t d, int32_t d_t, int32_t hidden,
+                                         const fc_rq_config* cfg, void* stream) {
+  return fused_linear(x, y, h, nullptr, w_pad, bias_pad, cols, logabsdet, err_flag, n, d, d_t, hidden, cfg, stream);
+}
+
+extern "C" int fc_rq_spline_fused_linear_split(const float* x, float* y, const void* h_split, const float* h_unscale,
+                                               const float* w_pad, const float* bias_pad, const int32_t* cols,
+                                               float* logabsdet, uint32_t* err_flag, int64_t n, int32_t d, int32_t d_t,
+                                               int32_t hidden, const fc_rq_config* cfg, void* stream) {
+  if (n > 0 && !h_unscale) return hipErrorInvalidValue;
+  return fused_linear(x, y, static_cast<const float*>(h_split), h_unscale, w_pad, bias_pad, cols, logabsdet, err_flag, n, d,
+                      d_t, hidden, cfg, stream);
+}
diff --git a/flowconductor_amd/csrc/fc_rq_fused3.hip b/flowconductor_amd/csrc/fc_rq_fused3.hip
--- a/flowconductor_amd/csrc/fc_rq_fused3.hip
+++ b/flowconductor_amd/csrc/fc_rq_fused3.hip
@@ -42,9 +42,10 @@
 
 size_t fused3_lds_bytes(int d, int rows) { return rows == 64 ? Fused3Lds<64>::bytes(d) : Fused3Lds<32>::bytes(d); }
 
-template <bool kInv, int R, int XV, bool kFull, bool kPadX>
+template <bool kInv, int R, int XV, bool kFull, bool kPadX, bool kSplitH>
 __global__ __launch_bounds__(512) void rq_fused_linear_kernel3(RQOp<kK> op, FusedArgs a) {
   using L = Fused3Lds<R>;
+  static_assert(!kSplitH || (kFull && XV <= 2), "the split hand-over is instantiated for the full-dims kernels of <= 64 columns");
   constexpr int kHPiece = L::kHPiece;
   constexpr int NB = R / 16;
   constexpr int HV = R / 32;
@@ -153,6 +154,7 @@
   constexpr bool kCarry = kFull && XV <= 2;
   float4 hv0, hv1, xv0, xv1, xv2, xv3;
   hv0 = hv1 = xv0 = xv1 = xv2 = xv3 = float4{0.f, 0.f, 0.f, 0.f};
+  float hun = 1.f;
   int64_t fetched = tile0;
   auto fetch = [&](int64_t t) __attribute__((always_inline)) {
     fetched = t;
@@ -160,6 +162,7 @@
     const float4* hg = reinterpret_cast<const float4*>(a.h + t * R * kH);
     hv0 = hg[tid];
     if constexpr (HV > 1 && kFull) hv1 = hg[tid + 512];
+    if constexpr (kSplitH && kCarry) hun = a.h_unscale[t * R + (tid & (R - 1))];
     const float4* xg = reinterpret_cast<const float4*>(a.x + t * R * D);
     xv0 = xg[tid < xvec ? tid : 0];
     if constexpr (kCarry) {
@@ -174,6 +177,11 @@
     return reinterpret_cast<float4*>(xbuf + (buf * R + r) * XS + c);
   };
   auto park_h = [&](int buf, int xbuf3, int k, const float4& hvk) __attribute__((always_inline)) {
+    if constexpr (kSplitH) {
+      const int i = tid + 512 * k, row = i >> 4, c16 = i & 15;
+      *reinterpret_cast<float4*>(hbuf + ((buf * 2 + (c16 >> 3)) * R + row) * kHB + (c16 & 7) * 8) = hvk;
+      return;
+    }
     const int c = (tid & 15) * 4, r = (tid >> 4) + 32 * k;
 #if FC_ABL & 32
     {
@@ -215,6 +223,9 @@
     if constexpr (XV > 1) if (tid + 512 < xvec) *xslot(x3, tid + 512) = xv1;
     if constexpr (XV > 2) if (tid + 1024 < xvec) *xslot(x3, tid + 1024) = xv2;
     if constexpr (XV > 3) if (tid + 1536 < xvec) *xslot(x3, tid + 1536) = xv3;
+    if constexpr (kSplitH) {
+      if (tid < R) hscale[x3 * R + tid] = hun;
+    }
   };
   auto hfrag = [&](int hb, int blk, int hp, int ks) {
     return *reinterpret_cast<const f16x8*>(hbuf + ((hb * 2 + hp) * R + 16 * blk + s16) * kHB + 32 * ks + 8 * g);
@@ -407,23 +418,29 @@
 #undef FC_TIMED_BARRIER
 #undef FC_PHASE
 
-template <bool kInv, int R, int XV, bool kFull, bool kPadX>
+template <bool kInv, int R, int XV, bool kFull, bool kPadX, bool kSplitH>
 static hipError_t launch_cfg(const RQOp<kK>& op, const FusedArgs& a, unsigned grid, hipStream_t stream) {
   const size_t lds = Fused3Lds<R>::bytes(a.D);
   if (lds > 160 * 1024) return hipErrorInvalidConfiguration;
   static PerDeviceOnce attr;
   const hipError_t ea = ensure_max_dynamic_lds(
-      attr, reinterpret_cast<const void*>(&rq_fused_linear_kernel3<kInv, R, XV, kFull, kPadX>), 160 * 1024);
+      attr, reinterpret_cast<const void*>(&rq_fused_linear_kernel3<kInv, R, XV, kFull, kPadX, kSplitH>), 160 * 1024);
   if (ea != hipSuccess) return ea;
-  hipLaunchKernelGGL((rq_fused_linear_kernel3<kInv, R, XV, kFull, kPadX>), dim3(grid), dim3(512), lds, stream, op, a);
+  hipLaunchKernelGGL((rq_fused_linear_kernel3<kInv, R, XV, kFull, kPadX, kSplitH>), dim3(grid), dim3(512), lds, stream, op, a);
   return hipGetLastError();
 }
 
 template <bool kInv, int R, int XV>
 static hipError_t launch_one(const RQOp<kK>& op, const FusedArgs& a, unsigned grid, hipStream_t stream) {
-  if (a.D & 3) return launch_cfg<kInv, R, XV, false, false>(op, a, grid, stream);
-  return a.dt == kDt ? launch_cfg<kInv, R, XV, true, true>(op, a, grid, stream)
-                     : launch_cfg<kInv, R, XV, false, true>(op, a, grid, stream);
+  if (a.h_unscale) {
+    if constexpr (XV <= 2) {
+      if (!(a.D & 3) && a.dt == kDt) return launch_cfg<kInv, R, XV, true, true, true>(op, a, grid, stream);
+    }
+    return hipErrorInvalidValue;
+  }
+  if (a.D & 3) return launch_cfg<kInv, R, XV, false, false, false>(op, a, grid, stream);
+  return a.dt == kDt ? launch_cfg<kInv, R, XV, true, true, false>(op, a, grid, stream)
+                     : launch_cfg<kInv, R, XV, false, true, false>(op, a, grid, stream);
 }
 
 hipError_t launch_fused3(const RQOp<kK>& op, const FusedArgs& a, int rows, unsigned grid, hipStream_t stream) {
diff --git a/flowconductor_amd/nn/nets/resnet.py b/flowconductor_amd/nn/nets/resnet.py
--- a/flowconductor_amd/nn/nets/resnet.py
+++ b/flowconductor_amd/nn/nets/resnet.py
@@ -202,7 +202,7 @@
                           lambda: F.pad(lin.weight.detach(), (0, 64 - lin.in_features)))
         return F.linear(hidden64, weight, lin.bias)
 
-    def hidden_hip(self, rows, id_cols, context=None):
+    def hidden_hip(self, rows, id_cols, context=None, split=False, keep_rows=False):
         from flowconductor_amd import ops
 
         in_features = self.initial_layer.in_features - (self.context_features or 0)
@@ -210,11 +210,15 @@
         if context is None:
             if self.training and self.hip_hidden_backward_supported():
                 w_frag, _, w_un, bias_acc, _ = self.hidden_backward_packed()
-                return ops.resnet_hidden_packed(rows, id_cols, (w_frag, w_un, bias_acc), in_features, len(self.blocks), act)
+                return ops.resnet_hidden_packed(rows, id_cols, (w_frag, w_un, bias_acc), in_features, len(self.blocks), act,
+                                                split=split, keep_rows=keep_rows)
             pack, image = ops.device_plan(self, "hip_image", self._storage_key(),
                                           lambda: ops.device_pack_resnet_hidden_forward(self))
             pack.refresh()
-            return ops.resnet_hidden_packed(rows, id_cols, image, in_features, len(self.blocks), act)
+            return ops.resnet_hidden_packed(rows, id_cols, image, in_features, len(self.blocks), act, split=split,
+                                            keep_rows=keep_rows)
+        if split:
+            raise ValueError("hidden_hip: the split hand-over has no context form")
         packed = ops.memo(self, "hip_packed", ops.cache_key(*self._param_list()), lambda: ops.pack_resnet_hidden(self))
         return ops.resnet_hidden(rows, id_cols, packed, in_features, len(self.blocks), context, act)
 
diff --git a/flowconductor_amd/ops/__init__.py b/flowconductor_amd/ops/__init__.py
--- a/flowconductor_amd/ops/__init__.py
+++ b/flowconductor_amd/ops/__init__.py
@@ -17,7 +17,8 @@
     pack_final_layer_general, pack_final_layer_transposed, pack_made_inverse, pack_made_inverse_context,
     pack_resnet_hidden, pack_resnet_hidden_backward, pack_resnet_hidden_wide, pack_sylvester)
 from .fused_rq import (
-    GENERAL_BINS, GENERAL_HIDDEN, fused_backward_supported, fused_general_supported, fused_linear_supported,
+    GENERAL_BINS, GENERAL_HIDDEN, fused_backward_supported, fused_general_supported, fused_linear_split_supported,
+    fused_linear_supported,
     general_hidden_width, rq_fused_linear_backward, rq_spline_fused_general, rq_spline_fused_linear)
 from .affine import (
     AFFINE_ADDITIVE, AFFINE_MAF_SOFTPLUS, AFFINE_SCALE_GIVEN, AFFINE_SCALE_SOFTPLUS, AFFINE_SHIFT_TANH2,
@@ -25,9 +26,9 @@
     _standard_normal_log_prob_nograd, affine_coupling, standard_normal_log_prob)
 from .conditioner import (
     ACT_ELU, ACT_LEAKY_RELU, ACT_RELU, ACT_SIGMOID, ACT_SILU, ACT_TANH, CONTEXT_ADDITIVE, CONTEXT_GLU, HIDDEN_BWD_ROWS,
-    HIDDEN_ROWS, MADE_AFFINE, MADE_RQ, WIDE_ROWS, activation_code, affine_coupling_resnet, affine_tail_activation,
+    HIDDEN_ROWS, MADE_AFFINE, MADE_RQ, WIDE_ROWS, SplitHidden, activation_code, affine_coupling_resnet, affine_tail_activation,
     affine_tail_fits, made_inverse, made_inverse_context_fits, resnet_hidden, resnet_hidden_backward,
-    resnet_hidden_packed, resnet_hidden_wide)
+    resnet_hidden_packed, resnet_hidden_wide, split_hidden_reference, split_hidden_supported)
 from .mog import (
     MOG_MAX_COMPONENTS, _MoGLogProbFunction, _mog_log_prob_nograd, _mog_operands, made_mog_sample, mog_log_prob,
     mog_log_prob_backward)
diff --git a/flowconductor_amd/ops/conditioner.py b/flowconductor_amd/ops/conditioner.py
--- a/flowconductor_amd/ops/conditioner.py
+++ b/flowconductor_amd/ops/conditioner.py
@@ -135,7 +135,31 @@
     return y, lad
 
 
-def resnet_hidden_packed(inputs, id_cols, packed, in_features, num_blocks, activation=(ACT_RELU, 0.0)):
+class SplitHidden:
+    __slots__ = ("pieces", "unscale", "rows")
+
+    def __init__(self, pieces, unscale, rows=None):
+        self.pieces, self.unscale, self.rows = pieces, unscale, rows
+
+
+def split_hidden_reference(hidden):
+    h = hidden.detach().float().contiguous()
+    e = (h.abs().amax(dim=1).view(torch.int32) >> 23) & 255
+    ok = (e > 14) & (e < 255)
+    scale = torch.where(ok, (268 - e) << 23, torch.full_like(e, 127 << 23)).view(torch.float32)
+    unscale = torch.where(ok, (e - 14) << 23, torch.full_like(e, 127 << 23)).view(torch.float32)
+    x = h * scale[:, None]
+    hi = x.to(torch.float16)
+    lo = (x - hi.float()).to(torch.float16)
+    return SplitHidden(torch.stack((hi, lo), dim=1).contiguous(), unscale.contiguous(), h)
+
+
+def split_hidden_supported(in_features, num_blocks, activation=(ACT_RELU, 0.0)):
+    return activation[0] == ACT_RELU and not (num_blocks == 4 and in_features > 32)
+
+
+def resnet_hidden_packed(inputs, id_cols, packed, in_features, num_blocks, activation=(ACT_RELU, 0.0), split=False,
+                         keep_rows=False):
     lib = _hip.load()
     x = _prep_2d(inputs)
     _hip.require_no_grad(inputs)
@@ -147,6 +171,16 @@
     if w_frag.numel() != (k0s + 4 * num_blocks) * 4096 or w_un.numel() != 1 + 2 * num_blocks:
         raise ValueError("weight image does not match in_features = %d, num_blocks = %d" % (in_features, num_blocks))
     ids = _as_cols(id_cols, x.device)
+    if split:
+        if not split_hidden_supported(in_features, num_blocks, activation):
+            raise ValueError("fc_resnet_hidden_packed_split has no instantiation for this stack")
+        out = SplitHidden(torch.empty(n, 2, 64, dtype=torch.float16, device=x.device),
+                          torch.empty(n, dtype=torch.float32, device=x.device),
+                          torch.empty(n, 64, dtype=torch.float32, device=x.device) if keep_rows else None)
+        _call("fc_resnet_hidden", lib.fc_resnet_hidden_packed_split, x.device, _hip.ptr(x), _hip.ptr(out.rows),
+              _hip.ptr(out.pieces), _hip.ptr(out.unscale), _hip.ptr(ids), _hip.ptr(w_frag), _hip.ptr(w_un), _hip.ptr(bias_acc),
+              n, d, in_features, 64, num_blocks, int(activation[0]), float(activation[1]), _hip.stream_ptr(x.device))
+        return out
     h = torch.empty(n, 64, dtype=torch.float32, device=x.device)
     _call("fc_resnet_hidden", lib.fc_resnet_hidden_packed, x.device, _hip.ptr(x), _hip.ptr(h), _hip.ptr(ids),
           _hip.ptr(w_frag), _hip.ptr(w_un), _hip.ptr(bias_acc), n, d, in_features, 64, num_blocks, int(activation[0]),
diff --git a/flowconductor_amd/ops/fused_rq.py b/flowconductor_amd/ops/fused_rq.py
--- a/flowconductor_amd/ops/fused_rq.py
+++ b/flowconductor_amd/ops/fused_rq.py
@@ -3,6 +3,7 @@
 from flowconductor_amd import _hip
 from ._core import _aligned16, _as_cols, _call, _err_word, _finish, _logabsdet_target, _prep_2d, rq_param_count
 from .rq import DEFAULT_MIN_BIN_HEIGHT, DEFAULT_MIN_BIN_WIDTH, DEFAULT_MIN_DERIVATIVE, _rq_config
+from .conditioner import SplitHidden
 from .packing import FUSED_BINS, FUSED_DT, FUSED_HIDDEN, FUSED_ROWS
 
 
@@ -11,18 +12,33 @@
             and d <= 128 and n >= FUSED_ROWS)
 
 
+def fused_linear_split_supported(d, d_t):
+    return d_t == FUSED_DT and d % 4 == 0 and d <= 64
+
+
 def rq_spline_fused_linear(inputs, hidden, w_pad, bias_pad, cols, *, num_bins, tail_bound,
                            min_bin_width=DEFAULT_MIN_BIN_WIDTH, min_bin_height=DEFAULT_MIN_BIN_HEIGHT,
                            min_derivative=DEFAULT_MIN_DERIVATIVE, wh_divisor=1.0, inverse=False,
                            logabsdet_accum=None, enable_identity_init=False):
     lib = _hip.load()
     x = _prep_2d(inputs, align16=True)
-    h = _aligned16(_hip.dev_f32(hidden, "hidden"))
-    _hip.require_no_grad(inputs, hidden)
+    split = isinstance(hidden, SplitHidden)
+    if split:
+        h, h_un = hidden.pieces, hidden.unscale
+        if (h.dtype != torch.float16 or h_un.dtype != torch.float32 or h_un.shape != (h.shape[0],) or h.device != x.device
+                or h_un.device != x.device or not h.is_contiguous() or not h_un.is_contiguous() or h.data_ptr() % 16):
+            raise ValueError("fused RQ layer: malformed split hidden image")
+        _hip.require_no_grad(inputs)
+        h = h.view(h.shape[0], -1).view(torch.float32)
+    else:
+        h = _aligned16(_hip.dev_f32(hidden, "hidden"))
+        _hip.require_no_grad(inputs, hidden)
     n, d = x.shape
     cols = _as_cols(cols, x.device)
     d_t = cols.numel()
     raw = w_pad.shape[0] == d_t * 23
+    if split and not fused_linear_split_supported(d, d_t):
+        raise ValueError("fused RQ layer: no split hand-over for D = %d, d_t = %d" % (d, d_t))
     if (n % FUSED_ROWS != 0 or h.shape != (n, FUSED_HIDDEN) or not 1 <= d_t <= FUSED_DT
             or (not raw and w_pad.shape[0] != -(-d_t // 4) * 4 * 24) or w_pad.shape[1] != FUSED_HIDDEN
             or bias_pad.numel() != w_pad.shape[0]):
@@ -36,6 +52,12 @@
     if raw:
         cfg.flags |= 4
     err = _err_word(x.device, True)
+    if split:
+        _call("fc_rq_spline_fused_linear", lib.fc_rq_spline_fused_linear_split, x.device, _hip.ptr(x), _hip.ptr(y),
+              _hip.ptr(h), _hip.ptr(h_un), _hip.ptr(w_pad), _hip.ptr(bias_pad), _hip.ptr(cols), _hip.ptr(lad), _hip.ptr(err),
+              n, d, d_t, FUSED_HIDDEN, cfg, _hip.stream_ptr(x.device))
+        _finish(True)
+        return y, lad
     _call("fc_rq_spline_fused_linear", lib.fc_rq_spline_fused_linear, x.device, _hip.ptr(x), _hip.ptr(y),
           _hip.ptr(h), _hip.ptr(w_pad), _hip.ptr(bias_pad), _hip.ptr(cols), _hip.ptr(lad), _hip.ptr(err), n, d,
           d_t, FUSED_HIDDEN, cfg, _hip.stream_ptr(x.device))
diff --git a/flowconductor_amd/options.py b/flowconductor_amd/options.py
--- a/flowconductor_amd/options.py
+++ b/flowconductor_amd/options.py
@@ -8,6 +8,7 @@
     "sylvester_mm": True,
     "ar_incremental": "auto",
     "ar_device_loop": True,
+    "split_hidden_handover": True,
     "rq_force_tile": False,
     "fused_training": True,
     "paranoid_caches": False,
diff --git a/flowconductor_amd/transforms/coupling.py b/flowconductor_amd/transforms/coupling.py
--- a/flowconductor_amd/transforms/coupling.py
+++ b/flowconductor_amd/transforms/coupling.py
@@ -463,7 +463,25 @@
             if inverse:
                 identity_split, logabsdet_identity = self.unconditional_transform.inverse(identity_split, context)
         width = 64 if mode == "k8" else ops.general_hidden_width(net.hidden_features)
-        hidden = self._hidden_for_fused(inputs, identity_split, context, width)
+        hidden_rest = None
+        if (mode == "k8" and identity_split is None and context is None and options.get("split_hidden_handover")
+                and options.get("fused_hidden") and net.hip_hidden_supported(inputs.shape[1], None)
+                and self.num_transform_features <= ops.FUSED_DT
+                and ops.fused_linear_split_supported(inputs.shape[1], self.num_transform_features)
+                and ops.split_hidden_supported(net.initial_layer.in_features, len(net.blocks),
+                                               ops.activation_code(net.blocks[0].activation) if len(net.blocks)
+                                               else (ops.ACT_RELU, 0.0))):
+            n = inputs.shape[0]
+            body, body16 = n - n % ops.FUSED_ROWS, n - n % ops.HIDDEN_ROWS
+            hidden = net.hidden_hip(inputs[:body16], self._id_cols(inputs.device), None, split=True, keep_rows=body16 > body)
+            if body16 > body:
+                hidden_rest = hidden.rows[body:]
+                hidden = ops.SplitHidden(hidden.pieces[:body], hidden.unscale[:body])
+            if body16 < n:
+                tail = net.hidden_padded(inputs[body16:, self.identity_features])
+                hidden_rest = tail if hidden_rest is None else torch.cat((hidden_rest, tail))
+        else:
+            hidden = self._hidden_for_fused(inputs, identity_split, context, width)
         chunks = fused_rq.packed_chunks(self, net.final_layer, mode, self.num_bins, self.tails, self._pack_spec)
         kw = self._fused_forward_kw(net, mode, inverse)
 
@@ -472,7 +490,7 @@
             params = torch.nn.functional.linear(h[:, :lin.in_features], lin.weight, lin.bias)
             return self._coupling_kernel(rows, params, inverse)
 
-        outputs, logabsdet = fused_rq.apply(inputs, hidden, chunks, mode, kw, total, leftover)
+        outputs, logabsdet = fused_rq.apply(inputs, hidden, chunks, mode, kw, total, leftover, hidden_rest)
         if self.unconditional_transform is not None:
             if not inverse:
                 identity_split, logabsdet_identity = self.unconditional_transform(identity_split, context)
diff --git a/flowconductor_amd/transforms/fused_rq.py b/flowconductor_amd/transforms/fused_rq.py
--- a/flowconductor_amd/transforms/fused_rq.py
+++ b/flowconductor_amd/transforms/fused_rq.py
@@ -35,16 +35,22 @@
     return rows, lad
 
 
-def apply(inputs, hidden, chunks, mode, kw, total, leftover_fn):
+def apply(inputs, hidden, chunks, mode, kw, total, leftover_fn, hidden_rest=None):
     n = inputs.shape[0]
     body = n - n % ops.FUSED_ROWS
+    if isinstance(hidden, ops.SplitHidden):
+        if body == n:
+            return run_chunks(inputs, hidden, chunks, mode, kw, total)
+        hidden_body = hidden
+    else:
+        hidden_body, hidden_rest = hidden[:body], hidden[body:]
     if body == n:
         if len(chunks) == 1:
             fn = ops.rq_spline_fused_linear if mode == "k8" else ops.rq_spline_fused_general
             return fn(inputs, hidden, *chunks[0], logabsdet_accum=total, **kw)
         return run_chunks(inputs, hidden, chunks, mode, kw, total)
-    out_a, lad_a = run_chunks(inputs[:body], hidden[:body], chunks, mode, kw, None if total is None else total[:body])
-    out_b, lad_b = leftover_fn(inputs[body:].contiguous(), hidden[body:])
+    out_a, lad_a = run_chunks(inputs[:body], hidden_body, chunks, mode, kw, None if total is None else total[:body])
+    out_b, lad_b = leftover_fn(inputs[body:].contiguous(), hidden_rest)
     outputs = torch.cat((out_a, out_b))
     if total is None:
         return outputs, torch.cat((lad_a, lad_b))
diff --git a/include/flowcon_hip.h b/include/flowcon_hip.h
--- a/include/flowcon_hip.h
+++ b/include/flowcon_hip.h
@@ -47,6 +47,11 @@
                               uint32_t* err_flag, int64_t n, int32_t d, int32_t d_t, int32_t hidden,
                               const fc_rq_config* cfg, void* stream);
 
+int fc_rq_spline_fused_linear_split(const float* x, float* y, const void* h_split, const float* h_unscale,
+                                    const float* w_pad, const float* bias_pad, const int32_t* cols, float* logabsdet,
+                                    uint32_t* err_flag, int64_t n, int32_t d, int32_t d_t, int32_t hidden,
+                                    const fc_rq_config* cfg, void* stream);
+
 int fc_rq_spline_fused_general(const float* x, float* y, const float* h, const void* w_frag,
                                const float* w_unscale, const float* bias_pad, const int32_t* cols,
                                float* logabsdet, uint32_t* err_flag, int64_t n, int32_t d, int32_t d_t,
@@ -115,6 +120,11 @@
                             const float* w_unscale, const float* bias_acc, int64_t n, int32_t d,
                             int32_t in_features, int32_t hidden, int32_t num_blocks, int32_t activation,
                             float activation_param, void* stream);
+
+int fc_resnet_hidden_packed_split(const float* x, float* h, void* h_split, float* h_unscale, const int32_t* id_cols,
+                                  const void* w_frag, const float* w_unscale, const float* bias_acc, int64_t n, int32_t d,
+                                  int32_t in_features, int32_t hidden, int32_t num_blocks, int32_t activation,
+                                  float activation_param, void* stream);
 
 int fc_affine_coupling_resnet(const float* x, float* y, const int32_t* id_cols, const int32_t* tr_cols,
                               const void* w_frag, const float* w_unscale, const float* bias_acc, float* logabsdet,
```
